# hku-mars/BALM

Measured on AMD Instinct MI355X. Metric: BA iterations/sec (W poses x F plane features), higher is better.
Workload: dtype f64

## Files before the change

### balm_amd/capi.py

```python
import ctypes as C
import os

import numpy as np

_HERE = os.path.dirname(os.path.abspath(__file__))
LIB_PATH = os.environ.get("BALM_HIP_LIB") or os.path.join(_HERE, "lib", "libbalm_hip.so")

FORM_LEFT, FORM_RIGHT = 0, 1
OK, ERR_ARG, ERR_HIP, ERR_STATE, ERR_TOO_FEW_PLANES, ERR_NUMERIC = range(6)
ABI_VERSION = 6
FLAG_TIMING = 1
FLAG_LOOPBACK_SHARDS = 2
FLAG_SYRK_INT8 = 4
T_MOMENTS, T_FACTORS, T_SYRK, T_ASSEMBLE, T_SOLVE, T_UPDATE, T_BUILD, T_VOXEL, T_COV, T_COMM, T_UPLOAD, T_COUNT = range(12)
TIMING_NAMES = ["moments", "factors", "syrk", "assemble", "solve", "update", "build", "voxel", "cov", "comm", "upload"]

EXPORTS = ["balm_create", "balm_prewarm", "balm_create_multi", "balm_destroy", "balm_set_features", "balm_set_features_cb", "balm_evaluate", "balm_only_residual",
           "balm_solve_damped", "balm_damping_iter", "balm_build_clusters", "balm_build_clusters_planes", "balm_voxel_defaults", "balm_associate", "balm_associate_scans", "balm_get_features", "balm_get_association", "balm_pose_covariance",
           "balm_window_open", "balm_window_add_scan", "balm_window_add_scan_strided", "balm_window_recut", "balm_window_get_points", "balm_window_features", "balm_window_marginalize", "balm_window_info", "balm_window_close",
           "balm_set_allreduce", "balm_comm_unique_id", "balm_comm_init_rank", "balm_comm_info",
           "balm_get_timing", "balm_get_shard_timing", "balm_get_solve_trace", "balm_chain_macro_plan", "balm_reset_timing", "balm_work_model", "balm_last_error", "balm_version", "balm_abi_version"]


class IterLog(C.Structure):
    _fields_ = [("r1", C.c_double), ("r2", C.c_double), ("u", C.c_double), ("v", C.c_double),
                ("q", C.c_double), ("q1", C.c_double), ("accepted", C.c_int), ("hess_evaluated", C.c_int)]


class LMOpts(C.Structure):
    _fields_ = [("form", C.c_int), ("u0", C.c_double), ("max_iter", C.c_int), ("rel_tol", C.c_double),
                ("min_planes_per_pose", C.c_int), ("force_hess", C.c_int), ("no_stop", C.c_int),
                ("verbose", C.c_int), ("reanchor", C.c_int), ("abs_tol", C.c_double)]


class VoxelOpts(C.Structure):
    _fields_ = [("voxel_size", C.c_double), ("eigen_thr", C.c_float * 3), ("min_ps", C.c_int), ("layer_limit", C.c_int),
                ("min_observers", C.c_int), ("fix_frames", C.c_int), ("max_plane_dist", C.c_double),
                ("max_lambda21", C.c_double), ("max_lambda0", C.c_double), ("want_point_features", C.c_int),
                ("fix_point_limit", C.c_int), ("defer_recut", C.c_int)]


ALLREDUCE_FN = C.CFUNCTYPE(C.c_int, C.c_void_p, C.c_long, C.c_void_p)
FILL_CLUSTERS_FN = C.CFUNCTYPE(None, C.c_void_p, C.c_int, C.c_int, C.POINTER(C.c_double))

_LIB = None


class BalmError(RuntimeError):
    def __init__(self, code, msg):
        super().__init__("balm_hip error %d: %s" % (code, msg))
        self.code = code


def lib():
    global _LIB
    if _LIB is None:
        if not os.path.exists(LIB_PATH):
            raise ImportError("libbalm_hip.so is not built (%s missing): run `python -m balm_amd.build`. "
                              "There is no CPU fallback for the HIP path." % LIB_PATH)
        L = C.CDLL(LIB_PATH)
        abi = getattr(L, "balm_abi_version", None)
        abi = abi() if abi is not None else 0
        if abi != ABI_VERSION:
            raise ImportError("libbalm_hip.so has ABI revision %d, this binding was written for %d: rebuild (python -m balm_amd.build)"
                              % (abi, ABI_VERSION))
        L.balm_create.restype = C.c_void_p
        L.balm_create.argtypes = [C.c_int, C.c_int, C.c_int]
        L.balm_create_multi.restype = C.c_void_p
        L.balm_create_multi.argtypes = [C.c_int, C.c_int, C.c_int, C.c_int]
        L.balm_prewarm.argtypes = [C.c_int]
        L.balm_destroy.restype = None
        L.balm_destroy.argtypes = [C.c_void_p]
        L.balm_set_features.argtypes = [C.c_void_p, C.c_int, C.c_void_p, C.c_void_p, C.c_void_p]
        L.balm_set_features_cb.argtypes = [C.c_void_p, C.c_int, FILL_CLUSTERS_FN, C.c_void_p, C.c_void_p, C.c_void_p]
        L.balm_evaluate.argtypes = [C.c_void_p, C.c_int, C.c_void_p, C.c_int, C.c_int, C.c_void_p, C.c_void_p,
                                    C.POINTER(C.c_double)]
        L.balm_only_residual.argtypes = [C.c_void_p, C.c_void_p, C.POINTER(C.c_double)]
        L.balm_solve_damped.argtypes = [C.c_void_p, C.c_void_p, C.c_void_p, C.c_double, C.c_void_p,
                                        C.POINTER(C.c_double)]
        L.balm_damping_iter.argtypes = [C.c_void_p, C.POINTER(LMOpts), C.c_void_p, C.POINTER(IterLog),
                                        C.POINTER(C.c_int)]
        L.balm_build_clusters.argtypes = [C.c_void_p, C.c_int, C.c_void_p, C.c_void_p, C.c_void_p, C.c_long,
                                          C.c_void_p, C.c_void_p, C.c_void_p]
        L.balm_build_clusters_planes.argtypes = [C.c_void_p, C.c_int, C.c_void_p, C.c_void_p, C.c_size_t, C.c_size_t, C.c_void_p,
                                                 C.c_void_p, C.c_void_p]
        L.balm_associate_scans.argtypes = [C.c_void_p, C.POINTER(VoxelOpts), C.c_int, C.c_void_p, C.c_void_p, C.c_size_t,
                                           C.c_void_p, C.POINTER(C.c_int), C.POINTER(C.c_long)]
        L.balm_window_add_scan_strided.argtypes = [C.c_void_p, C.c_void_p, C.c_long, C.c_size_t, C.c_void_p]
        L.balm_window_open.argtypes = [C.c_void_p, C.POINTER(VoxelOpts)]
        L.balm_window_add_scan.argtypes = [C.c_void_p, C.c_void_p, C.c_long, C.c_void_p]
        L.balm_window_recut.argtypes = [C.c_void_p]
        L.balm_window_get_points.argtypes = [C.c_void_p, C.c_void_p, C.c_void_p, C.c_void_p, C.c_long, C.c_void_p]
        L.balm_window_features.argtypes = [C.c_void_p, C.POINTER(C.c_int)]
        L.balm_window_marginalize.argtypes = [C.c_void_p, C.c_int, C.c_void_p]
        L.balm_window_info.argtypes = [C.c_void_p, C.POINTER(C.c_int), C.POINTER(C.c_long), C.POINTER(C.c_long)]
        L.balm_window_close.argtypes = [C.c_void_p]
        L.balm_associate.argtypes = [C.c_void_p, C.POINTER(VoxelOpts), C.c_void_p, C.c_void_p, C.c_long, C.c_void_p,
                                     C.POINTER(C.c_int), C.POINTER(C.c_long)]
        L.balm_get_features.argtypes = [C.c_void_p, C.c_void_p, C.c_void_p, C.c_void_p]
        L.balm_get_association.argtypes = [C.c_void_p, C.c_void_p, C.c_void_p]
        L.balm_voxel_defaults.restype = None
        L.balm_voxel_defaults.argtypes = [C.POINTER(VoxelOpts)]
        L.balm_pose_covariance.argtypes = [C.c_void_p, C.c_void_p, C.c_void_p, C.c_double, C.c_void_p, C.c_void_p]
        L.balm_set_allreduce.argtypes = [C.c_void_p, ALLREDUCE_FN, C.c_void_p]
        L.balm_comm_unique_id.argtypes = [C.c_void_p]
        L.balm_comm_init_rank.argtypes = [C.c_void_p, C.c_int, C.c_int, C.c_void_p]
        L.balm_comm_info.argtypes = [C.c_void_p, C.c_void_p]
        L.balm_get_timing.argtypes = [C.c_void_p, C.c_void_p, C.c_void_p]
        L.balm_get_shard_timing.argtypes = [C.c_void_p, C.c_int, C.c_void_p, C.c_void_p]
        L.balm_get_solve_trace.argtypes = [C.c_void_p, C.c_void_p, C.c_long, C.c_void_p]
        L.balm_chain_macro_plan.argtypes = [C.c_int, C.c_int, C.c_void_p, C.c_long]
        L.balm_reset_timing.argtypes = [C.c_void_p]
        L.balm_work_model.argtypes = [C.c_void_p, C.c_void_p]
        L.balm_last_error.restype = C.c_char_p
        L.balm_last_error.argtypes = [C.c_void_p]
        L.balm_version.restype = C.c_char_p
        _LIB = L
    return _LIB


def chain_macro_plan(panels, helpers):
    tab = np.empty(helpers * 64, np.int32)
    rc = lib().balm_chain_macro_plan(int(panels), int(helpers), tab.ctypes.data_as(C.c_void_p), tab.size)
    if rc != OK:
        raise BalmError(rc, "balm_chain_macro_plan(%d, %d)" % (panels, helpers))
    tab = tab.reshape(helpers, 64)
    return [[(int(e) & 0xffff, int(e) >> 16) for e in row if e >= 0] for row in tab]


def _p(a):
    return None if a is None else a.ctypes.data_as(C.c_void_p)


def _c(a, dtype=np.float64):
    return None if a is None else np.ascontiguousarray(a, dtype=dtype)


class Context:

    def __init__(self, win_size, device=0, flags=0, n_devices=None):
        self.L = lib()
        self.W = int(win_size)
        self.n = 6 * self.W
        if n_devices is None:
            self.h = self.L.balm_create(self.W, int(device), int(flags))
        else:
            self.h = self.L.balm_create_multi(self.W, int(device), int(n_devices), int(flags))
        if not self.h:
            raise BalmError(ERR_HIP, "balm_create(win_size=%d, device=%d, n_devices=%s) failed (no GPU, bad device, or "
                                     "win_size out of range)" % (win_size, device, n_devices))
        self.F = 0
        self._cb = None

    def close(self):
        if getattr(self, "h", None):
            self.L.balm_destroy(self.h)
            self.h = None

    def __del__(self):
        try:
            self.close()
        except Exception:
            pass

    def _check(self, rc):
        if rc != OK:
# ... 284 lines not shown
```

### balm_amd/csrc/balm_capi.hip

```cpp
#include <algorithm>
#include <array>
#include <atomic>
#include <chrono>
#include <cmath>
#include <cstdio>
#include <cstdlib>
#include <cstring>

#include "balm_internal.h"

using namespace balm;

#define HIP_TRY(expr)                                                                              \
  do {                                                                                             \
    hipError_t e_ = (expr);                                                                        \
    if (e_ != hipSuccess) {                                                                        \
      ctx->err = std::string(#expr) + ": " + hipGetErrorString(e_);                                \
      return BALM_ERR_HIP;                                                                         \
    }                                                                                              \
  } while (0)

namespace {

#ifdef BALM_COLD_TRACE
// ... 18 lines not shown
};
static DeviceWarm g_warm[64];

static void warm_body(int device) {
  DeviceWarm &w = g_warm[device];
  if (hipSetDevice(device) != hipSuccess) { hipGetLastError(); return; }
  std::thread ring_th([&w, device] {
    if (hipSetDevice(device) == hipSuccess && w.ring.init(device) == hipSuccess) w.ring_ready.store(true, std::memory_order_release);
    else hipGetLastError();
  });
  (void)preload_voxel(); (void)preload_build(); (void)prepare_device_accum(); (void)preload_solve(); (void)prepare_device_cov();
  hipGetLastError();
  ring_th.join();
}

static int warm_start(int device) {
  if (device < 0 || device >= 64) return BALM_ERR_ARG;
  DeviceWarm &w = g_warm[device];
  std::lock_guard<std::mutex> lk(w.mu);
  if (!w.started) { w.started = true; w.th = std::thread(warm_body, device); }
  return BALM_OK;
}

static void adopt_warm_ring(balm_ctx *ctx) {
  if (ctx->ring.buf[0] || ctx->device < 0 || ctx->device >= 64) return;
  DeviceWarm &w = g_warm[ctx->device];
  std::lock_guard<std::mutex> lk(w.mu);
  if (!w.started) return;
  if (w.th.joinable()) w.th.join();
  if (w.ring_ready.load(std::memory_order_acquire)) {
    const int key = ctx->ring.pool_key;
    ctx->ring = w.ring; ctx->ring.pool_key = key;
    w.ring = PinnedRing(); w.ring_ready.store(false);
  }
}

struct Span {
  balm_ctx *c; int slot; hipEvent_t a = nullptr, b = nullptr;
  Span(balm_ctx *ctx, int s) : c(ctx), slot(s) {
    if (!c->timer.on) return;
    a = take(); b = take();
    hipEventRecord(a, c->stream);
  }
  ~Span() {
    if (!c->timer.on) return;
    hipEventRecord(b, c->stream);
    c->timer.pending.push_back({a, b, slot});
  }
  hipEvent_t take() {
    if (!c->timer.pool.empty()) { hipEvent_t e = c->timer.pool.back(); c->timer.pool.pop_back(); return e; }
    hipEvent_t e; hipEventCreate(&e); return e;
  }
};

void collect_timing(balm_ctx *c) {
  for (auto &sp : c->timer.pending) {
    float ms = 0;
    if (hipEventElapsedTime(&ms, sp.a, sp.b) == hipSuccess) { c->timer.ms[sp.slot] += ms; c->timer.cnt[sp.slot]++; }
    c->timer.pool.push_back(sp.a); c->timer.pool.push_back(sp.b);
  }
  c->timer.pending.clear();
}

template <class T>
int dalloc(balm_ctx *ctx, T **p, size_t count) {
  if (*p) { hipFree(*p); *p = nullptr; }
  if (count == 0) count = 1;
  HIP_TRY(hipMalloc((void **)p, count * sizeof(T)));
  return BALM_OK;
}

template <class T>
int keep(balm_ctx *ctx, T **p, size_t *cap, size_t count) {
  if (*p && *cap >= count) return BALM_OK;
  for (int k = 0; k < balm_ctx::LM_GRAPHS; k++)
    if (ctx->lm_graph[k]) { hipGraphExecDestroy(ctx->lm_graph[k]); ctx->lm_graph[k] = nullptr; ctx->lm_graph_form[k] = -1; }
  int rc = dalloc(ctx, p, count + count / 4);
  *cap = rc ? 0 : count + count / 4;
  return rc;
}

template <class T>
int ensure(balm_ctx *ctx, T **p, size_t *cap, size_t count) {
  if (*p && *cap >= count) return BALM_OK;
  for (int k = 0; k < balm_ctx::LM_GRAPHS; k++)
    if (ctx->lm_graph[k]) { hipGraphExecDestroy(ctx->lm_graph[k]); ctx->lm_graph[k] = nullptr; ctx->lm_graph_form[k] = -1; }
  int rc = dalloc(ctx, p, count);
  if (rc) return rc;
  *cap = count;
  return BALM_OK;
}

int stage_begin(balm_ctx *ctx, size_t total_bytes) {
  total_bytes += 16 * 256;
  ctx->stage_off = 0;
  if (ctx->stage_cap >= total_bytes) return BALM_OK;
  if (ctx->d_stage) { hipStreamSynchronize(ctx->stream); hipFree(ctx->d_stage); ctx->d_stage = nullptr; ctx->stage_cap = 0; }
  const size_t want = total_bytes + total_bytes / 8;
  HIP_TRY(hipMalloc((void **)&ctx->d_stage, want));
  ctx->stage_cap = want;
  return BALM_OK;
}

template <class T>
T *stage_take(balm_ctx *ctx, size_t count) {
  const size_t off = (ctx->stage_off + 255) & ~(size_t)255;
  ctx->stage_off = off + count * sizeof(T);
  return reinterpret_cast<T *>(ctx->d_stage + off);
}

int sync_stream(balm_ctx *ctx) {
  HIP_TRY(hipStreamSynchronize(ctx->stream));
  HIP_TRY(hipGetLastError());
  collect_timing(ctx);
  return BALM_OK;
}

long red_dacc_off(const balm_ctx *c) { return (long)c->ntiles * TILE_ELEMS; }
long red_r_off(const balm_ctx *c) { return red_dacc_off(c) + (long)DACC_MAX * c->W; }

bool has_transport(const balm_ctx *ctx) { return ctx->comm || multi_is_loopback(ctx) || ctx->allreduce; }

int hook_allreduce(balm_ctx *ctx, double *buf, long n) {
  if (ctx->comm) { Span sp(ctx, BALM_T_COMM); return comm_allreduce(ctx, buf, n); }
  if (multi_is_loopback(ctx)) { Span sp(ctx, BALM_T_COMM); return loopback_allreduce(ctx, buf, n); }
  if (!ctx->allreduce) return BALM_OK;
  int rc = sync_stream(ctx);
  if (rc) return rc;
  if (ctx->allreduce((void *)buf, n, ctx->allreduce_user) != 0) {
    ctx->err = "all-reduce hook failed";
    return BALM_ERR_STATE;
  }
  return BALM_OK;
}

int set_damping(balm_ctx *ctx, double u) {
  ctx->u_value = u;
  ctx->u_on_device = false;
  return BALM_OK;
}
int push_damping(balm_ctx *ctx) {
  double *slot = ctx->h_scal + 16 + (ctx->u_ring++ & 63);
  *slot = ctx->u_value;
  HIP_TRY(hipMemcpyAsync(ctx->d_scal + SCAL_U, slot, sizeof(double), hipMemcpyHostToDevice, ctx->stream));
  ctx->u_on_device = true;
  return BALM_OK;
}

static void collect_timing_if_idle(balm_ctx *ctx) {
  if (!ctx->timer.on || ctx->timer.pending.empty()) return;
  if (hipStreamSynchronize(ctx->stream) == hipSuccess) collect_timing(ctx);
}

int wait_scalars(balm_ctx *ctx) {
  volatile double *stamp = ctx->h_scal + SCAL_STAMP;
  const double want = (double)ctx->mail_seq;
  const auto t0 = std::chrono::steady_clock::now();
  for (int spin = 0;; spin++) {
    if (*stamp == want) { std::atomic_thread_fence(std::memory_order_acquire); collect_timing_if_idle(ctx); return BALM_OK; }
    if ((spin & 255) == 255 && std::chrono::steady_clock::now() - t0 > std::chrono::microseconds(300)) break;
  }
  int rc = sync_stream(ctx);
  if (rc) return rc;
  if (*stamp != want) { ctx->err = "balm_damping_iter: the iteration's scalars did not arrive"; return BALM_ERR_HIP; }
  return BALM_OK;
}

void drop_lm_graphs(balm_ctx *ctx) {
  for (int k = 0; k < balm_ctx::LM_GRAPHS; k++) {
    if (ctx->lm_graph[k]) hipGraphExecDestroy(ctx->lm_graph[k]);
    ctx->lm_graph[k] = nullptr; ctx->lm_graph_form[k] = -1;
  }
}

int residual_device(balm_ctx *ctx, const double *d_poses, int f0, int f1, int slot, bool defer_sum = false, bool send_mail = false) {
  if (f1 <= f0) {
    HIP_TRY(hipMemsetAsync(ctx->d_scal + slot, 0, sizeof(double), ctx->stream));
    ctx->nr_tmp = 0;
  } else {
    Span sp(ctx, BALM_T_MOMENTS);
    launch_world_moments(ctx->stream, ctx->d_cl, d_poses, ctx->W, f0, f1, ctx->d_C);
    const EigenMail mail{ctx->d_scal, ctx->d_hscal, send_mail ? (double)++ctx->mail_seq : 0.0, slot};
    ctx->nr_tmp = launch_feature_eigen(ctx->stream, ctx->d_C, ctx->has_fix ? ctx->d_fix : nullptr, ctx->d_coe, f0, f1, ctx->d_feat_tmp,
                                       ctx->d_rpart_tmp, send_mail ? &mail : nullptr);
    if (!defer_sum) launch_sum_scalar(ctx->stream, ctx->d_rpart_tmp, ctx->nr_tmp, ctx->d_scal + slot);
  }
  HIP_TRY(hipGetLastError());
  if (defer_sum) return BALM_OK;
  return hook_allreduce(ctx, ctx->d_scal + slot, 1);
}

bool fuse_trial(const balm_ctx *ctx) {
  const char *e = getenv("BALM_FUSE_TRIAL");
  return ctx->W <= 256 && ctx->F > 0 && e && e[0] == '1';
}

static bool syrk_int8_mode(const balm_ctx *ctx) {
  if (ctx->flags & BALM_FLAG_SYRK_INT8) return true;
  const char *m = getenv("BALM_SYRK");
  return m && !strcmp(m, "int8");
}
static bool syrk_int8_for(const balm_ctx *ctx, long K) {
  if (!syrk_int8_mode(ctx)) return false;
  if (const char *m = getenv("BALM_SYRK_INT8_MIN_COLS")) return K >= atol(m);
  return K >= 12288L && ctx->W >= 96;
}

int prepare_evaluate(balm_ctx *ctx, int form, int nf) {
  if (nf <= 0) return BALM_OK;
  const SyrkPlan plan = plan_syrk(ctx->ntiles, 3L * nf);
  int rc;
  size_t gcols = (size_t)plan.Kpad + 64, parts = (size_t)plan.SG * ctx->ntiles;
  if (ctx->sparse && nf == ctx->F) {
    gcols = (size_t)ctx->sp_nchunks * ctx->sp_nsteps * 4 + 64;
    parts = (size_t)ctx->sp_nitems;
  }
  {
    const double *before = ctx->d_Gt;
    if ((rc = ensure(ctx, &ctx->d_Gt, &ctx->cap_Gt, gcols * ctx->npad))) return rc;
    if (ctx->d_Gt != before) ctx->gt_dirty_cols = ~(size_t)0;
  }
  if ((rc = ensure(ctx, &ctx->d_part, &ctx->cap_part, parts * TILE_ELEMS))) return rc;
  if (syrk_int8_for(ctx, 3L * nf) && !(ctx->sparse && nf == ctx->F)) {
    if ((rc = ensure(ctx, &ctx->d_i8, &ctx->cap_i8, syrk_i8_scratch_bytes(ctx->n, 3L * nf, nullptr)))) return rc;
    if (!ctx->d_rowmax) ctx->rowmax_cur_valid = false;
    if (!ctx->d_rowmax2) ctx->rowmax_trial_valid = false;
    if ((rc = ensure(ctx, &ctx->d_rowmax, &ctx->cap_rowmax, (size_t)ctx->npad + 128))) return rc;
    if ((rc = ensure(ctx, &ctx->d_rowmax2, &ctx->cap_rowmax2, (size_t)ctx->npad + 128))) return rc;
    if ((rc = ensure(ctx, &ctx->d_rowmax_part, &ctx->cap_rowmax_part, (size_t)factors_grid(ctx->W, nf, form) * 6 * ctx->W))) return rc;
    HIP_TRY(prepare_device_syrk_i8());
  }
  if ((rc = ensure(ctx, &ctx->d_dpart, &ctx->cap_dpart, (size_t)factors_grid(ctx->W, nf, form) * DACC_MAX * ctx->W))) return rc;
  if (nf == ctx->F && fuse_trial(ctx)) {
    if (ctx->cap_Gt2 < gcols * ctx->npad || ctx->cap_dpart2 < (size_t)factors_grid(ctx->W, nf, form) * DACC_MAX * ctx->W) ctx->gt_trial_valid = false;
    if ((rc = ensure(ctx, &ctx->d_Gt2, &ctx->cap_Gt2, gcols * ctx->npad))) return rc;
    if ((rc = ensure(ctx, &ctx->d_dpart2, &ctx->cap_dpart2, (size_t)factors_grid(ctx->W, nf, form) * DACC_MAX * ctx->W))) return rc;
  }
  return BALM_OK;
}

int evaluate_device(balm_ctx *ctx, int form, const double *d_poses, int f0, int f1, int slot) {
  const int W = ctx->W, nf = f1 - f0;
  const int dacc = form == 0 ? DACC_LEFT : DACC_RIGHT;
  int rc;
  if (nf <= 0) {
    HIP_TRY(hipMemsetAsync(ctx->d_red, 0, ctx->red_len * sizeof(double), ctx->stream));
    if ((rc = hook_allreduce(ctx, ctx->d_red, (long)ctx->red_len))) return rc;
    Span sp(ctx, BALM_T_ASSEMBLE);
    launch_assemble(ctx->stream, form, ctx->d_red, red_dacc_off(ctx), ctx->d_sub, ctx->ntiles, W, ctx->d_H, ctx->d_g,
                    ctx->d_red + red_r_off(ctx), ctx->d_scal + slot);
    return BALM_OK;
  }
  SyrkPlan plan = plan_syrk(ctx->ntiles, 3L * nf);
  if ((rc = prepare_evaluate(ctx, form, nf))) return rc;
  const int nblk = factors_grid(W, nf, form);
  hipStream_t s = ctx->stream;
  if (!(ctx->feat_cur_valid && f0 == 0 && f1 == ctx->F)) {
    Span sp(ctx, BALM_T_MOMENTS);
    launch_world_moments(s, ctx->d_cl, d_poses, W, f0, f1, ctx->d_C);
    ctx->nr_cur = launch_feature_eigen(s, ctx->d_C, ctx->has_fix ? ctx->d_fix : nullptr, ctx->d_coe, f0, f1, ctx->d_feat, ctx->d_rpart);
    ctx->feat_cur_valid = (f0 == 0 && f1 == ctx->F);
  }
  const int nr = ctx->nr_cur;
  const bool sparse = ctx->sparse && f0 == 0 && f1 == ctx->F;
  const size_t kpad = sparse ? (size_t)ctx->sp_nchunks * ctx->sp_nsteps * 4 : (size_t)plan.Kpad;
  if (!(ctx->gt_cur_valid && ctx->feat_cur_valid && f0 == 0 && f1 == ctx->F)) {
    Span sp(ctx, BALM_T_FACTORS);
    const size_t k0 = (size_t)3 * nf, k1 = kpad + 64;
    if (ctx->gt_dirty_cols == ~(size_t)0) {
      HIP_TRY(hipMemsetAsync(ctx->d_Gt, 0, ctx->cap_Gt * sizeof(double), s));
      ctx->gt_dirty_cols = 0;
    } else if (ctx->gt_dirty_cols > k0) {
      HIP_TRY(hipMemsetAsync(ctx->d_Gt + k0 * ctx->npad, 0, (std::max(ctx->gt_dirty_cols, k1) - k0) * ctx->npad * sizeof(double), s));
    }
    ctx->gt_dirty_cols = k0;
    ctx->rowmax_cur_valid = launch_factors(s, form, ctx->d_cl, d_poses, ctx->d_feat, W, ctx->npad, f0, f1, ctx->d_Gt, ctx->d_dpart, nblk,
                                           sparse ? ctx->d_slot : nullptr, (!sparse && syrk_int8_for(ctx, 3L * nf)) ? ctx->d_rowmax : nullptr, ctx->d_rowmax_part);
    ctx->gt_cur_valid = false;
  }
  HIP_TRY(hipGetLastError());
  const bool int8 = !sparse && syrk_int8_for(ctx, 3L * nf);
  {
    Span sp(ctx, BALM_T_SYRK);
    if (sparse) launch_syrk_sparse(s, ctx->d_Gt, ctx->npad, ctx->d_jobs, ctx->d_items, ctx->d_chunk_ids, ctx->sp_nsteps, ctx->sp_nitems, ctx->d_part);
    else if (int8) {
      if (launch_syrk_i8(s, ctx->d_Gt, ctx->npad, ctx->n, 3L * nf, ctx->d_sub, ctx->ntiles, ctx->d_i8, ctx->d_part,
                         ctx->rowmax_cur_valid ? ctx->d_rowmax : nullptr)) { ctx->err = "INT8 SYRK: unsupported size"; return BALM_ERR_ARG; }
      plan.SG = 1;
    }
    else launch_syrk(s, ctx->d_Gt, ctx->npad, ctx->ntiles, ctx->d_jobs, plan, ctx->d_part);
  }
  {
    Span sp(ctx, BALM_T_ASSEMBLE);
    launch_reduce(s, ctx->d_part, plan.SG, (long)ctx->ntiles * TILE_ELEMS, ctx->d_dpart, nblk, dacc * W,
                  ctx->d_rpart, nr, ctx->d_red, red_dacc_off(ctx), red_r_off(ctx), sparse ? ctx->d_csr : nullptr);
  }
  if ((rc = hook_allreduce(ctx, ctx->d_red, (long)ctx->red_len))) return rc;
  {
    Span sp(ctx, BALM_T_ASSEMBLE);
    launch_assemble(s, form, ctx->d_red, red_dacc_off(ctx), ctx->d_sub, ctx->ntiles, W, ctx->d_H, ctx->d_g, ctx->d_red + red_r_off(ctx),
                    ctx->d_scal + slot);
  }
  return BALM_OK;
}

int trial_device(balm_ctx *ctx, int form, const double *d_poses, int slot) {
  const int W = ctx->W, F = ctx->F;
  hipStream_t s = ctx->stream;
  const SyrkPlan plan = plan_syrk(ctx->ntiles, 3L * F);
  const bool sparse = ctx->sparse;
  const size_t kpad = sparse ? (size_t)ctx->sp_nchunks * ctx->sp_nsteps * 4 : (size_t)plan.Kpad;
  const int nblk = factors_grid(W, F, form);
  {
    Span sp(ctx, BALM_T_FACTORS);
    const size_t k0 = (size_t)3 * F, k1 = kpad + 64;
    HIP_TRY(hipMemsetAsync(ctx->d_Gt2 + k0 * ctx->npad, 0, (k1 - k0) * ctx->npad * sizeof(double), s));
    if (ctx->npad > ctx->n)
      HIP_TRY(hipMemset2DAsync(ctx->d_Gt2 + ctx->n, (size_t)ctx->npad * sizeof(double), 0,
                               (size_t)(ctx->npad - ctx->n) * sizeof(double), k0, s));
    ctx->nr_tmp = launch_moments_factors(s, form, ctx->d_cl, d_poses, ctx->has_fix ? ctx->d_fix : nullptr, ctx->d_coe, W, ctx->npad, F,
                                         ctx->d_Gt2, ctx->d_dpart2, nblk, sparse ? ctx->d_slot : nullptr, ctx->d_feat_tmp, ctx->d_rpart_tmp,
                                         (!sparse && syrk_int8_for(ctx, 3L * F) && ctx->d_rowmax2) ? ctx->d_rowmax2 : nullptr, ctx->d_rowmax_part);
    ctx->rowmax_trial_valid = !sparse && syrk_int8_for(ctx, 3L * F) && ctx->d_rowmax2;
  }
  HIP_TRY(hipGetLastError());
  {
    Span sp(ctx, BALM_T_MOMENTS);
    launch_sum_scalar(s, ctx->d_rpart_tmp, ctx->nr_tmp, ctx->d_scal + slot);
  }
  ctx->gt_trial_valid = true;
  return hook_allreduce(ctx, ctx->d_scal + slot, 1);
}

int read_scalars(balm_ctx *ctx) {
  HIP_TRY(hipMemcpyAsync(ctx->h_scal, ctx->d_scal, 16 * sizeof(double), hipMemcpyDeviceToHost, ctx->stream));
  return sync_stream(ctx);
}

std::vector<unsigned char> obs_of(const double *clusters, int F, int W) {
  std::vector<unsigned char> obs((size_t)F * W);
  parallel_ranges(obs.size(), (size_t)1 << 16, [&](size_t lo, size_t hi) {
    for (size_t t = lo; t < hi; t++) obs[t] = clusters[t * 10 + 9] != 0 ? 1 : 0;
  });
  return obs;
}

int feature_bookkeeping(balm_ctx *ctx, int F, const unsigned char *obs, const double *fix, const double *coeffs) {
  const int W = ctx->W;
  ctx->planes_per_pose.assign(W, 0);
  double S = 0, B = 0;
  int bad_a = F, bad_rc = BALM_OK;
  std::mutex mu;
  parallel_ranges((size_t)F, (size_t)(65536 / W + 1), [&](size_t lo, size_t hi) {
    std::vector<int> ppp((size_t)W, 0);
    double s = 0, b = 0;
    int my_bad = F, my_rc = BALM_OK;
    for (size_t a = lo; a < hi; a++) {
      int na = 0;
      const unsigned char *oa = obs + a * W;
      for (int i = 0; i < W; i++)
        if (oa[i]) { ppp[(size_t)i]++; na++; }
      if (my_rc == BALM_OK) {
        if (na == 0 && !(fix && fix[a * 10 + 9] != 0)) { my_bad = (int)a; my_rc = BALM_ERR_NUMERIC; }
        else if (!(coeffs[a] >= 0) || !std::isfinite(coeffs[a])) { my_bad = (int)a; my_rc = BALM_ERR_ARG; }
      }
      s += na; b += 0.5 * na * (na + 1.0);
    }
    std::lock_guard<std::mutex> lk(mu);
    for (int i = 0; i < W; i++) ctx->planes_per_pose[(size_t)i] += ppp[(size_t)i];
    S += s; B += b;
    if (my_rc != BALM_OK && my_bad < bad_a) { bad_a = my_bad; bad_rc = my_rc; }
  });
  if (bad_rc == BALM_ERR_NUMERIC) {
    ctx->err = "feature " + std::to_string(bad_a) + " has no observation and no fix cluster (zero point count)";
    return BALM_ERR_NUMERIC;
  }
  if (bad_rc == BALM_ERR_ARG) {
    ctx->err = "feature " + std::to_string(bad_a) + " has a negative or non-finite weight";
    return BALM_ERR_ARG;
  }
  ctx->work_S = S; ctx->work_B = B;
  return BALM_OK;
}

}

extern "C" {

const char *balm_version(void) { return "balm_hip 0.6.0 (gfx950)"; }
int balm_abi_version(void) { return BALM_ABI_VERSION; }

const char *balm_last_error(balm_ctx *ctx) { return ctx ? ctx->err.c_str() : "null context"; }

static void one_destroy(balm_ctx *ctx);

balm_ctx *balm_create(int win_size, int device, int flags) {
  if (win_size < 1 || win_size > MAX_W) return nullptr;
  cold_mark("balm_create: enter");
  int ndev = 0;
  if (hipGetDeviceCount(&ndev) != hipSuccess || ndev < 1 || device < 0 || device >= ndev) return nullptr;
  if (hipSetDevice(device) != hipSuccess) return nullptr;
  cold_mark("balm_create: hipGetDeviceCount + hipSetDevice");
  warm_start(device);
  if (prepare_device_accum() != hipSuccess || prepare_device_cov() != hipSuccess) return nullptr;
  cold_mark("balm_create: prepare_device (function attributes -> code objects)");
  balm_ctx *ctx = new balm_ctx();
  ctx->W = win_size;
  ctx->n = 6 * win_size;
  ctx->npad = (ctx->n + TILE - 1) / TILE * TILE;
  ctx->T = ctx->npad / TILE;
  ctx->nA = (ctx->n + NB - 1) / NB * NB;
  ctx->device = device;
  ctx->flags = flags;
  ctx->timer.on = (flags & BALM_FLAG_TIMING) != 0;
  auto fail = [&]() -> balm_ctx * { one_destroy(ctx); return nullptr; };
  std::vector<int> jobs, sub;
  {
    const int T = ctx->T, ngroups = T / 5;
    std::vector<std::array<int, 3>> mixed[4];
    std::vector<std::array<int, 2>> pairs;
    for (int r = 0; r < TM; r++) for (int c = r; c < TM; c++) pairs.push_back({r, c});
    for (int k = 0; k < 15; k++) mixed[1].push_back({0, pairs[k][0], pairs[k][1]});
    for (int k = 0; k < 10; k++) mixed[1].push_back({1, pairs[k][0], pairs[k][1]});
    for (int k = 10; k < 15; k++) mixed[2].push_back({1, pairs[k][0], pairs[k][1]});
    for (int k = 0; k < 15; k++) mixed[2].push_back({2, pairs[k][0], pairs[k][1]});
    for (int k = 0; k < 5; k++) mixed[2].push_back({3, pairs[k][0], pairs[k][1]});
    for (int k = 5; k < 15; k++) mixed[3].push_back({3, pairs[k][0], pairs[k][1]});
    for (int k = 0; k < 15; k++) mixed[3].push_back({4, pairs[k][0], pairs[k][1]});
    auto regular = [&](int I, int J) {
      jobs.insert(jobs.end(), {0, I, J, 0});
      for (int t = 0; t < 25; t++) sub.push_back(((TM * I + t / TM) << 16) | (TM * J + t % TM));
    };
    for (int m = 0; m < T; m++) {
      for (int i = 0; i < m; i++) regular(i, m);
      if (m >= TM * ngroups) regular(m, m);
      else if (m % TM == TM - 1) {
        const int b = m - (TM - 1);
        for (int v = 1; v <= 3; v++) {
          jobs.insert(jobs.end(), {v, b, b, 0});
          for (const auto &e : mixed[v]) sub.push_back(((TM * (b + e[0]) + e[1]) << 16) | (TM * (b + e[0]) + e[2]));
        }
      }
    }
  }
  ctx->ntiles = (int)(jobs.size() / 4);
  ctx->h_jobs = jobs;
  if (hipStreamCreateWithFlags(&ctx->stream, hipStreamNonBlocking) != hipSuccess) return fail();
  cold_mark("balm_create: job tables + stream");
  const int W = ctx->W, n = ctx->n, nA = ctx->nA;
  ctx->red_len = (size_t)ctx->ntiles * TILE_ELEMS + (size_t)DACC_MAX * W + 2;
  if (dalloc(ctx, &ctx->d_poses, (size_t)12 * W) || dalloc(ctx, &ctx->d_poses_tmp, (size_t)12 * W) ||
      dalloc(ctx, &ctx->d_red, ctx->red_len) || dalloc(ctx, &ctx->d_jobs, jobs.size()) || dalloc(ctx, &ctx->d_sub, sub.size()) ||
      dalloc(ctx, &ctx->d_H, (size_t)n * n) || dalloc(ctx, &ctx->d_g, (size_t)n) ||
      dalloc(ctx, &ctx->d_A, (size_t)(2 * nA + NB) * nA) || dalloc(ctx, &ctx->d_Wp, (size_t)2 * NB * (2 * nA + NB)) ||
      dalloc(ctx, &ctx->d_dvec, (size_t)nA) || dalloc(ctx, &ctx->d_z, (size_t)nA) || dalloc(ctx, &ctx->d_x, (size_t)16 * nA) ||
      dalloc(ctx, &ctx->d_perm, (size_t)nA) || dalloc(ctx, &ctx->d_flags, (size_t)2 * (2 * (nA / NB) + 1) * (nA / NB) + (nA / NB) + 8) || dalloc(ctx, &ctx->d_minv, (size_t)2 * (nA / NB) * NB * NB) || dalloc(ctx, &ctx->d_dx, (size_t)n) ||
      dalloc(ctx, &ctx->d_scal, (size_t)16) || dalloc(ctx, &ctx->d_pre, (size_t)W + 2))
    return fail();
  if (hipHostMalloc((void **)&ctx->h_scal, (16 + 64 + 8) * sizeof(double), hipHostMallocMapped | hipHostMallocCoherent) != hipSuccess) return fail();
  if (hipHostGetDevicePointer((void **)&ctx->d_hscal, ctx->h_scal, 0) != hipSuccess) return fail();
  ctx->h_scal[SCAL_STAMP] = 0.0;
  if (hipMemcpy(ctx->d_jobs, jobs.data(), jobs.size() * sizeof(int), hipMemcpyHostToDevice) != hipSuccess ||
      hipMemcpy(ctx->d_sub, sub.data(), sub.size() * sizeof(int), hipMemcpyHostToDevice) != hipSuccess)
    return fail();
  if (getenv("BALM_SOLVE_TRACE")) {
    const size_t cnt = (size_t)(2 * (nA / NB) + 1) * (nA / NB) * 6 + (size_t)(nA / NB) * 6;
    if (hipMalloc((void **)&ctx->d_trace, cnt * sizeof(long long)) != hipSuccess) return fail();
    hipMemset(ctx->d_trace, 0, cnt * sizeof(long long));
  }
  {
    std::vector<int> ident(nA);
    for (int i = 0; i < nA; i++) ident[i] = i;
    if (hipMemcpy(ctx->d_perm, ident.data(), (size_t)nA * sizeof(int), hipMemcpyHostToDevice) != hipSuccess) return fail();
  }
  if (hipMemset(ctx->d_scal, 0, 16 * sizeof(double)) != hipSuccess) return fail();
  if (hipMemset(ctx->d_red, 0, ctx->red_len * sizeof(double)) != hipSuccess) return fail();
  if (hipMemset(ctx->d_minv, 0, (size_t)2 * (nA / NB) * NB * NB * sizeof(double)) != hipSuccess) return fail();
  cold_mark("balm_create: device buffers + small copies");
  context_born(device); ctx->counted_live = true;
  return ctx;
}

static void one_destroy(balm_ctx *ctx) {
  if (!ctx) return;
  if (ctx->counted_live) { context_gone(ctx->device); ctx->counted_live = false; }
  comm_destroy(ctx);
  drop_lm_graphs(ctx);
  hipSetDevice(ctx->device);
  if (ctx->stream) hipStreamSynchronize(ctx->stream);
  if (ctx->window) { window_close(ctx->window); ctx->window = nullptr; }
  void *ptrs[] = {ctx->d_cl, ctx->d_fix, ctx->d_coe, ctx->d_poses, ctx->d_poses_tmp, ctx->d_C, ctx->d_feat,
                  ctx->d_Gt, ctx->d_Gt2, ctx->d_dpart2, ctx->d_part, ctx->d_dpart, ctx->d_rpart, ctx->d_feat_tmp, ctx->d_rpart_tmp, ctx->d_red, ctx->d_jobs, ctx->d_sub, ctx->d_H,
                  ctx->d_g, ctx->d_A, ctx->d_Wp, ctx->d_dvec, ctx->d_z, ctx->d_x, ctx->d_perm, ctx->d_dx, ctx->d_scal, ctx->d_arena, ctx->d_pre, ctx->d_flags, ctx->d_minv, ctx->d_macro_tab, ctx->d_trace, ctx->d_slot, ctx->d_items, ctx->d_csr, ctx->d_chunk_ids, ctx->d_stage, ctx->d_i8, ctx->d_rowmax, ctx->d_rowmax2, ctx->d_rowmax_part};
  for (void *p : ptrs) if (p) hipFree(p);
  if (ctx->h_scal) hipHostFree(ctx->h_scal);
  ctx->ring.release();
  if (ctx->amail.host) hipHostFree((void *)ctx->amail.host);
  if (ctx->amail.scan_state) hipFree(ctx->amail.scan_state);
  for (auto &sp : ctx->timer.pending) { hipEventDestroy(sp.a); hipEventDestroy(sp.b); }
  for (auto e : ctx->timer.pool) hipEventDestroy(e);
  if (ctx->stream) hipStreamDestroy(ctx->stream);
  delete ctx;
}

static int build_sparse_plan(balm_ctx *ctx, int F, const unsigned char *obs) {
  ctx->sparse = false;
  const char *mode = getenv("BALM_SYRK");
  if (mode && !strcmp(mode, "dense")) return BALM_OK;
  if (syrk_int8_for(ctx, 3L * F)) return BALM_OK;
  const int W = ctx->W, T = ctx->T, ntiles = ctx->ntiles;
  if (T > 128 || T <= 2 || F < 64) return BALM_OK;
  struct Key { uint64_t hi, lo; int a; };
  std::vector<Key> keys((size_t)F);
  parallel_ranges((size_t)F, (size_t)(65536 / W + 1), [&](size_t a0, size_t a1) {
    for (size_t a = a0; a < a1; a++) {
      uint64_t hi = 0, lo = 0;
      const unsigned char *oa = obs + a * W;
      for (int i = 0; i < W; i++)
        if (oa[i])
          for (int b = (6 * i) / TILE; b <= (6 * i + 5) / TILE; b++) {
            if (b < 64) hi |= 1ull << (63 - b); else lo |= 1ull << (127 - b);
          }
      keys[a] = {hi, lo, (int)a};
    }
  });
  auto first_of = [&](const Key &k) { for (int b = 0; b < T; b++) if (b < 64 ? (k.hi >> (63 - b)) & 1 : (k.lo >> (127 - b)) & 1) return b; return T; };
  auto last_of = [&](const Key &k) { for (int b = T - 1; b >= 0; b--) if (b < 64 ? (k.hi >> (63 - b)) & 1 : (k.lo >> (127 - b)) & 1) return b; return -1; };
  std::vector<int> fb((size_t)F), lb((size_t)F);
  for (int a = 0; a < F; a++) { fb[(size_t)a] = first_of(keys[(size_t)a]); lb[(size_t)a] = last_of(keys[(size_t)a]); }
  std::sort(keys.begin(), keys.end(), [&](const Key &x, const Key &y) {
    if (fb[(size_t)x.a] != fb[(size_t)y.a]) return fb[(size_t)x.a] < fb[(size_t)y.a];
    if (lb[(size_t)x.a] != lb[(size_t)y.a]) return lb[(size_t)x.a] < lb[(size_t)y.a];
    return x.hi != y.hi ? x.hi > y.hi : (x.lo != y.lo ? x.lo > y.lo : x.a < y.a);
  });
  const int C = 16, nsteps = 3 * C / 4, nchunks = (F + C - 1) / C;
  auto touched = [](const Key &k, int b) { return b < 64 ? (k.hi >> (63 - b)) & 1 : (k.lo >> (127 - b)) & 1; };
  std::vector<int> slot((size_t)F);
  std::vector<std::vector<int>> chunks_of((size_t)ntiles);
  long total = 0;
  for (int c = 0; c < nchunks; c++) {
    Key cm{0, 0, 0};
    for (int k = c * C; k < F && k < (c + 1) * C; k++) { cm.hi |= keys[(size_t)k].hi; cm.lo |= keys[(size_t)k].lo; slot[(size_t)keys[(size_t)k].a] = k; }
    for (int j = 0; j < ntiles; j++) {
      const int type = ctx->h_jobs[(size_t)4 * j], I = ctx->h_jobs[(size_t)4 * j + 1], J = ctx->h_jobs[(size_t)4 * j + 2];
      bool need;
      if (type == 0) need = touched(cm, I) && touched(cm, J);
      else if (type == 1) need = touched(cm, I) || touched(cm, I + 1);
      else if (type == 2) need = touched(cm, I + 1) || touched(cm, I + 2) || touched(cm, I + 3);
      else need = touched(cm, I + 3) || touched(cm, I + 4);
      if (need) { chunks_of[(size_t)j].push_back(c); total++; }
    }
  }
  const double dense_steps = (double)ntiles * ((3.0 * F + 3) / 4), sparse_steps = (double)total * nsteps;
  const bool forced = mode && !strcmp(mode, "sparse");
  if (total == 0 || (!forced && !(sparse_steps < 0.8 * dense_steps))) return BALM_OK;
  long per = total / 2048;
  if (per < 8) per = 8;
  std::vector<int> items, chunk_ids, csr((size_t)ntiles + 1, 0);
  struct Order { int first_chunk, item; };
  std::vector<Order> order;
  int run = 0;
  for (int j = 0; j < ntiles; j++) {
    csr[(size_t)j] = run;
    const std::vector<int> &L = chunks_of[(size_t)j];
    const long pieces = ((long)L.size() + per - 1) / per;
    for (long q = 0; q < pieces; q++) {
      const size_t b = (size_t)((long)L.size() * q / pieces), e = (size_t)((long)L.size() * (q + 1) / pieces);
      order.push_back({L[b], (int)(items.size() / 4)});
      items.insert(items.end(), {j, (int)chunk_ids.size(), (int)(e - b), run++});
      chunk_ids.insert(chunk_ids.end(), L.begin() + (long)b, L.begin() + (long)e);
    }
  }
  csr[(size_t)ntiles] = run;
  std::stable_sort(order.begin(), order.end(), [](const Order &x, const Order &y) { return x.first_chunk < y.first_chunk; });
  std::vector<int> sorted_items;
  sorted_items.reserve(items.size());
  for (const Order &o : order) sorted_items.insert(sorted_items.end(), items.begin() + 4L * o.item, items.begin() + 4L * o.item + 4);
  if (chunk_ids.empty()) chunk_ids.push_back(0);
  int rc;
  if ((rc = keep(ctx, &ctx->d_slot, &ctx->cap_slot, (size_t)F)) || (rc = keep(ctx, &ctx->d_items, &ctx->cap_items, sorted_items.size())) ||
      (rc = keep(ctx, &ctx->d_chunk_ids, &ctx->cap_chunk_ids, chunk_ids.size())) || (rc = keep(ctx, &ctx->d_csr, &ctx->cap_csr, csr.size())))
    return rc;
  HIP_TRY(hipMemcpy(ctx->d_slot, slot.data(), slot.size() * sizeof(int), hipMemcpyHostToDevice));
  HIP_TRY(hipMemcpy(ctx->d_items, sorted_items.data(), sorted_items.size() * sizeof(int), hipMemcpyHostToDevice));
  HIP_TRY(hipMemcpy(ctx->d_chunk_ids, chunk_ids.data(), chunk_ids.size() * sizeof(int), hipMemcpyHostToDevice));
  HIP_TRY(hipMemcpy(ctx->d_csr, csr.data(), csr.size() * sizeof(int), hipMemcpyHostToDevice));
  ctx->sparse = true; ctx->sp_nsteps = nsteps; ctx->sp_nchunks = nchunks; ctx->sp_nitems = run; ctx->sp_steps = sparse_steps;
  return BALM_OK;
}

static int install_feature_buffers(balm_ctx *ctx, int F, const double *fix, const double *coeffs,
                                   hipMemcpyKind kind = hipMemcpyHostToDevice) {
  int rc;
  drop_lm_graphs(ctx);
  ctx->has_fix = fix != nullptr;
  if (fix) {
    if ((rc = keep(ctx, &ctx->d_fix, &ctx->cap_fix, (size_t)F * 10))) return rc;
    HIP_TRY(hipMemcpyAsync(ctx->d_fix, fix, (size_t)F * 10 * sizeof(double), kind, ctx->stream));
  }
  if ((rc = keep(ctx, &ctx->d_coe, &ctx->cap_coe, (size_t)F))) return rc;
  HIP_TRY(hipMemcpyAsync(ctx->d_coe, coeffs, (size_t)F * sizeof(double), kind, ctx->stream));
  if ((rc = keep(ctx, &ctx->d_C, &ctx->cap_C, (size_t)F * 10))) return rc;
  if ((rc = keep(ctx, &ctx->d_feat, &ctx->cap_feat, (size_t)F * FEAT_STRIDE))) return rc;
  if ((rc = keep(ctx, &ctx->d_feat_tmp, &ctx->cap_feat_tmp, (size_t)F * FEAT_STRIDE))) return rc;
  if ((rc = keep(ctx, &ctx->d_rpart, &ctx->cap_rpart, (size_t)(F + 255) / 256 + 1024 + 1))) return rc;
  if ((rc = keep(ctx, &ctx->d_rpart_tmp, &ctx->cap_rpart_tmp, (size_t)(F + 255) / 256 + 1024 + 1))) return rc;
  ctx->feat_cur_valid = false; ctx->gt_cur_valid = false;
  ctx->F = F;
  return BALM_OK;
}

static int assoc_clusters_host(balm_ctx *ctx);

using FillClusters = std::function<void(int, int, double *, unsigned char *)>;

static int one_set_features_fn(balm_ctx *ctx, int F, const FillClusters &fill, const double *fix, const double *coeffs, bool shard_books = false) {
  if (!ctx) return BALM_ERR_ARG;
  if (ctx->multi && F == 0) { ctx->F = 0; ctx->feat_cur_valid = false; ctx->gt_cur_valid = false; ctx->planes_per_pose.clear(); ctx->work_S = ctx->work_B = 0; return BALM_OK; }
  if (F < 1 || !fill || !coeffs) { ctx->err = "balm_set_features: bad argument"; return BALM_ERR_ARG; }
  HIP_TRY(hipSetDevice(ctx->device));
  const int W = ctx->W;
  const size_t count = (size_t)F * W * 10;
  int rc;
  if ((rc = assoc_clusters_host(ctx))) return rc;
  ctx->F = 0;
  adopt_warm_ring(ctx);
  if ((rc = keep(ctx, &ctx->d_cl, &ctx->cap_cl, count))) return rc;
  if ((rc = stage_begin(ctx, count * sizeof(double)))) return rc;
  double *d_aos = stage_take<double>(ctx, count);
  std::vector<unsigned char> obs((size_t)F * W);
  const size_t unit = (size_t)W * 10 * sizeof(double);
  hipError_t e;
  {
    Span sp(ctx, BALM_T_UPLOAD);
    e = staged_upload(ctx->ring, ctx->device, ctx->stream, d_aos, count * sizeof(double), unit, [&](char *dst, size_t off, size_t len) {
      const int f0 = (int)(off / unit), f1 = f0 + (int)(len / unit);
      fill(f0, f1, reinterpret_cast<double *>(dst), obs.data() + (size_t)f0 * W);
    });
  }
  if (e == hipSuccess) launch_transpose_clusters(ctx->stream, d_aos, ctx->d_cl, F, W);
  HIP_TRY(e);
  if ((!ctx->multi || shard_books) && (rc = feature_bookkeeping(ctx, F, obs.data(), fix, coeffs))) { hipStreamSynchronize(ctx->stream); return rc; }
  if ((rc = build_sparse_plan(ctx, F, obs.data()))) { hipStreamSynchronize(ctx->stream); return rc; }
  if ((rc = install_feature_buffers(ctx, F, fix, coeffs))) { hipStreamSynchronize(ctx->stream); return rc; }
  return sync_stream(ctx);
}

static int one_set_features(balm_ctx *ctx, int F, const double *clusters, const double *fix, const double *coeffs) {
  if (ctx && !(ctx->multi && F == 0) && !clusters) { ctx->err = "balm_set_features: bad argument"; return BALM_ERR_ARG; }
  const size_t row = ctx ? (size_t)ctx->W * 10 : 0;
  return one_set_features_fn(ctx, F, [clusters, row](int f0, int f1, double *dst, unsigned char *o) {
    const double *src = clusters + (size_t)f0 * row;
    stream_copy(dst, src, (size_t)(f1 - f0) * row * sizeof(double));
// ... 415 lines not shown
  const int nblk = cov_factors_grid(W, F > 0 ? F : 1);
  if ((rc = ensure(ctx, &ctx->d_dpart, &ctx->cap_dpart, (size_t)nblk * DACC_MAX * W))) return rc;
  const bool int8 = F > 0 && syrk_int8_for(ctx, 3L * F);
  if (int8) {
    if ((rc = ensure(ctx, &ctx->d_i8, &ctx->cap_i8, syrk_i8_scratch_bytes(ctx->n, 3L * F, nullptr)))) return rc;
    HIP_TRY(prepare_device_syrk_i8());
  }
  const size_t pay = 2 * tiles + (size_t)21 * W, nn = (size_t)n * n;
  const size_t ncc = (cluster_cov && F > 0) ? (size_t)F * W * 81 : 0;
  if ((rc = stage_begin(ctx, (pay + 2 * nn + 2 * (size_t)nA * nA + ncc) * sizeof(double)))) return rc;
  double *buf = stage_take<double>(ctx, pay + 2 * nn + 2 * (size_t)nA * nA), *d_cc = nullptr;
  double *redx = buf, *redy = buf + tiles, *sdiag = buf + 2 * tiles, *Rraw = buf + pay, *Rc = Rraw + nn,
         *T0 = Rc + nn, *T1 = T0 + (size_t)nA * nA;
  hipError_t e = hipSuccess;
  if (ncc) {
    d_cc = stage_take<double>(ctx, ncc);
    adopt_warm_ring(ctx);
    if (e == hipSuccess) { Span sp(ctx, BALM_T_UPLOAD); e = staged_copy(ctx->ring, ctx->device, s, d_cc, cluster_cov, (size_t)F * W * 81 * sizeof(double)); }
  }
  double *Gx = ctx->d_Gt, *Gy = ctx->d_Gt + gcols * ctx->npad;
  if (e == hipSuccess && F == 0) e = hipMemsetAsync(buf, 0, pay * sizeof(double), s);
  if (e == hipSuccess && F > 0) {
    Span sp(ctx, BALM_T_COV);
    const size_t k0 = (size_t)3 * F;
    hipMemsetAsync(Gx + k0 * ctx->npad, 0, (gcols - k0) * ctx->npad * sizeof(double), s);
    hipMemsetAsync(Gy + k0 * ctx->npad, 0, (gcols - k0) * ctx->npad * sizeof(double), s);
    launch_cov_factors(s, ctx->d_cl, d_cc, point_sigma * point_sigma, ctx->d_poses, ctx->d_feat, W, ctx->npad, F, Gx, Gy,
                       ctx->d_dpart, nblk);
    e = hipGetLastError();
    if (int8) {
      if (launch_syrk_i8(s, Gx, ctx->npad, ctx->n, 3L * F, ctx->d_sub, ctx->ntiles, ctx->d_i8, ctx->d_part)) e = hipErrorInvalidValue;
      launch_cov_reduce_tiles(s, ctx->d_part, 1, (long)tiles, redx);
      if (launch_syrk_i8(s, Gy, ctx->npad, ctx->n, 3L * F, ctx->d_sub, ctx->ntiles, ctx->d_i8, ctx->d_part)) e = hipErrorInvalidValue;
      launch_cov_reduce_tiles(s, ctx->d_part, 1, (long)tiles, redy);
    } else {
      launch_syrk(s, Gx, ctx->npad, ctx->ntiles, ctx->d_jobs, plan, ctx->d_part);
      launch_cov_reduce_tiles(s, ctx->d_part, plan.SG, (long)tiles, redx);
      launch_syrk(s, Gy, ctx->npad, ctx->ntiles, ctx->d_jobs, plan, ctx->d_part);
      launch_cov_reduce_tiles(s, ctx->d_part, plan.SG, (long)tiles, redy);
    }
    launch_cov_reduce_dacc(s, ctx->d_dpart, nblk, W, sdiag);
  }
  if (e == hipSuccess) rc = hook_allreduce(ctx, buf, (long)pay);
  if (e == hipSuccess && !rc) {
    Span sp(ctx, BALM_T_COV);
    launch_cov_assemble(s, redx, redy, sdiag, ctx->d_sub, ctx->ntiles, W, Rraw);
    hipMemsetAsync(ctx->d_g, 0, (size_t)n * sizeof(double), s);
    set_damping(ctx, 0.0);
    ctx->need_minv = true;
    launch_solve(ctx, true);
    ctx->need_minv = false;
    launch_congruence_inverse(ctx, Rraw, T0, T1, Rc);
    if (Rcov) e = hipMemcpyAsync(Rcov, Rc, nn * sizeof(double), hipMemcpyDeviceToHost, s);
    if (e == hipSuccess && Rcov_raw) e = hipMemcpyAsync(Rcov_raw, Rraw, nn * sizeof(double), hipMemcpyDeviceToHost, s);
  }
  if (e == hipSuccess) e = hipStreamSynchronize(s);
  if (e == hipSuccess) e = hipGetLastError();
  if (rc) return rc;
  HIP_TRY(e);
  collect_timing(ctx);
  return BALM_OK;
}

int balm_comm_info(balm_ctx *ctx, long *out4) {
  if (!ctx || !out4) return BALM_ERR_ARG;
  out4[0] = 1; out4[1] = 0; out4[2] = (long)ctx->red_len; out4[3] = 0;
  if (ctx->comm) {
    int cnt = -1, rk = -1;
    comm_query(ctx, &cnt, &rk);
    out4[0] = cnt; out4[1] = rk; out4[3] = 1;
  } else if (multi_is_loopback(ctx)) {
    out4[0] = ctx->multi->n; out4[1] = ctx->rank; out4[3] = 2;
  } else if (ctx->allreduce) {
    out4[0] = -1; out4[3] = 3;
  }
  return BALM_OK;
}

int balm_set_allreduce(balm_ctx *ctx, balm_allreduce_fn fn, void *user) {
  if (!ctx) return BALM_ERR_ARG;
  if (fn && (ctx->multi || ctx->comm)) { ctx->err = "balm_set_allreduce: the context already has a collective transport"; return BALM_ERR_STATE; }
  ctx->allreduce = fn;
  ctx->allreduce_user = user;
  return BALM_OK;
}

static int one_evaluate(balm_ctx *ctx, int form, const double *poses, int head, int end, double *Hess, double *JacT,
                  double *residual) {
  if (!ctx) return BALM_ERR_ARG;
  if (!ctx->multi) {
    if (ctx->F < 1) { ctx->err = "balm_evaluate: no features installed"; return BALM_ERR_STATE; }
    if ((form != 0 && form != 1) || !poses || head < 0 || end > ctx->F || head >= end) {
      ctx->err = "balm_evaluate: bad argument"; return BALM_ERR_ARG;
    }
  }
  HIP_TRY(hipSetDevice(ctx->device));
  const int n = ctx->n;
  HIP_TRY(hipMemcpyAsync(ctx->d_poses, poses, (size_t)12 * ctx->W * sizeof(double), hipMemcpyHostToDevice, ctx->stream));
  ctx->feat_cur_valid = false; ctx->gt_cur_valid = false;
  int rc = evaluate_device(ctx, form, ctx->d_poses, head, end, 0);
  ctx->feat_cur_valid = false; ctx->gt_cur_valid = false;
  if (rc) return rc;
  if (Hess) HIP_TRY(hipMemcpyAsync(Hess, ctx->d_H, (size_t)n * n * sizeof(double), hipMemcpyDeviceToHost, ctx->stream));
  if (JacT) HIP_TRY(hipMemcpyAsync(JacT, ctx->d_g, (size_t)n * sizeof(double), hipMemcpyDeviceToHost, ctx->stream));
  if ((rc = read_scalars(ctx))) return rc;
  if (residual) *residual = ctx->h_scal[0];
  if (!std::isfinite(ctx->h_scal[0])) { ctx->err = "balm_evaluate: non-finite residual"; return BALM_ERR_NUMERIC; }
  return BALM_OK;
}

static int one_only_residual(balm_ctx *ctx, const double *poses, double *residual) {
  if (!ctx) return BALM_ERR_ARG;
  if (!ctx->multi && ctx->F < 1) { ctx->err = "balm_only_residual: no features installed"; return BALM_ERR_STATE; }
  if (!poses || !residual) { ctx->err = "balm_only_residual: bad argument"; return BALM_ERR_ARG; }
  HIP_TRY(hipSetDevice(ctx->device));
  HIP_TRY(hipMemcpyAsync(ctx->d_poses_tmp, poses, (size_t)12 * ctx->W * sizeof(double), hipMemcpyHostToDevice, ctx->stream));
  int rc = residual_device(ctx, ctx->d_poses_tmp, 0, ctx->F, 1);
  if (rc) return rc;
  if ((rc = read_scalars(ctx))) return rc;
  *residual = ctx->h_scal[1];
  if (!std::isfinite(ctx->h_scal[1])) { ctx->err = "balm_only_residual: non-finite residual"; return BALM_ERR_NUMERIC; }
  return BALM_OK;
}

int balm_solve_damped(balm_ctx *ctx, const double *Hess, const double *JacT, double u, double *dxi, double *q1) {
  if (!ctx) return BALM_ERR_ARG;
  if (!Hess || !JacT || !dxi) { ctx->err = "balm_solve_damped: bad argument"; return BALM_ERR_ARG; }
  HIP_TRY(hipSetDevice(ctx->device));
  const int n = ctx->n;
  HIP_TRY(hipMemcpyAsync(ctx->d_H, Hess, (size_t)n * n * sizeof(double), hipMemcpyHostToDevice, ctx->stream));
  HIP_TRY(hipMemcpyAsync(ctx->d_g, JacT, (size_t)n * sizeof(double), hipMemcpyHostToDevice, ctx->stream));
  {
    Span sp(ctx, BALM_T_SOLVE);
    int rcu = set_damping(ctx, u);
    if (rcu) return rcu;
    launch_solve(ctx, true);
  }
  HIP_TRY(hipMemcpyAsync(dxi, ctx->d_dx, (size_t)n * sizeof(double), hipMemcpyDeviceToHost, ctx->stream));
  int rc = read_scalars(ctx);
  if (rc) return rc;
  if (!std::isfinite(ctx->h_scal[2]) && !ctx->persistent_off && solve_timed_out(ctx)) {
    ctx->persistent_off = true;
    {
      Span sp(ctx, BALM_T_SOLVE);
      launch_solve(ctx, true);
    }
    HIP_TRY(hipMemcpyAsync(dxi, ctx->d_dx, (size_t)n * sizeof(double), hipMemcpyDeviceToHost, ctx->stream));
    if ((rc = read_scalars(ctx))) return rc;
  }
  if (q1) *q1 = ctx->h_scal[2];
  return BALM_OK;
}

static int lm_enqueue(balm_ctx *ctx, int form, bool evaluated, bool mail) {
  int rc;
  if (evaluated && (rc = evaluate_device(ctx, form, ctx->d_poses, 0, ctx->F, 0))) return rc;
  {
    Span sp(ctx, BALM_T_SOLVE);
    launch_solve(ctx, evaluated, form, ctx->d_poses, ctx->d_poses_tmp);
  }
  ctx->gt_trial_valid = false;
  bool sum_in_mail = false;
  if (fuse_trial(ctx) && ctx->d_Gt2 && ctx->d_dpart2) {
    if ((rc = trial_device(ctx, form, ctx->d_poses_tmp, 1))) return rc;
  } else {
    sum_in_mail = mail && !has_transport(ctx) && ctx->F > 0;
    const bool eigen_mails = sum_in_mail && ctx->F <= 256;
    if ((rc = residual_device(ctx, ctx->d_poses_tmp, 0, ctx->F, 1, sum_in_mail, eigen_mails))) return rc;
    if (eigen_mails) return BALM_OK;
  }
  if (mail) launch_scalars_mail(ctx->stream, ctx->d_scal, ctx->d_hscal, (double)++ctx->mail_seq, sum_in_mail ? ctx->d_rpart_tmp : nullptr,
                                ctx->nr_tmp, 1);
  else HIP_TRY(hipMemcpyAsync(ctx->h_scal, ctx->d_scal, 16 * sizeof(double), hipMemcpyDeviceToHost, ctx->stream));
  return BALM_OK;
}

static int lm_iteration(balm_ctx *ctx, int form, bool evaluated, int it) {
  const char *genv = getenv("BALM_GRAPH");
  const bool disabled = !(genv && (!strcmp(genv, "1") || !strcmp(genv, "debug")));
  const bool graphable = !disabled && ctx->graphs_ok && it >= 1 && !ctx->timer.on && !has_transport(ctx) && !ctx->multi &&
                         ctx->feat_cur_valid && ctx->F > 0 && !solve_is_persistent(ctx);
  if (graphable) {
    const bool fused = fuse_trial(ctx) && ctx->d_Gt2 && ctx->d_dpart2;
    const int slot = (ctx->gt_parity ? 16 : 0) | (fused ? 8 : 0) | (ctx->gt_cur_valid ? 4 : 0) | (evaluated ? 2 : 0) | ctx->parity;
    if (ctx->lm_graph[slot] && ctx->lm_graph_form[slot] != form) {
      hipGraphExecDestroy(ctx->lm_graph[slot]); ctx->lm_graph[slot] = nullptr;
    }
    if (!ctx->lm_graph[slot]) {
      hipGraph_t g = nullptr;
      ctx->u_on_device = true;
      bool ok = hipStreamBeginCapture(ctx->stream, hipStreamCaptureModeThreadLocal) == hipSuccess;
      if (ok) {
        const int rc = lm_enqueue(ctx, form, evaluated, false);
        const hipError_t e = hipStreamEndCapture(ctx->stream, &g);
        ok = rc == BALM_OK && e == hipSuccess && g != nullptr;
      }
      if (ok) ok = hipGraphInstantiate(&ctx->lm_graph[slot], g, nullptr, nullptr, 0) == hipSuccess;
      if (g) hipGraphDestroy(g);
      if (genv && !strcmp(genv, "debug")) fprintf(stderr, "balm_hip: LM graph slot %d capture %s\n", slot, ok ? "ok" : "FAILED");
      if (!ok) {
        hipGetLastError();
        ctx->lm_graph[slot] = nullptr;
        ctx->graphs_ok = false;
      } else {
        ctx->lm_graph_form[slot] = form;
      }
    }
    if (ctx->lm_graph[slot]) {
      int rcu = push_damping(ctx);
      if (rcu) return rcu;
      HIP_TRY(hipGraphLaunch(ctx->lm_graph[slot], ctx->stream));
      return sync_stream(ctx);
    }
    ctx->u_on_device = false;
  }
  int rc = lm_enqueue(ctx, form, evaluated, true);
  if (rc) return rc;
  return wait_scalars(ctx);
}

static int one_damping_iter(balm_ctx *ctx, const balm_lm_opts *o, double *poses, balm_iter_log *log, int *n_iters) {
  if (!ctx) return BALM_ERR_ARG;
  if (!ctx->multi && ctx->F < 1) { ctx->err = "balm_damping_iter: no features installed"; return BALM_ERR_STATE; }
  if (!o || !poses || (o->form != 0 && o->form != 1) || o->max_iter < 1) {
    ctx->err = "balm_damping_iter: bad argument"; return BALM_ERR_ARG;
  }
  if (n_iters) *n_iters = 0;
  HIP_TRY(hipSetDevice(ctx->device));
  const int W = ctx->W, F = ctx->F;
  hipStream_t s = ctx->stream;
  cold_mark("damping_iter: enter");
  int rc = prepare_evaluate(ctx, o->form, F);
  cold_mark("damping_iter: prepare_evaluate (scratch allocations)");
  std::vector<double> pre((size_t)W + 2, 0.0);
  for (size_t i = 0; i < ctx->planes_per_pose.size() && i < (size_t)W; i++) pre[i] = ctx->planes_per_pose[i];
  pre[(size_t)W] = rc ? 1.0 : 0.0;
  if (has_transport(ctx)) {
    int rc2;
    if (hipMemcpyAsync(ctx->d_pre, pre.data(), pre.size() * sizeof(double), hipMemcpyHostToDevice, s) != hipSuccess) return BALM_ERR_HIP;
    if ((rc2 = hook_allreduce(ctx, ctx->d_pre, (long)pre.size()))) return rc2;
    if (hipMemcpyAsync(pre.data(), ctx->d_pre, pre.size() * sizeof(double), hipMemcpyDeviceToHost, s) != hipSuccess) return BALM_ERR_HIP;
    if ((rc2 = sync_stream(ctx))) return rc2;
    if (pre[(size_t)W] != 0.0 && !rc) { ctx->err = "balm_damping_iter: another rank failed before the loop"; rc = BALM_ERR_STATE; }
  }
  if (rc) return rc;
  if (o->min_planes_per_pose > 0) {
    double mn = pre[0];
    for (int i = 1; i < W; i++) mn = pre[(size_t)i] < mn ? pre[(size_t)i] : mn;
    if (mn < o->min_planes_per_pose) {
      ctx->err = "Initial error too large. Please loose plane determination criteria for more planes. "
                 "The optimization is terminated.";
      return BALM_ERR_TOO_FEW_PLANES;
    }
  }
  HIP_TRY(hipMemcpyAsync(ctx->d_poses, poses, (size_t)12 * W * sizeof(double), hipMemcpyHostToDevice, s));
  ctx->feat_cur_valid = false; ctx->gt_cur_valid = false;
  double u = o->u0, v = 2, r1 = 0, r2 = 0;
  bool calc = true;
  int it = 0;
  int fault_rank = -1, fault_it = -1, timeout_it = -1;
  if (const char *fi = getenv("BALM_FAULT_INJECT")) {
    if (!strncmp(fi, "timeout,", 8)) timeout_it = atoi(fi + 8);
    else if (ctx->multi) sscanf(fi, "%d,%d", &fault_rank, &fault_it);
  }
  while (it < o->max_iter) {
    const bool evaluated = calc || o->force_hess;
    if (ctx->rank == fault_rank && it == fault_it) { ctx->err = "balm_damping_iter: injected fault"; return BALM_ERR_HIP; }
    if (it == timeout_it) { ctx->inject_solve_timeout = true; timeout_it = -1; }
    if ((rc = set_damping(ctx, u))) return rc;
    if ((rc = lm_iteration(ctx, o->form, evaluated, it))) return rc;
    double sc[3] = {ctx->h_scal[0], ctx->h_scal[1], ctx->h_scal[2]};
    if ((rc = multi_share_scalars(ctx, it, sc, 3))) return rc;
    r1 = sc[0]; r2 = sc[1];
    const double q1 = sc[2];
    double q = r1 - r2;
    if (!ctx->multi && !ctx->persistent_off && !(std::isfinite(r2) && std::isfinite(q1)) && std::isfinite(r1) && solve_timed_out(ctx)) {
      ctx->persistent_off = true;
      drop_lm_graphs(ctx);
      ctx->feat_cur_valid = false; ctx->gt_cur_valid = false;
      calc = true;
      continue;
    }
    if (!(std::isfinite(r1) && std::isfinite(r2))) {
      ctx->err = "balm_damping_iter: non-finite residual";
      return BALM_ERR_NUMERIC;
    }
    if (log) { log[it].r1 = r1; log[it].r2 = r2; log[it].u = u; log[it].v = v; log[it].q = q; log[it].q1 = q1;
               log[it].accepted = q > 0; log[it].hess_evaluated = evaluated; }
    if (o->verbose)
    {
      printf("iter%d: (%lf %lf) u: %lf v: %.1lf q: %.3lf %lf %lf\n", it, r1, r2, u, v, q / q1, q1, q);
      fflush(stdout);
    }
    if (q > 0) {
      double *t = ctx->d_poses; ctx->d_poses = ctx->d_poses_tmp; ctx->d_poses_tmp = t;
      t = ctx->d_feat; ctx->d_feat = ctx->d_feat_tmp; ctx->d_feat_tmp = t;
      t = ctx->d_rpart; ctx->d_rpart = ctx->d_rpart_tmp; ctx->d_rpart_tmp = t;
      ctx->nr_cur = ctx->nr_tmp;
      ctx->feat_cur_valid = true;
      ctx->gt_cur_valid = ctx->gt_trial_valid;
      if (ctx->gt_trial_valid) {
        std::swap(ctx->d_Gt, ctx->d_Gt2); std::swap(ctx->cap_Gt, ctx->cap_Gt2);
        std::swap(ctx->d_rowmax, ctx->d_rowmax2); std::swap(ctx->cap_rowmax, ctx->cap_rowmax2);
        ctx->rowmax_cur_valid = ctx->rowmax_trial_valid;
        ctx->gt_dirty_cols = ~(size_t)0;
        std::swap(ctx->d_dpart, ctx->d_dpart2); std::swap(ctx->cap_dpart, ctx->cap_dpart2);
        ctx->gt_parity ^= 1;
      }
      ctx->parity ^= 1;
      q = q / q1; v = 2; q = 1 - std::pow(2 * q - 1, 3);
      u *= (q < 1.0 / 3.0 ? 1.0 / 3.0 : q);
      calc = true;
    } else {
      u = u * v; v = 2 * v; calc = false;
    }
    it++;
    if (!o->no_stop && std::fabs(r1 - r2) / r1 < o->rel_tol) break;
    if (!o->no_stop && o->abs_tol > 0 && std::fabs(r1 - r2) < o->abs_tol) break;
  }
  ctx->feat_cur_valid = false; ctx->gt_cur_valid = false;
  if (o->reanchor) launch_reanchor(s, W, ctx->d_poses);
  HIP_TRY(hipMemcpyAsync(poses, ctx->d_poses, (size_t)12 * W * sizeof(double), hipMemcpyDeviceToHost, s));
  if ((rc = sync_stream(ctx))) return rc;
  if (n_iters) *n_iters = it;
  cold_mark("damping_iter: done");
  return BALM_OK;
}

static balm_multi *leader_of(balm_ctx *ctx) { return (ctx && ctx->multi && ctx->rank == 0) ? ctx->multi : nullptr; }

int balm_prewarm(int device) {
  int ndev = 0;
  if (hipGetDeviceCount(&ndev) != hipSuccess || device < 0 || device >= ndev) { hipGetLastError(); return BALM_ERR_ARG; }
  return warm_start(device);
}

balm_ctx *balm_create_multi(int win_size, int first_device, int n_devices, int flags) {
  if (n_devices < 1 || n_devices > MAX_SHARDS) return nullptr;
  const bool loopback = (flags & BALM_FLAG_LOOPBACK_SHARDS) != 0;
  HostPool::shard_pool_threads() = n_devices > 4 ? 8 : 0;
  std::vector<balm_ctx *> subs;
  for (int k = 0; k < n_devices; k++) {
    balm_ctx *c = balm_create(win_size, loopback ? first_device : first_device + k, flags);
    if (!c) { for (auto *q : subs) one_destroy(q); return nullptr; }
    c->ring.pool_key = k;
    subs.push_back(c);
  }
  std::string err;
  balm_multi *m = multi_new(subs, loopback, &err);
  if (!m) {
    fprintf(stderr, "balm_create_multi: %s\n", err.c_str());
    for (auto *q : subs) one_destroy(q);
    return nullptr;
  }
  return subs[0];
}

void balm_destroy(balm_ctx *ctx) {
  if (!ctx) return;
  if (balm_multi *m = ctx->multi) {
    std::vector<balm_ctx *> subs = m->sub;
    for (auto *q : subs) { hipSetDevice(q->device); if (q->stream) hipStreamSynchronize(q->stream); }
    multi_delete(m);
    for (auto *q : subs) { q->multi = nullptr; one_destroy(q); }
    return;
  }
  one_destroy(ctx);
}

int balm_comm_unique_id(void *id128) {
  if (!id128) return BALM_ERR_ARG;
  return comm_unique_id(id128);
}

int balm_comm_init_rank(balm_ctx *ctx, int n_ranks, int rank, const void *id128) {
  if (!ctx) return BALM_ERR_ARG;
  if (!id128 || n_ranks < 1 || rank < 0 || rank >= n_ranks) { ctx->err = "balm_comm_init_rank: bad argument"; return BALM_ERR_ARG; }
  if (ctx->multi || ctx->comm) { ctx->err = "balm_comm_init_rank: the context already has a collective transport"; return BALM_ERR_STATE; }
  HIP_TRY(hipSetDevice(ctx->device));
  return comm_init_rank(ctx, n_ranks, rank, id128);
}

static int multi_set_features(balm_ctx *ctx, balm_multi *m, int F, const double *clusters, const double *fix, const double *coeffs) {
  if (F < 1 || !clusters || !coeffs) { ctx->err = "balm_set_features: bad argument"; return BALM_ERR_ARG; }
  m->F = 0;
  m->books_per_shard = false;
  for (size_t k = 1; k < m->sub.size(); k++) { m->sub[k]->planes_per_pose.clear(); m->sub[k]->work_S = m->sub[k]->work_B = 0; }
  const std::vector<unsigned char> obs = obs_of(clusters, F, ctx->W);
  int rc = feature_bookkeeping(ctx, F, obs.data(), fix, coeffs);
  if (rc) return rc;
  {
    const int W = ctx->W;
    std::vector<double> cum((size_t)F + 1, 0.0);
    parallel_ranges((size_t)F, (size_t)(65536 / W + 1), [&](size_t lo, size_t hi) {
      for (size_t a = lo; a < hi; a++) {
        int na = 0;
        const unsigned char *oa = obs.data() + a * W;
        for (int i = 0; i < W; i++) na += oa[i];
        cum[a + 1] = 0.5 * na * (na + 1.0) + 4.0 * na + 1.0;
      }
    });
    for (int a = 0; a < F; a++) cum[(size_t)a + 1] += cum[(size_t)a];
    m->fbeg[0] = 0;
    for (int k = 1; k < m->n; k++) {
      const double target = cum[(size_t)F] * k / m->n;
      int f = (int)(std::lower_bound(cum.begin(), cum.end(), target) - cum.begin());
      if (f < m->fbeg[(size_t)k - 1]) f = m->fbeg[(size_t)k - 1];
      if (f > F) f = F;
      m->fbeg[(size_t)k] = f;
    }
    m->fbeg[(size_t)m->n] = F;
  }
  const size_t W = (size_t)ctx->W;
  rc = multi_run(m, [&](int k) {
    const int f0 = m->fbeg[(size_t)k], nf = m->fbeg[(size_t)k + 1] - f0;
    return one_set_features(m->sub[(size_t)k], nf, clusters + (size_t)f0 * W * 10, fix ? fix + (size_t)f0 * 10 : nullptr, coeffs + f0);
  });
  if (rc) { if (ctx->err.empty()) ctx->err = "balm_set_features: a device failed"; return rc; }
  m->F = F;
  return BALM_OK;
}

int balm_set_features(balm_ctx *ctx, int F, const double *clusters, const double *fix, const double *coeffs) {
  if (balm_multi *m = leader_of(ctx)) return multi_set_features(ctx, m, F, clusters, fix, coeffs);
  return one_set_features(ctx, F, clusters, fix, coeffs);
}

static void multi_cut(balm_multi *m, int F, const std::vector<double> &cum ) {
  m->fbeg[0] = 0;
  for (int k = 1; k < m->n; k++) {
    const double target = cum[(size_t)F] * k / m->n;
    int f = (int)(std::lower_bound(cum.begin(), cum.end(), target) - cum.begin());
    if (f < m->fbeg[(size_t)k - 1]) f = m->fbeg[(size_t)k - 1];
    if (f > F) f = F;
    m->fbeg[(size_t)k] = f;
  }
  m->fbeg[(size_t)m->n] = F;
}

static int multi_done(balm_ctx *ctx, balm_multi *m, int F, int rc, const char *who) {
  if (rc) { if (ctx->err.empty()) ctx->err = std::string(who) + ": a device failed"; for (auto *q : m->sub) if (!q->err.empty()) { ctx->err = q->err; break; } return rc; }
  m->F = F;
  m->books_per_shard = true;
  return BALM_OK;
}

int balm_set_features_cb(balm_ctx *ctx, int F, balm_fill_clusters_fn fill, void *user, const double *fix, const double *coeffs) {
  if (!ctx) return BALM_ERR_ARG;
  if (F < 1 || !fill || !coeffs) { ctx->err = "balm_set_features_cb: bad argument"; return BALM_ERR_ARG; }
  if (balm_multi *m = leader_of(ctx)) {
    const size_t Wc = (size_t)ctx->W, row = Wc * 10;
    m->F = 0;
    std::vector<double> cum((size_t)F + 1, 0.0);
    parallel_ranges((size_t)F, (size_t)(32768 / row + 1), [&](size_t lo, size_t hi) {
      const size_t blk = std::max<size_t>(1, (size_t)65536 / (row * sizeof(double)));
      std::vector<double> scratch(blk * row);
      for (size_t a0 = lo; a0 < hi; a0 += blk) {
        const size_t a1 = std::min(hi, a0 + blk);
        fill(user, (int)a0, (int)a1, scratch.data());
        for (size_t a = a0; a < a1; a++) {
          int na = 0;
          const double *r = scratch.data() + (a - a0) * row;
          for (size_t i = 0; i < Wc; i++) na += r[i * 10 + 9] != 0 ? 1 : 0;
          cum[a + 1] = 0.5 * na * (na + 1.0) + 4.0 * na + 1.0;
        }
      }
    });
    for (int a = 0; a < F; a++) cum[(size_t)a + 1] += cum[(size_t)a];
    multi_cut(m, F, cum);
    int rc = multi_run(m, [&](int k) {
      const int f0 = m->fbeg[(size_t)k], nf = m->fbeg[(size_t)k + 1] - f0;
      return one_set_features_fn(m->sub[(size_t)k], nf, [fill, user, Wc, f0](int a0, int a1, double *dst, unsigned char *o) {
        fill(user, f0 + a0, f0 + a1, dst);
        const size_t cnt = (size_t)(a1 - a0) * Wc;
        for (size_t t = 0; t < cnt; t++) o[t] = dst[t * 10 + 9] != 0 ? 1 : 0;
      }, fix ? fix + (size_t)f0 * 10 : nullptr, coeffs + f0, true);
    });
    return multi_done(ctx, m, F, rc, "balm_set_features_cb");
  }
// ... 286 lines not shown
```

### balm_amd/csrc/balm_internal.h

```cpp
#pragma once
#include <hip/hip_runtime.h>
#include <atomic>
#include <condition_variable>
#include <cstddef>
#include <cstdint>
#include <functional>
#include <mutex>
#include <string>
#include <thread>
#include <vector>

#include "../../include/balm_hip.h"
#include "host_stage.h"

namespace balm {

constexpr int TILE = 80;
constexpr int TM = 5;
constexpr int TILE_ELEMS = TILE * TILE;
constexpr int FEAT_STRIDE = 24;
constexpr int DACC_LEFT = 27;
constexpr int DACC_RIGHT = 30;
constexpr int DACC_MAX = 30;
constexpr int NB = 48;
constexpr int MAX_W_LDS = 480;
constexpr int MAX_W = 1024;
constexpr int MAX_SHARDS = 16;

enum { FT_NN = 0, FT_VBAR = 1, FT_LAM = 4, FT_U0 = 7, FT_U1 = 10, FT_U2 = 13, FT_C0 = 16, FT_C1 = 17,
       FT_C2 = 18, FT_COE = 19 };

struct Timer {
  bool on = false;
  struct Span { hipEvent_t a, b; int slot; };
  std::vector<Span> pending;
  std::vector<hipEvent_t> pool;
  double ms[BALM_T_COUNT] = {0};
  long cnt[BALM_T_COUNT] = {0};
};

}

namespace balm {
struct WindowSession;
struct AssocMail {
  volatile unsigned int *host = nullptr; unsigned int *dev = nullptr; unsigned int seq = 0;
  unsigned long long *scan_state = nullptr; unsigned int scan_gen = 0;
};
constexpr long SCAN_TILES_CAP = 8192;
}

struct balm_ctx {
  int W = 0, n = 0, npad = 0, T = 0, ntiles = 0, device = 0, flags = 0;
  int nA = 0;
  int F = 0;
  hipStream_t stream = nullptr;
  std::string err;

  double *d_cl = nullptr;
  double *d_fix = nullptr;
  double *d_coe = nullptr;
  double *d_poses = nullptr;
  double *d_poses_tmp = nullptr;
  double *d_C = nullptr;
  double *d_feat = nullptr;
  double *d_feat_tmp = nullptr;
  double *d_rpart_tmp = nullptr;
  int nr_cur = 0, nr_tmp = 0;
  bool feat_cur_valid = false;
  double *d_Gt = nullptr;
  double *d_Gt2 = nullptr, *d_dpart2 = nullptr;
  size_t cap_Gt2 = 0, cap_dpart2 = 0;
  size_t gt_dirty_cols = ~(size_t)0;
  bool gt_cur_valid = false;
  int gt_parity = 0;
  bool gt_trial_valid = false;
  size_t cap_cl = 0, cap_fix = 0, cap_coe = 0, cap_C = 0, cap_feat = 0, cap_feat_tmp = 0, cap_rpart = 0, cap_rpart_tmp = 0;
  size_t cap_slot = 0, cap_items = 0, cap_chunk_ids = 0, cap_csr = 0;
  bool has_fix = false;
  size_t cap_Gt = 0;
  double *d_part = nullptr;
  size_t cap_part = 0;
  double *d_dpart = nullptr;
  size_t cap_dpart = 0;
  double *d_rpart = nullptr;
  double *d_red = nullptr;
  size_t red_len = 0;
  std::vector<int> h_jobs;
  bool sparse = false;
  int sp_nsteps = 0, sp_nchunks = 0, sp_nitems = 0;
  int *d_slot = nullptr;
  int *d_items = nullptr;
  int *d_chunk_ids = nullptr;
  double sp_steps = 0;
  int *d_csr = nullptr;
  int *d_jobs = nullptr;
  int *d_sub = nullptr;
  double *d_H = nullptr;
  double *d_g = nullptr;
  double *d_A = nullptr;
  double *d_Wp = nullptr;
  double *d_dvec = nullptr;
  double *d_z = nullptr;
  double *d_x = nullptr;
  int *d_perm = nullptr;
  int *d_flags = nullptr;
  long long *d_trace = nullptr;
  int fused_cap = -1;
  int chain_cap = -1;
  double *d_minv = nullptr;
  int *d_macro_tab = nullptr;
  int macro_tab_P = 0, macro_tab_NH = 0;
  double *d_dx = nullptr;
  double *d_scal = nullptr;
  double *h_scal = nullptr;
  double *d_hscal = nullptr;
  unsigned long long mail_seq = 0;
  bool need_minv = false;
  bool solve_tiled = false;
  int chain_refused_P[2] = {-1, -1};
  bool solve_backsub = false;
  bool counted_live = false;
  bool persistent_off = false;
  bool inject_solve_timeout = false;
  bool small_ready = false, small_refused = false;
  double u_value = 0.0;
  bool u_on_device = false;
  int u_ring = 0;
  static constexpr int LM_GRAPHS = 32;
  hipGraphExec_t lm_graph[LM_GRAPHS] = {};
  int lm_graph_form[LM_GRAPHS] = {};
  bool graphs_ok = true;
  int parity = 0;
  std::vector<int> planes_per_pose;
  double work_S = 0, work_B = 0;
  std::vector<double> assoc_clusters, assoc_coeffs;
  bool assoc_cl_on_device = false;
  std::vector<int> assoc_layer, assoc_point_feat;
  std::vector<double> assoc_fix;
  balm::WindowSession *window = nullptr;
  bool window_dead = false;
  balm::AssocMail amail;
  void *d_arena = nullptr;
  size_t arena_cap = 0;
  char *d_stage = nullptr;
  size_t stage_cap = 0, stage_off = 0;
  balm::PinnedRing ring;
  balm_allreduce_fn allreduce = nullptr;
  void *allreduce_user = nullptr;
  balm::Timer timer;
  void *comm = nullptr;
  std::atomic<bool> comm_dead{false};
  bool comm_aborted = false;
  std::timed_mutex comm_mu;
  int rank = 0, nranks = 1;
  unsigned long long *d_rowmax = nullptr, *d_rowmax2 = nullptr; size_t cap_rowmax = 0, cap_rowmax2 = 0;
  double *d_rowmax_part = nullptr; size_t cap_rowmax_part = 0;
  bool rowmax_cur_valid = false, rowmax_trial_valid = false;
  unsigned char *d_i8 = nullptr; size_t cap_i8 = 0;
  struct balm_multi *multi = nullptr;
  double *d_pre = nullptr;
};

namespace balm {

hipError_t prepare_device_accum();
hipError_t prepare_device_cov();
hipError_t preload_solve();
hipError_t preload_build();
hipError_t preload_voxel();
void launch_transpose_clusters(hipStream_t s, const double *aos, double *soa, int F, int W);
void launch_world_moments(hipStream_t s, const double *cl, const double *poses, int W, int f0, int f1, double *C);
struct EigenMail { double *scal; double *host; double stamp; int slot; };
int launch_feature_eigen(hipStream_t s, const double *C, const double *fix, const double *coe, int f0, int f1,
                         double *feat, double *rpart, const EigenMail *mail = nullptr);
int factors_grid(int W, int nfeat, int form);
int factors_chunk(int W);
bool launch_factors(hipStream_t s, int form, const double *cl, const double *poses, const double *feat, int W,
                    int npad, int f0, int f1, double *Gt, double *dpart, int nblk, const int *slot = nullptr,
                    unsigned long long *rowmax = nullptr, double *rowmax_part = nullptr);
int launch_moments_factors(hipStream_t s, int form, const double *cl, const double *poses, const double *fix, const double *coe, int W,
                           int npad, int F, double *Gt, double *dpart, int nblk, const int *slot, double *feat, double *rpart,
                           unsigned long long *rowmax = nullptr, double *rowmax_part = nullptr);
struct SyrkPlan { int SG; int nsteps; int Kpad; long nblocks; };
SyrkPlan plan_syrk(int ntiles, long K);
void launch_syrk(hipStream_t s, const double *Gt, int npad, int ntiles, const int *tileIJ, const SyrkPlan &p,
                 double *part);
void launch_syrk_sparse(hipStream_t s, const double *Gt, int npad, const int *jobs, const int *items, const int *chunk_ids,
                        int nsteps, long nitems, double *part);
void launch_reduce(hipStream_t s, const double *part, int SG, long tile_elems_total, const double *dpart, int nblk,
                   int dacc_len, const double *rpart, int nr, double *red, long red_dacc_off, long red_r_off,
                   const int *csr_ptr = nullptr);
void launch_assemble(hipStream_t s, int form, const double *red, long red_dacc_off, const int *tileIJ, int ntiles,
                     int W, double *H, double *g, const double *r_in = nullptr, double *r_out = nullptr);
void launch_sum_scalar(hipStream_t s, const double *rpart, int nr, double *out);
struct I8Layout { int T, rows_p, NT, M; long Kp; size_t off_digits, off_rowmax, off_scale, off_part; };
size_t syrk_i8_scratch_bytes(int n, long K, I8Layout *lay);
hipError_t prepare_device_syrk_i8();
int launch_syrk_i8(hipStream_t s, const double *Gt, int npad, int n, long K, const int *tileIJ, int ntiles, unsigned char *scratch, double *part,
                   const unsigned long long *rowmax_known = nullptr);

struct Barrier;
}

struct balm_multi {
  int n = 0;
  bool loopback = false;
  std::vector<balm_ctx *> sub;
  std::vector<int> fbeg;
  int F = 0;
  bool books_per_shard = false;
  std::vector<std::thread> th;
  std::mutex mu;
  std::condition_variable cv_go, cv_done;
  uint64_t gen = 0;
  int pending = 0;
  bool quit = false;
  const std::function<int(int)> *job = nullptr;
  std::vector<int> rc;
  balm::Barrier *bar = nullptr;
  std::atomic<int> abort_rc{0};
  std::atomic<bool> dead{false};
  std::atomic<uint64_t> lm_seq{0};
  uint64_t lm_epoch = 0;
  double lm_vals[2][8] = {{0}};
  std::vector<hipEvent_t> ev1, ev2;
  std::vector<double *> lb_tmp, lb_buf;
  std::vector<size_t> lb_cap;
};

namespace balm {
balm_multi *multi_new(const std::vector<balm_ctx *> &subs, bool loopback, std::string *err);
void multi_delete(balm_multi *m);
int multi_run(balm_multi *m, const std::function<int(int)> &f);
int comm_unique_id(void *out128);
int comm_init_rank(balm_ctx *ctx, int nranks, int rank, const void *id128);
void comm_destroy(balm_ctx *ctx);
const char *rccl_load_error();
int comm_allreduce(balm_ctx *ctx, double *buf, long n);
void comm_query(const balm_ctx *ctx, int *count, int *rank);
int loopback_allreduce(balm_ctx *ctx, double *buf, long n);
bool multi_is_loopback(const balm_ctx *ctx);
int multi_share_scalars(balm_ctx *ctx, int it, double *vals, int count);
void multi_abort(balm_multi *m, int rc);
int multi_host_barrier_rc(balm_ctx *ctx, int rc);

constexpr int SCAL_U = 5;
constexpr int SCAL_STAMP = 16 + 64;
bool chain_macro_plan(int P, int NH, std::vector<int> &tab);
void context_born(int device);
void context_gone(int device);
bool solve_timed_out(balm_ctx *c);
bool solve_is_persistent(const balm_ctx *c);
void launch_solve(balm_ctx *c, bool new_hessian, int upd_form = 0, const double *upd_poses = nullptr, double *upd_out = nullptr);
void launch_update_poses(hipStream_t s, int form, int W, const double *poses, const double *dx, double *out);
void launch_scalars_mail(hipStream_t s, double *d_scal, double *d_hscal, double stamp, const double *rpart = nullptr, int nr = 0,
                         int slot = 0);
void launch_reanchor(hipStream_t s, int W, double *poses);

struct AssocOpts {
  int W;
  double voxel_size;
  float thr[3];
  int min_ps, layer_limit, min_observers, fix_frames;
  double max_dis, ratio21_max, lam0_max;
  int fix_limit = 50;
  int defer_recut = 0;
};
int associate_device(hipStream_t s, const float *d_xyz, const int *d_frame, const long *d_first, const double *d_poses, long n, const AssocOpts &o,
                     void *arena, size_t arena_cap, size_t *arena_need, int *F_out, double **d_out, double **d_coe,
                     double **d_fix, int **d_layer, int **d_point_feat, long *n_roots, AssocMail *mail, bool *outputs_owned);

WindowSession *window_open(hipStream_t s, const AssocOpts &o);
void window_close(WindowSession *w);
int window_add_scan(WindowSession *w, const float *xyz_new, long n_new, const double *pose12, bool xyz_on_host);
int window_recut(WindowSession *w);
int window_marginalize(WindowSession *w, int mg, const double *poses);
int window_features(WindowSession *w, int min_observers, int *F_out, double **d_out, double **d_coe, double **d_fix, int **d_layer);
long window_get_points(WindowSession *w, float *xyz, int *slot, int *feature, long cap);
int window_count(const WindowSession *w);
int window_min_observers(const WindowSession *w);
long window_points(const WindowSession *w);
long window_nodes(const WindowSession *w);

int cov_factors_grid(int W, int F);
void launch_cov_factors(hipStream_t s, const double *cl, const double *ccov, double sigma2, const double *poses,
                        const double *feat, int W, int npad, int F, double *Gx, double *Gy, double *dpart, int nblk);
void launch_cov_reduce_tiles(hipStream_t s, const double *part, int SG, long tile_total, double *red);
void launch_cov_reduce_dacc(hipStream_t s, const double *dpart, int nblk, int W, double *out);
void launch_cov_assemble(hipStream_t s, const double *redx, const double *redy, const double *sdiag, const int *tileIJ,
                         int ntiles, int W, double *Rout);
void launch_congruence_inverse(balm_ctx *c, const double *Rraw, double *T0, double *T1, double *Rcov);

void launch_build_clusters(hipStream_t s, const float *xyz, const int *feat_id, const int *pose_id, long n_pts,
                           int F, int W, double *soa, int *unsorted_flag);
void launch_build_clusters_any(hipStream_t s, const float *xyz, const int *feat_id, const int *pose_id, long n_pts,
                               int F, int W, double *soa);
void launch_soa_to_aos(hipStream_t s, const double *soa, double *aos, int F, int W);
void launch_rebase_ids(hipStream_t s, int *d_id, long n, int base);
void launch_expand_ids(hipStream_t s, const long *d_first, int m, long n, int *d_id);
void launch_unpack_xyzw(hipStream_t s, const float *d_rec, long n, float *d_xyz, int *d_aux);
void launch_obs_mask(hipStream_t s, const double *soa, int F, int W, unsigned char *mask);

}
```

### balm_amd/csrc/kernels_accum.hip

```cpp
#include "balm_internal.h"

namespace balm {

typedef double d4 __attribute__((ext_vector_type(4)));
typedef double d2 __attribute__((ext_vector_type(2)));

__device__ __forceinline__ double wave_sum(double v) {
#pragma unroll
  for (int off = 32; off > 0; off >>= 1) v += __shfl_xor(v, off, 64);
  return v;
}

struct Obs {
  double N;
  double Rv[3];
  double b[3];
  double Pw[6];
};

__device__ __forceinline__ void to_world(const double P[6], const double v[3], double N, const double R[9],
                                         const double p[3], Obs &o) {
  o.N = N;
#pragma unroll
  for (int r = 0; r < 3; r++) o.Rv[r] = R[r] * v[0] + R[3 + r] * v[1] + R[6 + r] * v[2];
// ... 57 lines not shown
  for (int t0 = 0; t0 < 12 * W; t0 += 10 * (int)blockDim.x) {
    double pv[10];
#pragma unroll
    for (int j = 0; j < 10; j++) {
      const int t = t0 + j * (int)blockDim.x + (int)threadIdx.x;
      pv[j] = t < 12 * W ? poses[t] : 0.0;
    }
#pragma unroll
    for (int j = 0; j < 10; j++) {
      const int t = t0 + j * (int)blockDim.x + (int)threadIdx.x;
      if (t < 12 * W) { const int i = t / 12, c = t - 12 * i; sp[c * W + i] = pv[j]; }
    }
  }
  __syncthreads();
  const int lane = threadIdx.x & 63, wv = threadIdx.x >> 6, nw = blockDim.x >> 6;
  for (int a = f0 + blockIdx.x * nw + wv; a < f1; a += gridDim.x * nw) {
    const double *ca = cl + (size_t)a * 10 * W;
    double acc[10];
#pragma unroll
    for (int c = 0; c < 10; c++) acc[c] = 0.0;
    for (int i = lane; i < W; i += 64) {
      double P[6], v[3];
      const double N = ca[(size_t)9 * W + i];
#pragma unroll
      for (int c = 0; c < 6; c++) P[c] = ca[(size_t)c * W + i];
#pragma unroll
      for (int c = 0; c < 3; c++) v[c] = ca[(size_t)(6 + c) * W + i];
      if ((int)N > 0) {
        double R[9], p[3];
#pragma unroll
        for (int c = 0; c < 9; c++) R[c] = sp[c * W + i];
#pragma unroll
        for (int c = 0; c < 3; c++) p[c] = sp[(9 + c) * W + i];
        Obs o;
        to_world(P, v, N, R, p, o);
#pragma unroll
        for (int c = 0; c < 6; c++) acc[c] += o.Pw[c];
#pragma unroll
        for (int c = 0; c < 3; c++) acc[6 + c] += o.b[c];
        acc[9] += N;
      }
    }
#pragma unroll
    for (int c = 0; c < 10; c++) acc[c] = wave_sum(acc[c]);
    if (lane == 0) {
#pragma unroll
      for (int c = 0; c < 10; c++) Cout[(size_t)a * 10 + c] = acc[c];
    }
  }
}

void launch_world_moments(hipStream_t s, const double *cl, const double *poses, int W, int f0, int f1, double *C) {
  int nf = f1 - f0;
  if (nf <= 0) return;
  int grid = (nf + 3) / 4;
  if (grid > 2048) grid = 2048;
  size_t lds = (size_t)12 * W * sizeof(double);
  hipLaunchKernelGGL(k_world_moments, dim3(grid), dim3(256), lds, s, cl, poses, W, f0, f1, C);
}

__device__ __forceinline__ void jrot(double &app, double &aqq, double &apq, double &arp, double &arq, double &v0p,
                                     double &v0q, double &v1p, double &v1q, double &v2p, double &v2q) {
  if (apq == 0.0) return;
  const double theta = (aqq - app) / (2.0 * apq);
  const double t = (theta >= 0.0 ? 1.0 : -1.0) / (fabs(theta) + sqrt(theta * theta + 1.0));
  const double c = 1.0 / sqrt(t * t + 1.0), s = t * c;
  app -= t * apq;
  aqq += t * apq;
  apq = 0.0;
  const double rp = c * arp - s * arq, rq = s * arp + c * arq;
  arp = rp; arq = rq;
  double x, y;
  x = c * v0p - s * v0q; y = s * v0p + c * v0q; v0p = x; v0q = y;
  x = c * v1p - s * v1q; y = s * v1p + c * v1q; v1p = x; v1q = y;
  x = c * v2p - s * v2q; y = s * v2p + c * v2q; v2p = x; v2q = y;
}

__device__ __forceinline__ void eig3_jacobi(double a00, double a01, double a02, double a11, double a12, double a22,
                                            double lam[3], double U[3][3]) {
  double v00 = 1, v01 = 0, v02 = 0, v10 = 0, v11 = 1, v12 = 0, v20 = 0, v21 = 0, v22 = 1;
  for (int sweep = 0; sweep < 30; sweep++) {
    const double off = a01 * a01 + a02 * a02 + a12 * a12;
    const double dia = a00 * a00 + a11 * a11 + a22 * a22;
    if (off <= 1e-300 || off <= 1e-34 * dia) break;
    jrot(a00, a11, a01, a02, a12, v00, v01, v10, v11, v20, v21);
    jrot(a00, a22, a02, a01, a12, v00, v02, v10, v12, v20, v22);
    jrot(a11, a22, a12, a01, a02, v01, v02, v11, v12, v21, v22);
  }
  double l0 = a00, l1 = a11, l2 = a22;
  double c0[3] = {v00, v10, v20}, c1[3] = {v01, v11, v21}, c2[3] = {v02, v12, v22};
#define BALM_CSWAP(la, lb, ca, cb)                                                         \
  if (la > lb) {                                                                            \
    double t_ = la; la = lb; lb = t_;                                                       \
    for (int k_ = 0; k_ < 3; k_++) { double s_ = ca[k_]; ca[k_] = cb[k_]; cb[k_] = s_; }    \
  }
  BALM_CSWAP(l0, l1, c0, c1)
  BALM_CSWAP(l1, l2, c1, c2)
  BALM_CSWAP(l0, l1, c0, c1)
#undef BALM_CSWAP
  lam[0] = l0; lam[1] = l1; lam[2] = l2;
  for (int k = 0; k < 3; k++) { U[k][0] = c0[k]; U[k][1] = c1[k]; U[k][2] = c2[k]; }
}

__global__ __launch_bounds__(256) void k_feature_eigen(const double *__restrict__ C, const double *__restrict__ fix,
                                                       const double *__restrict__ coe, int f0, int f1,
                                                       double *__restrict__ feat, double *__restrict__ rpart, EigenMail mail) {
  __shared__ double sred[256];
  const int a = f0 + blockIdx.x * blockDim.x + threadIdx.x;
  double res = 0.0;
  if (a < f1) {
    double c[10];
#pragma unroll
    for (int k = 0; k < 10; k++) c[k] = C[(size_t)a * 10 + k];
    if (fix) {
#pragma unroll
      for (int k = 0; k < 10; k++) c[k] += fix[(size_t)a * 10 + k];
    }
    const double NN = c[9];
    const double inv = 1.0 / NN;
    const double vb0 = c[6] * inv, vb1 = c[7] * inv, vb2 = c[8] * inv;
    double lam[3], U[3][3];
    eig3_jacobi(c[0] * inv - vb0 * vb0, c[1] * inv - vb0 * vb1, c[2] * inv - vb0 * vb2, c[3] * inv - vb1 * vb1,
                c[4] * inv - vb1 * vb2, c[5] * inv - vb2 * vb2, lam, U);
    const double w = coe[a];
    res = w * lam[0];
    double *f = feat + (size_t)a * FEAT_STRIDE;
    f[FT_NN] = NN;
    f[FT_VBAR] = vb0; f[FT_VBAR + 1] = vb1; f[FT_VBAR + 2] = vb2;
    f[FT_LAM] = lam[0]; f[FT_LAM + 1] = lam[1]; f[FT_LAM + 2] = lam[2];
#pragma unroll
    for (int k = 0; k < 3; k++) {
      f[FT_U0 + k] = U[k][0]; f[FT_U1 + k] = U[k][1]; f[FT_U2 + k] = U[k][2];
    }
    f[FT_C0] = sqrt(2.0 * w) * inv;
    f[FT_C1] = sqrt(2.0 * w / (lam[1] - lam[0])) * inv;
    f[FT_C2] = sqrt(2.0 * w / (lam[2] - lam[0])) * inv;
    f[FT_COE] = w;
  }
  sred[threadIdx.x] = res;
  __syncthreads();
  for (int s = 128; s > 0; s >>= 1) {
    if (threadIdx.x < s) sred[threadIdx.x] += sred[threadIdx.x + s];
    __syncthreads();
  }
  if (threadIdx.x == 0) rpart[blockIdx.x] = sred[0];
  if (!mail.host) return;
  if (threadIdx.x == 0) mail.scal[mail.slot] = sred[0];
  __syncthreads();
  volatile double *host = mail.host;
  if (threadIdx.x < 16) host[threadIdx.x] = ((int)threadIdx.x == mail.slot) ? sred[0] : mail.scal[threadIdx.x];
  __threadfence_system();
  __syncthreads();
  if (threadIdx.x == 0) { host[SCAL_STAMP] = mail.stamp; __threadfence_system(); }
}

int launch_feature_eigen(hipStream_t s, const double *C, const double *fix, const double *coe, int f0, int f1,
                         double *feat, double *rpart, const EigenMail *mail) {
  int nf = f1 - f0;
  if (nf <= 0) return 0;
  int grid = (nf + 255) / 256;
  const EigenMail none{nullptr, nullptr, 0.0, 0};
  hipLaunchKernelGGL(k_feature_eigen, dim3(grid), dim3(256), 0, s, C, fix, coe, f0, f1, feat, rpart, (mail && grid == 1) ? *mail : none);
  return grid;
}

__global__ __launch_bounds__(256) void k_sum_scalar(const double *__restrict__ part, int nr, double *__restrict__ out) {
  __shared__ double sred[256];
  double s = 0.0;
  for (int t = threadIdx.x; t < nr; t += 256) s += part[t];
  sred[threadIdx.x] = s;
  __syncthreads();
  for (int k = 128; k > 0; k >>= 1) {
    if (threadIdx.x < k) sred[threadIdx.x] += sred[threadIdx.x + k];
    __syncthreads();
  }
  if (threadIdx.x == 0) out[0] = sred[0];
}

void launch_sum_scalar(hipStream_t s, const double *rpart, int nr, double *out) {
  hipLaunchKernelGGL(k_sum_scalar, dim3(1), dim3(256), 0, s, rpart, nr, out);
}

__device__ __forceinline__ void cross3(const double a[3], const double b[3], double o[3]) {
  o[0] = a[1] * b[2] - a[2] * b[1];
  o[1] = a[2] * b[0] - a[0] * b[2];
  o[2] = a[0] * b[1] - a[1] * b[0];
}

__device__ __forceinline__ void store6(double *dst, const double x[6]) {
  d2 *q = reinterpret_cast<d2 *>(dst);
  d2 t0 = {x[0], x[1]}, t1 = {x[2], x[3]}, t2 = {x[4], x[5]};
  q[0] = t0; q[1] = t1; q[2] = t2;
}

struct FeatRec { double NN, iNN, vbar[3], u0[3], u1[3], u2[3], c0, c1, c2, coe; };

template <int FORM>
__device__ __forceinline__ void obs_factors(const FeatRec &fr, const double P[6], const double v[3], const double N,
                                            const double *__restrict__ sp, double *__restrict__ sacc, const int Wc, const int il,
                                            double col0[6], double col1[6], double col2[6]) {
  const double NN = fr.NN, iNN = fr.iNN, c0 = fr.c0, c1 = fr.c1, c2 = fr.c2, coe = fr.coe;
  const double *vbar = fr.vbar, *u0 = fr.u0, *u1 = fr.u1, *u2 = fr.u2;
  if ((int)N > 0) {
    double R[9], p[3];
#pragma unroll
    for (int c = 0; c < 9; c++) R[c] = sp[c * Wc + il];
#pragma unroll
    for (int c = 0; c < 3; c++) p[c] = sp[(9 + c) * Wc + il];

    if (FORM == 0) {
      Obs o;
      to_world(P, v, N, R, p, o);
      const double Pw[3][3] = {{o.Pw[0], o.Pw[1], o.Pw[2]}, {o.Pw[1], o.Pw[3], o.Pw[4]}, {o.Pw[2], o.Pw[4], o.Pw[5]}};
      double cvec[3];
#pragma unroll
      for (int r = 0; r < 3; r++) cvec[r] = o.b[r] - N * vbar[r];
      double m0[3], m1[3], m2[3];
      const double vu0 = vbar[0] * u0[0] + vbar[1] * u0[1] + vbar[2] * u0[2];
      const double vu1 = vbar[0] * u1[0] + vbar[1] * u1[1] + vbar[2] * u1[2];
      const double vu2 = vbar[0] * u2[0] + vbar[1] * u2[1] + vbar[2] * u2[2];
#pragma unroll
      for (int r = 0; r < 3; r++) {
        m0[r] = Pw[r][0] * u0[0] + Pw[r][1] * u0[1] + Pw[r][2] * u0[2] - o.b[r] * vu0;
        m1[r] = Pw[r][0] * u1[0] + Pw[r][1] * u1[1] + Pw[r][2] * u1[2] - o.b[r] * vu1;
        m2[r] = Pw[r][0] * u2[0] + Pw[r][1] * u2[1] + Pw[r][2] * u2[2] - o.b[r] * vu2;
      }
      const double s0 = cvec[0] * u0[0] + cvec[1] * u0[1] + cvec[2] * u0[2];
      const double s1 = cvec[0] * u1[0] + cvec[1] * u1[1] + cvec[2] * u1[2];
      const double s2 = cvec[0] * u2[0] + cvec[1] * u2[1] + cvec[2] * u2[2];
      double x00[3], x01[3], x10[3], x02[3], x20[3], bxu[3];
      cross3(m0, u0, x00);
      cross3(m0, u1, x01); cross3(m1, u0, x10);
      cross3(m0, u2, x02); cross3(m2, u0, x20);
      cross3(o.b, u0, bxu);
      double grad[6];
#pragma unroll
      for (int r = 0; r < 3; r++) {
        grad[r] = 2.0 * coe * iNN * x00[r];
        grad[3 + r] = 2.0 * coe * iNN * s0 * u0[r];
        col0[r] = c0 * bxu[r];
        col0[3 + r] = c0 * N * u0[r];
        col1[r] = c1 * (x01[r] + x10[r]);
        col1[3 + r] = c1 * (s0 * u1[r] + s1 * u0[r]);
        col2[r] = c2 * (x02[r] + x20[r]);
        col2[3 + r] = c2 * (s0 * u2[r] + s2 * u0[r]);
      }
      const double K[3][3] = {{0, -u0[2], u0[1]}, {u0[2], 0, -u0[0]}, {-u0[1], u0[0], 0}};
      double KP[3][3];
#pragma unroll
      for (int r = 0; r < 3; r++)
#pragma unroll
        for (int c = 0; c < 3; c++) KP[r][c] = K[r][0] * Pw[0][c] + K[r][1] * Pw[1][c] + K[r][2] * Pw[2][c];
      const double m0u0 = m0[0] * u0[0] + m0[1] * u0[1] + m0[2] * u0[2];
      const double k1 = coe * iNN, k2 = 2.0 * coe * iNN;
      double bd[21];
      int q = 0;
#pragma unroll
      for (int r = 0; r < 3; r++)
#pragma unroll
        for (int c = r; c < 3; c++) {
          double kpk = KP[r][0] * K[c][0] + KP[r][1] * K[c][1] + KP[r][2] * K[c][2];
          double ell = u0[r] * m0[c] + m0[r] * u0[c] - (r == c ? 2.0 * m0u0 : 0.0);
          bd[q++] = k1 * ell + k2 * kpk;
        }
#pragma unroll
      for (int r = 0; r < 3; r++)
#pragma unroll
        for (int c = 0; c < 3; c++) bd[q++] = k2 * bxu[r] * u0[c];
#pragma unroll
      for (int r = 0; r < 3; r++)
#pragma unroll
        for (int c = r; c < 3; c++) bd[q++] = k2 * N * u0[r] * u0[c];
#pragma unroll
      for (int k = 0; k < 6; k++) sacc[k * Wc + il] += grad[k];
#pragma unroll
      for (int k = 0; k < 21; k++) sacc[(6 + k) * Wc + il] += bd[k];
    } else {
      const double Pf[3][3] = {{P[0], P[1], P[2]}, {P[1], P[3], P[4]}, {P[2], P[4], P[5]}};
      const double NNi = (double)(int)NN;
      const double jNN = 1.0 / NNi;
      double r3[3];
#pragma unroll
      for (int c = 0; c < 3; c++) r3[c] = R[3 * c] * u0[0] + R[3 * c + 1] * u0[1] + R[3 * c + 2] * u0[2];
      double ai[3];
      cross3(v, r3, ai);
      double ti[3];
#pragma unroll
      for (int r = 0; r < 3; r++) ti[r] = p[r] - vbar[r];
      const double s = u0[0] * ti[0] + u0[1] * ti[1] + u0[2] * ti[2];
      double Pr[3];
#pragma unroll
      for (int r = 0; r < 3; r++) Pr[r] = Pf[r][0] * r3[0] + Pf[r][1] * r3[1] + Pf[r][2] * r3[2];
      const double h1[3] = {Pr[0] + v[0] * s, Pr[1] + v[1] * s, Pr[2] + v[2] * s};
      const double C1[3][3] = {{0, -h1[2], h1[1]}, {h1[2], 0, -h1[0]}, {-h1[1], h1[0], 0}};
      const double rh[3][3] = {{0, -r3[2], r3[1]}, {r3[2], 0, -r3[0]}, {-r3[1], r3[0], 0}};
      double Rv[3], combo2[3];
#pragma unroll
      for (int r = 0; r < 3; r++) {
        Rv[r] = R[r] * v[0] + R[3 + r] * v[1] + R[6 + r] * v[2];
        combo2[r] = Rv[r] + N * ti[r];
      }
      double E[3][3];
#pragma unroll
      for (int r = 0; r < 3; r++)
#pragma unroll
        for (int c = 0; c < 3; c++)
          E[r][c] = R[r] * Pf[0][c] + R[3 + r] * Pf[1][c] + R[6 + r] * Pf[2][c] + ti[r] * v[c];
      double Auk[3][6];
      const double c2u = combo2[0] * u0[0] + combo2[1] * u0[1] + combo2[2] * u0[2];
#pragma unroll
      for (int r = 0; r < 3; r++)
#pragma unroll
        for (int c = 0; c < 3; c++) {
          double erh = E[r][0] * rh[0][c] + E[r][1] * rh[1][c] + E[r][2] * rh[2][c];
          double rc1 = R[r] * C1[0][c] + R[3 + r] * C1[1][c] + R[6 + r] * C1[2][c];
          Auk[r][c] = (erh - rc1) * jNN;
          Auk[r][3 + c] = (combo2[r] * u0[c] + (r == c ? c2u : 0.0)) * jNN;
        }
      double jjt[6], a1[6], a2[6];
#pragma unroll
      for (int c = 0; c < 6; c++) {
        jjt[c] = Auk[0][c] * u0[0] + Auk[1][c] * u0[1] + Auk[2][c] * u0[2];
        a1[c] = Auk[0][c] * u1[0] + Auk[1][c] * u1[1] + Auk[2][c] * u1[2];
        a2[c] = Auk[0][c] * u2[0] + Auk[1][c] * u2[1] + Auk[2][c] * u2[2];
      }
      const double r0 = c0 * NN * jNN, r1 = c1 * NN, r2 = c2 * NN;
#pragma unroll
      for (int r = 0; r < 3; r++) {
        col0[r] = r0 * ai[r];
        col0[3 + r] = r0 * N * u0[r];
      }
#pragma unroll
      for (int c = 0; c < 6; c++) { col1[c] = r1 * a1[c]; col2[c] = r2 * a2[c]; }
      double D1[3][3];
#pragma unroll
      for (int r = 0; r < 3; r++)
#pragma unroll
        for (int c = 0; c < 3; c++)
          D1[r][c] = C1[r][c] - (rh[r][0] * Pf[0][c] + rh[r][1] * Pf[1][c] + rh[r][2] * Pf[2][c]);
      const double hj[3][3] = {{0, -jjt[2], jjt[1]}, {jjt[2], 0, -jjt[0]}, {-jjt[1], jjt[0], 0}};
      const double k2 = 2.0 * coe * jNN;
      double bd[24];
      int q = 0;
#pragma unroll
      for (int r = 0; r < 3; r++)
#pragma unroll
        for (int c = 0; c < 3; c++) {
          double d1rh = D1[r][0] * rh[0][c] + D1[r][1] * rh[1][c] + D1[r][2] * rh[2][c];
          bd[q++] = k2 * d1rh - 0.5 * coe * hj[r][c];
        }
#pragma unroll
      for (int r = 0; r < 3; r++)
#pragma unroll
        for (int c = 0; c < 3; c++) bd[q++] = k2 * ai[r] * u0[c];
#pragma unroll
      for (int r = 0; r < 3; r++)
#pragma unroll
        for (int c = r; c < 3; c++) bd[q++] = k2 * N * u0[r] * u0[c];
#pragma unroll
      for (int k = 0; k < 6; k++) sacc[k * Wc + il] += coe * jjt[k];
#pragma unroll
      for (int k = 0; k < 24; k++) sacc[(6 + k) * Wc + il] += bd[k];
    }
  } else {
#pragma unroll
    for (int k = 0; k < 6; k++) col0[k] = col1[k] = col2[k] = 0.0;
  }
}

__device__ __forceinline__ void track_rowmax(double rm[6], double &bad, const double col0[6], const double col1[6], const double col2[6]) {
#pragma unroll
  for (int k = 0; k < 6; k++) {
    rm[k] = fmax(rm[k], fmax(fabs(col0[k]), fmax(fabs(col1[k]), fabs(col2[k]))));
    bad = fma(col0[k] + col1[k] + col2[k], 0.0, bad);
  }
}
__device__ __forceinline__ void publish_rowmax(double *__restrict__ part, int W, int pose, const double rm[6], double bad) {
#pragma unroll
  for (int k = 0; k < 6; k++) part[(size_t)(blockIdx.x * 6 + k) * W + pose] = bad != bad ? bad : rm[k];
}
__device__ __forceinline__ double nanmax(double a, double b) { return (a != a || b != b) ? __longlong_as_double(0x7ff8000000000000ll) : fmax(a, b); }
__global__ __launch_bounds__(1024) void k_rowmax_reduce(const double *__restrict__ part, int nblk, int W, int npad, unsigned long long *__restrict__ rowmax) {
  __shared__ double sm[16][64];
  const int tx = threadIdx.x & 63, ty = threadIdx.x >> 6, t = blockIdx.x * 64 + tx;
  double m[4] = {0.0, 0.0, 0.0, 0.0};
  if (t < 6 * W) {
    int b = ty;
    for (; b + 48 < nblk; b += 64) {
#pragma unroll
      for (int u = 0; u < 4; u++) m[u] = nanmax(m[u], part[(size_t)(b + 16 * u) * 6 * W + t]);
    }
    for (; b < nblk; b += 16) m[0] = nanmax(m[0], part[(size_t)b * 6 * W + t]);
  }
  sm[ty][tx] = nanmax(nanmax(m[0], m[1]), nanmax(m[2], m[3]));
  __syncthreads();
  if (ty == 0) {
    double v = sm[0][tx];
#pragma unroll
    for (int k = 1; k < 16; k++) v = nanmax(v, sm[k][tx]);
    if (t < 6 * W) {
      const int r = t / W, pose = t - r * W;
      rowmax[6 * pose + r] = (unsigned long long)__double_as_longlong(v);
    } else if (t < npad) {
      rowmax[t] = 0ull;
    }
  }
}

template <int FORM, bool REGS, bool MAXR = false>
__global__ __launch_bounds__(256) void k_feature_factors(const double *__restrict__ cl,
                                                         const double *__restrict__ poses,
                                                         const double *__restrict__ feat, int W, int Wc, int npad, int f0,
                                                         int f1, double *__restrict__ Gt,
                                                         double *__restrict__ dpart, const int *__restrict__ slot, int staged,
                                                         double *__restrict__ rowmax_part = nullptr) {
  static_assert(!MAXR || REGS, "the row maxima live in the lane that owns the pose");
  double rm[6] = {0.0, 0.0, 0.0, 0.0, 0.0, 0.0}, bad = 0.0;
  constexpr int DACC = FORM == 0 ? DACC_LEFT : DACC_RIGHT;
  extern __shared__ __attribute__((aligned(16))) double sm[];
  const int p0 = blockIdx.y * Wc, wc = min(Wc, W - p0);
  double *sp = sm;
  double *sacc = sm + 12 * Wc;
  double preg[12], racc[DACC];
  if (REGS) {
    const double *q = poses + 12 * (p0 + (threadIdx.x < (unsigned)wc ? (int)threadIdx.x : 0));
#pragma unroll
    for (int c = 0; c < 12; c++) preg[c] = q[c];
#pragma unroll
    for (int k = 0; k < DACC; k++) racc[k] = 0.0;
  }
  if (!REGS)
  for (int t0 = 0; t0 < 12 * wc; t0 += 10 * (int)blockDim.x) {
    double pv[10];
#pragma unroll
    for (int j = 0; j < 10; j++) {
      const int t = t0 + j * (int)blockDim.x + (int)threadIdx.x;
      pv[j] = t < 12 * wc ? poses[12 * p0 + t] : 0.0;
    }
#pragma unroll
    for (int j = 0; j < 10; j++) {
      const int t = t0 + j * (int)blockDim.x + (int)threadIdx.x;
      if (t < 12 * wc) { const int il = t / 12, c = t - 12 * il; sp[c * Wc + il] = pv[j]; }
    }
  }
  if (!REGS) {
    for (int t = threadIdx.x; t < DACC * Wc; t += blockDim.x) sacc[t] = 0.0;
    __syncthreads();
  }

  double nxt[10];
  auto fetch = [&](int a, int i) {
    const double *ca = cl + (size_t)a * 10 * W + i;
#pragma unroll
    for (int c = 0; c < 10; c++) nxt[c] = ca[(size_t)c * W];
  };
  const int i_first = p0 + (threadIdx.x < (unsigned)wc ? (int)threadIdx.x : 0);
  const int a_begin = f0 + (int)blockIdx.x, a_end = f1, a_step = (int)gridDim.x;
  const int lane = threadIdx.x & 63;
  double *stg = sm + (12 + DACC) * Wc + (threadIdx.x >> 6) * 384;
  if (a_begin < a_end) fetch(a_begin, i_first);

  for (int a = a_begin; a < a_end; a += a_step) {
    const double *f = feat + (size_t)a * FEAT_STRIDE;
    const FeatRec fr = {f[FT_NN], 1.0 / f[FT_NN], {f[FT_VBAR], f[FT_VBAR + 1], f[FT_VBAR + 2]}, {f[FT_U0], f[FT_U0 + 1], f[FT_U0 + 2]},
                        {f[FT_U1], f[FT_U1 + 1], f[FT_U1 + 2]}, {f[FT_U2], f[FT_U2 + 1], f[FT_U2 + 2]}, f[FT_C0], f[FT_C1], f[FT_C2], f[FT_COE]};
    const double *ca = cl + (size_t)a * 10 * W;
    double *g0 = Gt + (size_t)(3 * (slot ? slot[a] : a - f0)) * npad;

    for (int ilb = 0; ilb < wc; ilb += blockDim.x) {
      const int il = ilb + (int)threadIdx.x;
      if (il - lane >= wc) break;
      const bool act = il < wc;
      const int i = p0 + (act ? il : wc - 1);
      double col0[6], col1[6], col2[6];
      double P[6], v[3];
      if (!act) {
#pragma unroll
        for (int c = 0; c < 6; c++) P[c] = 0.0;
        v[0] = v[1] = v[2] = 0.0;
      } else if (il == (int)threadIdx.x) {
#pragma unroll
        for (int c = 0; c < 6; c++) P[c] = nxt[c];
#pragma unroll
        for (int c = 0; c < 3; c++) v[c] = nxt[6 + c];
      } else {
#pragma unroll
        for (int c = 0; c < 6; c++) P[c] = ca[(size_t)c * W + i];
#pragma unroll
        for (int c = 0; c < 3; c++) v[c] = ca[(size_t)(6 + c) * W + i];
      }
      const double N = !act ? 0.0 : (il == (int)threadIdx.x ? nxt[9] : ca[(size_t)9 * W + i]);
      if (il == (int)threadIdx.x && a + a_step < a_end) fetch(a + a_step, i_first);
      if (REGS) obs_factors<FORM>(fr, P, v, N, preg, racc, 1, 0, col0, col1, col2);
      else obs_factors<FORM>(fr, P, v, N, sp, sacc, Wc, act ? il : wc - 1, col0, col1, col2);
      if (MAXR) track_rowmax(rm, bad, col0, col1, col2);
      if (!staged) {
        if (act) {
          store6(g0 + 6 * i, col0);
          store6(g0 + (size_t)npad + 6 * i, col1);
          store6(g0 + (size_t)2 * npad + 6 * i, col2);
        }
      } else {
        const int nval = 6 * min(64, wc - (il - lane));
        double *gw = g0 + 6 * (size_t)(p0 + il - lane);
        auto flush = [&](const double col[6], double *gcol) {
          d2 *q = reinterpret_cast<d2 *>(stg + 6 * lane);
          d2 t0 = {col[0], col[1]}, t1 = {col[2], col[3]}, t2 = {col[4], col[5]};
          q[0] = t0; q[1] = t1; q[2] = t2;
          asm volatile("" ::: "memory");
#pragma unroll
          for (int j = 0; j < 3; j++) {
            const int idx = 2 * (64 * j + lane);
            const d2 w = *reinterpret_cast<const d2 *>(stg + idx);
            if (idx < nval) *reinterpret_cast<d2 *>(gcol + idx) = w;
          }
          asm volatile("" ::: "memory");
        };
        flush(col0, gw);
        flush(col1, gw + (size_t)npad);
        flush(col2, gw + (size_t)2 * npad);
      }
    }
  }
  double *dp = dpart + (size_t)blockIdx.x * DACC * W + p0;
  if (REGS) {
    if (threadIdx.x < (unsigned)wc) {
#pragma unroll
      for (int k = 0; k < DACC; k++) dp[(size_t)k * W + threadIdx.x] = racc[k];
      if (MAXR) publish_rowmax(rowmax_part, W, p0 + (int)threadIdx.x, rm, bad);
    }
    return;
  }
  __syncthreads();
  for (int t = threadIdx.x; t < DACC * wc; t += blockDim.x) {
    const int k = t / wc, il = t - k * wc;
    dp[(size_t)k * W + il] = sacc[k * Wc + il];
  }
}

template <int FORM, bool MAXR = false>
__global__ __launch_bounds__(320, 3) void k_moments_factors(const double *__restrict__ cl, const double *__restrict__ poses,
                                                         const double *__restrict__ fix, const double *__restrict__ coe_in, int W, int npad,
                                                         int F, double *__restrict__ Gt, double *__restrict__ dpart,
                                                         const int *__restrict__ slot, double *__restrict__ feat_out,
                                                         double *__restrict__ rpart, double *__restrict__ rowmax_part = nullptr) {
  constexpr int DACC = FORM == 0 ? DACC_LEFT : DACC_RIGHT;
  double rm[6] = {0.0, 0.0, 0.0, 0.0, 0.0, 0.0}, bad = 0.0;
  extern __shared__ __attribute__((aligned(16))) double sm[];
  const int npl = (int)blockDim.x - 64, npw = npl >> 6;
  double *sp = sm;
  double *sacc = sm + 12 * W;
  double *mom = sacc + DACC * W;
  double *eig = mom + 80;
  const int tid = threadIdx.x, lane = tid & 63, wv = tid >> 6;
  const bool is_pose = tid < npl;
  for (int t = tid; t < 12 * W; t += blockDim.x) {
    const int i = t / 12, c = t - 12 * i;
    sp[c * W + i] = poses[t];
  }
  for (int t = tid; t < DACC * W; t += blockDim.x) sacc[t] = 0.0;
  __syncthreads();
  const int il = tid, G = gridDim.x, a0 = blockIdx.x;
  const bool has_pose = is_pose && il < W;
  double cur[10], nxt[10];
#pragma unroll
  for (int c = 0; c < 10; c++) cur[c] = nxt[c] = 0.0;
  auto fetch = [&](int a, double (&dst)[10]) {
    const double *ca = cl + (size_t)a * 10 * W + il;
#pragma unroll
// ... 11 lines not shown
      for (int c = 0; c < 3; c++) p[c] = sp[(9 + c) * W + il];
      Obs o;
      to_world(c10, c10 + 6, c10[9], R, p, o);
#pragma unroll
      for (int c = 0; c < 6; c++) m[c] = o.Pw[c];
#pragma unroll
      for (int c = 0; c < 3; c++) m[6 + c] = o.b[c];
      m[9] = c10[9];
    }
#pragma unroll
    for (int c = 0; c < 10; c++) m[c] = wave_sum(m[c]);
    if (lane == 0) {
#pragma unroll
      for (int c = 0; c < 10; c++) mom[(buf * 4 + wv) * 10 + c] = m[c];
    }
  };
  double res = 0.0;
  auto eigen_step = [&](int a, int buf) {
    double c[10];
#pragma unroll
    for (int k = 0; k < 10; k++) {
      double t = mom[(buf * 4) * 10 + k];
      for (int w = 1; w < npw; w++) t += mom[(buf * 4 + w) * 10 + k];
      c[k] = t;
    }
    if (fix) {
#pragma unroll
      for (int k = 0; k < 10; k++) c[k] += fix[(size_t)a * 10 + k];
    }
    const double NN = c[9], inv = 1.0 / NN;
    const double vb0 = c[6] * inv, vb1 = c[7] * inv, vb2 = c[8] * inv;
    double lam[3], U[3][3];
    eig3_jacobi(c[0] * inv - vb0 * vb0, c[1] * inv - vb0 * vb1, c[2] * inv - vb0 * vb2, c[3] * inv - vb1 * vb1,
                c[4] * inv - vb1 * vb2, c[5] * inv - vb2 * vb2, lam, U);
    const double w = coe_in[a];
    res += w * lam[0];
    double rec[FEAT_STRIDE];
#pragma unroll
    for (int k = 0; k < FEAT_STRIDE; k++) rec[k] = 0.0;
    rec[FT_NN] = NN;
    rec[FT_VBAR] = vb0; rec[FT_VBAR + 1] = vb1; rec[FT_VBAR + 2] = vb2;
    rec[FT_LAM] = lam[0]; rec[FT_LAM + 1] = lam[1]; rec[FT_LAM + 2] = lam[2];
#pragma unroll
    for (int k = 0; k < 3; k++) { rec[FT_U0 + k] = U[k][0]; rec[FT_U1 + k] = U[k][1]; rec[FT_U2 + k] = U[k][2]; }
    rec[FT_C0] = sqrt(2.0 * w) * inv;
    rec[FT_C1] = sqrt(2.0 * w / (lam[1] - lam[0])) * inv;
    rec[FT_C2] = sqrt(2.0 * w / (lam[2] - lam[0])) * inv;
    rec[FT_COE] = w;
    if (lane == 0) {
#pragma unroll
      for (int k = 0; k < FEAT_STRIDE; k++) { eig[buf * FEAT_STRIDE + k] = rec[k]; feat_out[(size_t)a * FEAT_STRIDE + k] = rec[k]; }
    }
  };

  if (a0 < F) {
    if (has_pose) fetch(a0, cur);
    if (is_pose) partial_moments(cur, 0);
    if (has_pose && a0 + G < F) fetch(a0 + G, nxt);
  }
  __syncthreads();
  if (!is_pose && a0 < F) eigen_step(a0, 0);
  __syncthreads();
  int b = 0;
  for (int a = a0; a < F; a += G, b ^= 1) {
    const bool has_next = a + G < F;
    if (is_pose && has_next) partial_moments(nxt, b ^ 1);
    __syncthreads();
    if (!is_pose) {
      if (has_next) eigen_step(a + G, b ^ 1);
    } else {
      const double *f = eig + b * FEAT_STRIDE;
      const FeatRec fr = {f[FT_NN], 1.0 / f[FT_NN], {f[FT_VBAR], f[FT_VBAR + 1], f[FT_VBAR + 2]}, {f[FT_U0], f[FT_U0 + 1], f[FT_U0 + 2]},
                          {f[FT_U1], f[FT_U1 + 1], f[FT_U1 + 2]}, {f[FT_U2], f[FT_U2 + 1], f[FT_U2 + 2]}, f[FT_C0], f[FT_C1], f[FT_C2], f[FT_COE]};
      if (has_pose) {
        double col0[6], col1[6], col2[6];
        obs_factors<FORM>(fr, cur, cur + 6, cur[9], sp, sacc, W, il, col0, col1, col2);
        if (MAXR) track_rowmax(rm, bad, col0, col1, col2);
        double *g0 = Gt + (size_t)(3 * (slot ? slot[a] : a)) * npad;
        store6(g0 + 6 * il, col0);
        store6(g0 + (size_t)npad + 6 * il, col1);
        store6(g0 + (size_t)2 * npad + 6 * il, col2);
#pragma unroll
        for (int c = 0; c < 10; c++) cur[c] = nxt[c];
        if (a + 2 * G < F) fetch(a + 2 * G, nxt);
      }
    }
    __syncthreads();
  }
  double *dp = dpart + (size_t)blockIdx.x * DACC * W;
  for (int t = tid; t < DACC * W; t += blockDim.x) dp[t] = sacc[t];
  if (MAXR && has_pose) publish_rowmax(rowmax_part, W, il, rm, bad);
  if (!is_pose && lane == 0) rpart[blockIdx.x] = res;
}

int factors_chunk(int W) { return W <= MAX_W_LDS ? W : 256; }

static size_t factors_lds(int W, int form) {
  const int dacc = form == 0 ? DACC_LEFT : DACC_RIGHT;
  return (size_t)(12 + dacc) * factors_chunk(W) * sizeof(double);
}
constexpr size_t FACTORS_STAGE_BYTES = 4 * 384 * sizeof(double);
static bool factors_staged(int W, int nfeat, int form) {
  if (factors_lds(W, form) + FACTORS_STAGE_BYTES > 160 * 1024) return false;
  if (const char *es = getenv("BALM_FACTORS_STAGE")) return es[0] != '0';
  return (long)nfeat * W >= 1000000;
}

int factors_grid(int W, int nfeat, int form) {
  size_t lds = factors_lds(W, form) + (factors_staged(W, nfeat, form) ? FACTORS_STAGE_BYTES : 0);
  int per_cu = (int)(160 * 1024 / lds);
  if (per_cu < 1) per_cu = 1;
  if (per_cu > 4) per_cu = 4;
  int grid = 256 * per_cu;
  if (grid > nfeat) grid = nfeat;
  if (grid < 1) grid = 1;
  return grid;
}

hipError_t prepare_device_accum() {
  hipError_t e = hipFuncSetAttribute((const void *)k_world_moments, hipFuncAttributeMaxDynamicSharedMemorySize, 160 * 1024);
  if (e == hipSuccess) e = hipFuncSetAttribute((const void *)k_feature_factors<0, false>, hipFuncAttributeMaxDynamicSharedMemorySize, 160 * 1024);
  if (e == hipSuccess) e = hipFuncSetAttribute((const void *)k_feature_factors<1, false>, hipFuncAttributeMaxDynamicSharedMemorySize, 160 * 1024);
  if (e == hipSuccess) e = hipFuncSetAttribute((const void *)k_feature_factors<0, true>, hipFuncAttributeMaxDynamicSharedMemorySize, 160 * 1024);
  if (e == hipSuccess) e = hipFuncSetAttribute((const void *)k_feature_factors<0, true, true>, hipFuncAttributeMaxDynamicSharedMemorySize, 160 * 1024);
  if (e == hipSuccess) e = hipFuncSetAttribute((const void *)k_moments_factors<0, false>, hipFuncAttributeMaxDynamicSharedMemorySize, 160 * 1024);
  if (e == hipSuccess) e = hipFuncSetAttribute((const void *)k_moments_factors<1, false>, hipFuncAttributeMaxDynamicSharedMemorySize, 160 * 1024);
  if (e == hipSuccess) e = hipFuncSetAttribute((const void *)k_moments_factors<0, true>, hipFuncAttributeMaxDynamicSharedMemorySize, 160 * 1024);
  if (e == hipSuccess) e = hipFuncSetAttribute((const void *)k_moments_factors<1, true>, hipFuncAttributeMaxDynamicSharedMemorySize, 160 * 1024);
  return e;
}

int launch_moments_factors(hipStream_t s, int form, const double *cl, const double *poses, const double *fix, const double *coe, int W,
                           int npad, int F, double *Gt, double *dpart, int nblk, const int *slot, double *feat, double *rpart,
                           unsigned long long *rowmax, double *rowmax_part) {
  const int dacc = form == 0 ? DACC_LEFT : DACC_RIGHT;
  const size_t lds = (size_t)((12 + dacc) * W + 80 + 2 * FEAT_STRIDE) * sizeof(double);
  const int bs = (W <= 64 ? 64 : (W <= 128 ? 128 : 256)) + 64;
  if (rowmax) {
    if (form == 0)
      hipLaunchKernelGGL((k_moments_factors<0, true>), dim3(nblk), dim3(bs), lds, s, cl, poses, fix, coe, W, npad, F, Gt, dpart, slot, feat, rpart, rowmax_part);
    else
      hipLaunchKernelGGL((k_moments_factors<1, true>), dim3(nblk), dim3(bs), lds, s, cl, poses, fix, coe, W, npad, F, Gt, dpart, slot, feat, rpart, rowmax_part);
    hipLaunchKernelGGL(k_rowmax_reduce, dim3((npad + 63) / 64), dim3(1024), 0, s, rowmax_part, nblk, W, npad, rowmax);
    return nblk;
  }
  if (form == 0)
    hipLaunchKernelGGL((k_moments_factors<0, false>), dim3(nblk), dim3(bs), lds, s, cl, poses, fix, coe, W, npad, F, Gt, dpart, slot, feat, rpart, nullptr);
  else
    hipLaunchKernelGGL((k_moments_factors<1, false>), dim3(nblk), dim3(bs), lds, s, cl, poses, fix, coe, W, npad, F, Gt, dpart, slot, feat, rpart, nullptr);
  return nblk;
}

bool launch_factors(hipStream_t s, int form, const double *cl, const double *poses, const double *feat, int W,
                    int npad, int f0, int f1, double *Gt, double *dpart, int nblk, const int *slot, unsigned long long *rowmax, double *rowmax_part) {
  const int Wc = factors_chunk(W), chunks = (W + Wc - 1) / Wc;
  size_t lds = factors_lds(W, form);
  int bs = W <= 64 ? 64 : (W <= 128 ? 128 : 256);
  const int staged = factors_staged(W, f1 - f0, form);
  if (staged) lds += FACTORS_STAGE_BYTES;
  const char *er = getenv("BALM_FACTORS_REGS");
  const bool regs = form == 0 && chunks == 1 && W <= bs && !(er && er[0] == '0');
  if (rowmax && regs) {
    hipLaunchKernelGGL((k_feature_factors<0, true, true>), dim3(nblk, chunks), dim3(bs), lds, s, cl, poses, feat, W, Wc, npad, f0, f1, Gt, dpart, slot, staged, rowmax_part);
    hipLaunchKernelGGL(k_rowmax_reduce, dim3((npad + 63) / 64), dim3(1024), 0, s, rowmax_part, nblk, W, npad, rowmax);
    return true;
  }
#define BALM_FACTORS(F, R) hipLaunchKernelGGL((k_feature_factors<F, R, false>), dim3(nblk, chunks), dim3(bs), lds, s, cl, poses, feat, W, Wc, npad, f0, f1, Gt, dpart, slot, staged, nullptr)
  if (form == 0) { if (regs) BALM_FACTORS(0, true); else BALM_FACTORS(0, false); }
  else BALM_FACTORS(1, false);
#undef BALM_FACTORS
  return false;
}

#include "syrk_mfma_asm.inc"

__device__ __forceinline__ void load5(const double *__restrict__ p, double (&x)[TM]) {
#pragma unroll
  for (int r = 0; r < TM; r++) x[r] = p[16 * r];
}

constexpr int SYRK_NBUF = 4;

__device__ __forceinline__ void syrk_sweep(const double *__restrict__ pa, const double *__restrict__ pb, size_t step,
                                           int nsteps) {
  double a[SYRK_NBUF][TM], b[SYRK_NBUF][TM];
#pragma unroll
  for (int i = 0; i < SYRK_NBUF - 1; i++) {
    load5(pa + i * step, a[i]);
    load5(pb + i * step, b[i]);
  }
  pa += (SYRK_NBUF - 1) * step;
  pb += (SYRK_NBUF - 1) * step;
  for (int s = 0; s < nsteps; s += SYRK_NBUF) {
#pragma unroll
    for (int j = 0; j < SYRK_NBUF; j++) {
      const int nb = (j + SYRK_NBUF - 1) % SYRK_NBUF;
      load5(pa, a[nb]);
      load5(pb, b[nb]);
      pa += step; pb += step;
      BALM_SYRK_MFMA_FULL(a[j], b[j])
    }
  }
}

#define BALM_DEFINE_MIXED_SWEEP(V)                                                                                  \
  __device__ __forceinline__ void syrk_sweep_mixed##V(const double *__restrict__ p, size_t step, int nsteps) {    \
    double x[SYRK_NBUF][BALM_SYRK_MIX##V##_NLOAD];                                                                  \
    _Pragma("unroll") for (int i = 0; i < SYRK_NBUF - 1; i++) {                                                    \
      const double *q = p + i * step;                                                                               \
      BALM_SYRK_MIX##V##_LOAD(q, x[i])                                                                              \
    }                                                                                                               \
    p += (SYRK_NBUF - 1) * step;                                                                                    \
    for (int s = 0; s < nsteps; s += SYRK_NBUF) {                                                                   \
      _Pragma("unroll") for (int j = 0; j < SYRK_NBUF; j++) {                                                      \
        const int nb = (j + SYRK_NBUF - 1) % SYRK_NBUF;                                                             \
        BALM_SYRK_MIX##V##_LOAD(p, x[nb])                                                                           \
        p += step;                                                                                                  \
        BALM_SYRK_MIX##V##_MFMA(x[j])                                                                               \
      }                                                                                                             \
    }                                                                                                               \
  }
BALM_DEFINE_MIXED_SWEEP(1)
BALM_DEFINE_MIXED_SWEEP(2)
BALM_DEFINE_MIXED_SWEEP(3)
#undef BALM_DEFINE_MIXED_SWEEP

__device__ __forceinline__ void syrk_accumulate(const double *__restrict__ Gt, int npad, int type, int I, int J,
                                                size_t k_begin, int nsteps) {
  const int lane = threadIdx.x;
  const double *base = Gt + (k_begin + (lane >> 4)) * (size_t)npad + (lane & 15);
  const double *pa = base + I * TILE;
  const double *pb = base + J * TILE;
  const size_t step = (size_t)4 * npad;
  if (type == 0) syrk_sweep(pa, pb, step, nsteps);
  else if (type == 1) syrk_sweep_mixed1(pa, step, nsteps);
  else if (type == 2) syrk_sweep_mixed2(pa, step, nsteps);
  else syrk_sweep_mixed3(pa, step, nsteps);
}

__device__ __forceinline__ void syrk_write_out(double *__restrict__ out) {
  asm volatile("s_nop 15\n\ts_nop 15\n\ts_nop 15" ::: "memory");
  out += threadIdx.x;
#define BALM_X(T)                                                                             \
  {                                                                                           \
    unsigned U[8];                                                                            \
    BALM_SYRK_READ_##T(U);                                                                    \
    _Pragma("unroll") for (int e = 0; e < 4; e++) out[(T * 4 + e) * 64] = __hiloint2double(U[2 * e + 1], U[2 * e]); \
  }
  BALM_SYRK_FOR_TILES(BALM_X)
#undef BALM_X
}

__device__ __forceinline__ long xcd_remap(long bid, long nblocks) {
  const long q = nblocks >> 3, r = nblocks & 7, x = bid & 7;
  return x * q + (x < r ? x : r) + (bid >> 3);
}

__global__ __launch_bounds__(64) void k_hessian_syrk(const double *__restrict__ Gt, int npad, int njobs,
                                                     const int *__restrict__ jobs, int nsteps, long nblocks,
                                                     double *__restrict__ part) {
  const long bid = xcd_remap(blockIdx.x, nblocks);
  const int tile = (int)(bid % njobs);
  const int sg = (int)(bid / njobs);
  BALM_SYRK_ZERO_ACC();
  syrk_accumulate(Gt, npad, jobs[4 * tile], jobs[4 * tile + 1], jobs[4 * tile + 2], (size_t)sg * nsteps * 4, nsteps);
  syrk_write_out(part + ((size_t)sg * njobs + tile) * TILE_ELEMS);
}

__global__ __launch_bounds__(64) void k_hessian_syrk_sparse(const double *__restrict__ Gt, int npad,
                                                            const int *__restrict__ jobs, const int *__restrict__ items,
                                                            const int *__restrict__ chunk_ids, int nsteps, long nitems,
                                                            double *__restrict__ part) {
  const long bid = xcd_remap(blockIdx.x, nitems);
  const int tile = items[4 * bid], first = items[4 * bid + 1], count = items[4 * bid + 2], slot = items[4 * bid + 3];
  const int type = jobs[4 * tile], I = jobs[4 * tile + 1], J = jobs[4 * tile + 2];
  BALM_SYRK_ZERO_ACC();
  for (int c = 0; c < count; c++)
    syrk_accumulate(Gt, npad, type, I, J, (size_t)chunk_ids[first + c] * nsteps * 4, nsteps);
  syrk_write_out(part + (size_t)slot * TILE_ELEMS);
}

SyrkPlan plan_syrk(int ntiles, long K) {
  SyrkPlan p;
  long steps = (K + 3) / 4;
  if (steps < 1) steps = 1;
  long max_sg = steps / 64;
  if (max_sg < 1) max_sg = 1;
  {
    const long one_round = 1024 / ntiles > 1 ? 1024 / ntiles : 1;
    if (max_sg < one_round) {
      long nst = SYRK_NBUF;
      while ((steps + nst - 1) / nst > one_round) nst += SYRK_NBUF;
      p.SG = (int)((steps + nst - 1) / nst);
      p.nsteps = (int)nst;
      p.Kpad = (int)(p.SG * nst * 4);
      p.nblocks = (long)p.SG * ntiles;
      return p;
    }
  }
  long base = (4096 + ntiles - 1) / ntiles, sg = base;
  double best = -1.0;
  for (long c = (base > 6 ? base - 6 : 1); c <= base + 6; c++) {
    const double per_xcd = (double)ntiles * c / 8.0;
    const double rounds = (double)(long)((per_xcd + 127.0) / 128.0);
    const double eff = per_xcd / (rounds * 128.0);
    if (eff > best + 1e-9) { best = eff; sg = c; }
  }
  if (sg > max_sg) sg = max_sg;
  if (steps / sg < 128 && sg > 1) {
    long one_round = 1024 / ntiles;
    if (one_round < 1) one_round = 1;
    if (one_round < sg) sg = one_round;
  }
  long nst = (steps + sg - 1) / sg;
  nst = (nst + SYRK_NBUF - 1) / SYRK_NBUF * SYRK_NBUF;
  p.SG = (int)sg;
  p.nsteps = (int)nst;
  p.Kpad = (int)(sg * nst * 4);
  p.nblocks = sg * ntiles;
  return p;
}

void launch_syrk_sparse(hipStream_t s, const double *Gt, int npad, const int *jobs, const int *items, const int *chunk_ids,
                        int nsteps, long nitems, double *part) {
  hipLaunchKernelGGL(k_hessian_syrk_sparse, dim3((unsigned)nitems), dim3(64), 0, s, Gt, npad, jobs, items, chunk_ids, nsteps,
                     nitems, part);
}

void launch_syrk(hipStream_t s, const double *Gt, int npad, int ntiles, const int *tileIJ, const SyrkPlan &p,
                 double *part) {
  hipLaunchKernelGGL(k_hessian_syrk, dim3((unsigned)p.nblocks), dim3(64), 0, s, Gt, npad, ntiles, tileIJ,
                     p.nsteps, p.nblocks, part);
}

template <class Sink>
__device__ __forceinline__ void reduce_tiles(const double *__restrict__ part, int SG, long tile_total, Sink sink,
                                             int bid, int nb) {
  for (long t = (long)bid * blockDim.x + threadIdx.x; t < tile_total; t += (long)nb * blockDim.x) {
    double s0 = 0.0, s1 = 0.0, s2 = 0.0, s3 = 0.0;
    const double *pp = part + t;
    int g = 0;
    for (; g + 3 < SG; g += 4) {
      s0 += pp[(size_t)g * tile_total];
      s1 += pp[(size_t)(g + 1) * tile_total];
      s2 += pp[(size_t)(g + 2) * tile_total];
      s3 += pp[(size_t)(g + 3) * tile_total];
    }
    for (; g < SG; g++) s0 += pp[(size_t)g * tile_total];
    sink(t, (s0 + s1) + (s2 + s3));
  }
}

template <class Sink>
__device__ __forceinline__ void reduce_tiles_quads(const double *__restrict__ part, int SG, long tile_total, Sink sink, int bid, int nb) {
  const int c = threadIdx.x & 3;
  const int full = SG / 4;
  for (long t = ((long)bid * blockDim.x + threadIdx.x) >> 2; t < tile_total; t += ((long)nb * blockDim.x) >> 2) {
    const double *pp = part + t + (size_t)c * tile_total;
    double s = 0.0;
    int m = 0;
    for (; m + 3 < full; m += 4) {
      const double v0 = pp[(size_t)(4 * m) * tile_total], v1 = pp[(size_t)(4 * m + 4) * tile_total],
                   v2 = pp[(size_t)(4 * m + 8) * tile_total], v3 = pp[(size_t)(4 * m + 12) * tile_total];
      s += v0;
      s += v1;
      s += v2;
      s += v3;
    }
    for (; m < full; m++) s += pp[(size_t)(4 * m) * tile_total];
    if (c == 0)
      for (int g = 4 * full; g < SG; g++) s += part[(size_t)g * tile_total + t];
    s += __shfl_xor(s, 1, 64);
    s += __shfl_xor(s, 2, 64);
    if (c == 0) sink(t, s);
  }
}

template <class Sink>
__device__ __forceinline__ void reduce_tiles_csr(const double *__restrict__ part, const int *__restrict__ ptr, long tile_total,
                                                 Sink sink, int bid, int nb) {
  for (long t = (long)bid * blockDim.x + threadIdx.x; t < tile_total; t += (long)nb * blockDim.x) {
    const int job = (int)(t / TILE_ELEMS);
    const long e = t - (long)job * TILE_ELEMS;
    const int s0 = ptr[job], s1 = ptr[job + 1];
    double a0 = 0.0, a1 = 0.0, a2 = 0.0, a3 = 0.0;
    int g = s0;
    for (; g + 3 < s1; g += 4) {
      a0 += part[(size_t)g * TILE_ELEMS + e];
      a1 += part[(size_t)(g + 1) * TILE_ELEMS + e];
      a2 += part[(size_t)(g + 2) * TILE_ELEMS + e];
      a3 += part[(size_t)(g + 3) * TILE_ELEMS + e];
    }
    for (; g < s1; g++) a0 += part[(size_t)g * TILE_ELEMS + e];
    sink(t, (a0 + a1) + (a2 + a3));
  }
}

__device__ __forceinline__ void reduce_dacc(const double *__restrict__ dpart, int nblk, int dacc_len, int dacc_cap,
                                            const double *__restrict__ rpart, int nr, double *__restrict__ red_dacc,
                                            double *__restrict__ red_r, int bid) {
  __shared__ double sq[256];
  const int jl = threadIdx.x & 63, q = threadIdx.x >> 6;
  const int j = bid * 64 + jl;
  double s = 0.0;
  if (j < dacc_len) {
    const int chunk = (nblk + 3) / 4;
    const int b0 = q * chunk, b1 = min(nblk, b0 + chunk);
    double a[8];
#pragma unroll
    for (int k = 0; k < 8; k++) a[k] = 0.0;
    int b = b0;
    for (; b + 7 < b1; b += 8) {
#pragma unroll
      for (int k = 0; k < 8; k++) a[k] += dpart[(size_t)(b + k) * dacc_len + j];
    }
    for (; b < b1; b++) a[0] += dpart[(size_t)b * dacc_len + j];
    s = ((a[0] + a[1]) + (a[2] + a[3])) + ((a[4] + a[5]) + (a[6] + a[7]));
  }
  sq[threadIdx.x] = s;
  __syncthreads();
  if (q == 0 && j < dacc_len) red_dacc[j] = (sq[jl] + sq[64 + jl]) + (sq[128 + jl] + sq[192 + jl]);
  if (q == 0 && j >= dacc_len && j < dacc_cap) red_dacc[j] = 0.0;
  if (bid == 0) {
    __syncthreads();
    double r = 0.0;
    for (int t = threadIdx.x; t < nr; t += 256) r += rpart[t];
    sq[threadIdx.x] = r;
    __syncthreads();
    for (int k = 128; k > 0; k >>= 1) {
      if (threadIdx.x < k) sq[threadIdx.x] += sq[threadIdx.x + k];
      __syncthreads();
    }
    if (threadIdx.x == 0) { red_r[0] = sq[0]; red_r[1] = 0.0; }
  }
}

__global__ __launch_bounds__(256) void k_reduce_all(const double *__restrict__ part, int SG, const int *__restrict__ csr_ptr, long tile_total,
                                                    int tile_blocks, const double *__restrict__ dpart, int nblk, int dacc_len, int dacc_cap,
                                                    const double *__restrict__ rpart, int nr, double *__restrict__ red, long dacc_off, long r_off, int quads) {
  if ((int)blockIdx.x < tile_blocks) {
    auto to_payload = [&](long t, double v) { red[t] = v; };
    if (csr_ptr) reduce_tiles_csr(part, csr_ptr, tile_total, to_payload, blockIdx.x, tile_blocks);
    else if (quads) reduce_tiles_quads(part, SG, tile_total, to_payload, blockIdx.x, tile_blocks);
    else reduce_tiles(part, SG, tile_total, to_payload, blockIdx.x, tile_blocks);
  } else {
    reduce_dacc(dpart, nblk, dacc_len, dacc_cap, rpart, nr, red + dacc_off, red + r_off, (int)blockIdx.x - tile_blocks);
  }
}

void launch_reduce(hipStream_t s, const double *part, int SG, long tile_total, const double *dpart, int nblk,
                   int dacc_len, const double *rpart, int nr, double *red, long dacc_off, long r_off, const int *csr_ptr) {
  const int dacc_cap = (int)(r_off - dacc_off);
  static const bool no_quads = getenv("BALM_REDUCE_QUADS") && getenv("BALM_REDUCE_QUADS")[0] == '0';
  const int quads = !csr_ptr && !no_quads && tile_total <= 32768 && SG >= 8;
  int grid = (int)(((quads ? 4 : 1) * tile_total + 255) / 256);
  if (grid > 8192) grid = 8192;
  hipLaunchKernelGGL(k_reduce_all, dim3(grid + (dacc_cap + 63) / 64), dim3(256), 0, s, part, SG, csr_ptr, tile_total, grid, dpart, nblk, dacc_len,
                     dacc_cap, rpart, nr, red, dacc_off, r_off, quads);
}

__device__ __forceinline__ int sym3(int r, int c) {
  if (r > c) { int t = r; r = c; c = t; }
  return r == 0 ? c : (r == 1 ? 2 + c : 5);
}

template <int FORM>
__device__ __forceinline__ double blockdiag_at(const double *__restrict__ dacc, int W, int i, int r, int c) {
  const double *d = dacc + i;
  if (FORM == 0) {
    if (r < 3 && c < 3) return d[(size_t)(6 + sym3(r, c)) * W];
    if (r < 3 && c >= 3) return d[(size_t)(12 + 3 * r + (c - 3)) * W];
    if (r >= 3 && c < 3) return d[(size_t)(12 + 3 * c + (r - 3)) * W];
    return d[(size_t)(21 + sym3(r - 3, c - 3)) * W];
  } else {
    if (r < 3 && c < 3) return d[(size_t)(6 + 3 * r + c) * W];
    if (r < 3 && c >= 3) return d[(size_t)(15 + 3 * r + (c - 3)) * W];
    if (r >= 3 && c < 3) return d[(size_t)(15 + 3 * c + (r - 3)) * W];
    return d[(size_t)(24 + sym3(r - 3, c - 3)) * W];
  }
}

template <int FORM>
__global__ __launch_bounds__(256) void k_assemble(const double *__restrict__ red, long dacc_off,
                                                  const int *__restrict__ tileIJ, int ntiles, int W,
                                                  double *__restrict__ H, double *__restrict__ g, const double *__restrict__ r_in,
                                                  double *__restrict__ r_out) {
  const int n = 6 * W;
  if (r_out && blockIdx.x == 0 && threadIdx.x == 0) *r_out = *r_in;
  const long total = (long)ntiles * TILE_ELEMS;
  const double *dacc = red + dacc_off;
  for (long t = (long)blockIdx.x * blockDim.x + threadIdx.x; t < total; t += (long)gridDim.x * blockDim.x) {
    const int tile = (int)(t / TILE_ELEMS);
    const int e = (int)(t - (long)tile * TILE_ELEMS);
    const int lane = e & 63, slot = e >> 6;
    const int reg = slot & 3, mt = slot >> 2;
    const int rc = tileIJ[tile * 25 + mt];
    const int row = (rc >> 16) * 16 + (lane >> 4) + 4 * reg;
    const int col = (rc & 0xffff) * 16 + (lane & 15);
    if (row >= n || col >= n || row > col) continue;
    double val = -red[t];
    const int pi = row / 6, pj = col / 6;
    if (pi == pj) {
      const int r = row - 6 * pi, c = col - 6 * pi;
      val += blockdiag_at<FORM>(dacc, W, pi, r, c);
      if (FORM == 1 && r != c) {
        H[(size_t)row * n + col] = -red[t] + blockdiag_at<FORM>(dacc, W, pi, c, r);
        H[(size_t)col * n + row] = val;
        continue;
      }
    }
    H[(size_t)col * n + row] = val;
    H[(size_t)row * n + col] = val;
  }
  for (long t = (long)blockIdx.x * blockDim.x + threadIdx.x; t < n; t += (long)gridDim.x * blockDim.x) {
    const int i = (int)(t / 6), k = (int)(t - 6 * (t / 6));
    g[t] = dacc[(size_t)k * W + i];
  }
}

void launch_assemble(hipStream_t s, int form, const double *red, long dacc_off, const int *tileIJ, int ntiles, int W,
                     double *H, double *g, const double *r_in, double *r_out) {
  long total = (long)ntiles * TILE_ELEMS;
  int grid = (int)((total + 255) / 256);
  if (grid > 4096) grid = 4096;
  if (form == 0)
    hipLaunchKernelGGL(k_assemble<0>, dim3(grid), dim3(256), 0, s, red, dacc_off, tileIJ, ntiles, W, H, g, r_in, r_out);
  else
    hipLaunchKernelGGL(k_assemble<1>, dim3(grid), dim3(256), 0, s, red, dacc_off, tileIJ, ntiles, W, H, g, r_in, r_out);
}


}
```

### balm_amd/csrc/kernels_solve.hip

```cpp
#include <algorithm>
#include <cfloat>
#include <cstdlib>
#include <cstring>

#include "balm_internal.h"

namespace balm {

typedef double d4 __attribute__((ext_vector_type(4)));

template <int MAXI>
__global__ __launch_bounds__(256) void k_rank_diag(const double *__restrict__ H, int n, int nA, int *__restrict__ perm) {
  extern __shared__ __attribute__((aligned(16))) double dabs[];
  int *part = reinterpret_cast<int *>(dabs + nA);
  double dv[MAXI];
#pragma unroll
  for (int it = 0; it < MAXI; it++) {
    const int i = threadIdx.x + 256 * it;
    dv[it] = i < n ? fabs(H[(size_t)i * n + i]) : -1.0;
  }
#pragma unroll
  for (int it = 0; it < MAXI; it++) {
    const int i = threadIdx.x + 256 * it;
    if (i < nA) dabs[i] = dv[it] == dv[it] ? dv[it] : -0.5;
// ... 707 lines not shown
}

static void launch_build_A(balm_ctx *c) {
  const int n = c->n, nA = c->nA, P = nA / NB;
  const double *pu = c->u_on_device ? c->d_scal + SCAL_U : nullptr;
  const int tiled = c->solve_tiled ? 1 : 0;
  const int nflags = 2 * (2 * P + 1) * P + P + 8;
  const size_t lds = (size_t)n * sizeof(double);
#define BALM_BUILD_A(M) hipLaunchKernelGGL(k_build_A<M>, dim3(nA), dim3(256), lds, c->stream, c->d_H, c->d_g, n, nA, c->d_perm, pu, c->u_value, \
                                           c->d_A, c->d_flags, nflags, c->d_x + nA, c->d_minv + (size_t)P * NB * NB, tiled)
  if (nA <= 256 * 5) BALM_BUILD_A(5);
  else if (nA <= 256 * 10) BALM_BUILD_A(10);
  else if (nA <= 256 * 16) BALM_BUILD_A(16);
  else BALM_BUILD_A(25);
#undef BALM_BUILD_A
}

static void launch_factor(balm_ctx *c) {
  hipStream_t s = c->stream;
  const int nA = c->nA, P = nA / NB;
  const bool backsub = c->solve_tiled;
  bool want_fused = backsub || solve_is_persistent(c);
  c->solve_backsub = false;
  static const bool dbg = getenv("BALM_SOLVE_DEBUG") != nullptr;
  if (dbg) fprintf(stderr, "balm_hip: solve P=%d persistent=%d backsub=%d chain_cap=%d fused_cap=%d multi=%d\n", P, (int)want_fused,
                   (int)backsub, c->chain_cap, c->fused_cap, c->multi ? c->multi->n : 0);
  if (backsub) {
    if (launch_factor_chain(c, false, c->solve_tiled)) { c->solve_backsub = true; return; }
    if (P > FUSED_MAX_P) want_fused = false;
    if (c->solve_tiled) { c->solve_tiled = false; launch_build_A(c); }
  } else {
    if (want_fused && solve_wants_chain(c, solve_mode()) && launch_factor_chain(c, true, false)) return;
  }
  if (want_fused) {
    const size_t lds = (size_t)(12 * FLR + 2 * NB * NB + NB) * sizeof(double);
    if (c->fused_cap < 0) c->fused_cap = fused_capacity(lds);
    const int RB = 2 * P + 1;
    int NH = persistent_slots(c, c->fused_cap) - RB;
    const int most = (P - 2) * P;
    if (NH > most) NH = most;
    if (P == 2) NH = 0;
    if (NH >= (P > 2 ? 1 : 0)) {
      FusedArgs fa{c->d_A, c->d_dvec, c->d_z, c->d_flags, c->d_flags + (size_t)RB * P, nA, P, RB, NH > 0 ? NH : 1, c->d_trace};
      if (persistent_launch(c, k_ldl_fused, dim3(RB + (P > 2 ? NH : 0)), dim3(FT), fa, lds, s) == hipSuccess)
        return;
      hipGetLastError();
      c->fused_cap = 0;
    }
  }
  const char *la = getenv("BALM_LOOKAHEAD");
  const bool lookahead = la ? !strcmp(la, "1") : true;
  const size_t wp_stride = (size_t)NB * (2 * nA + NB);
  for (int p = 0; p < P; p++) {
    const int c0 = p * NB;
    const int m = nA - c0 - NB;
    const int nR = nA + NB + NB * (p + 1);
    const int rows = nR - (c0 + NB);
    const int npb = (rows + PANEL_ROWS - 1) / PANEL_ROWS;
    const int mt = m / NB;
    double *Wp = c->d_Wp + (lookahead ? (size_t)(p & 1) * wp_stride : 0);
    const int mt_prev = mt + 1;
    if (lookahead && p > 0 && mt_prev > 1) {
      const int gx = (3 * (mt_prev - 1) + 3) / 4, gy = mt_prev + 1 + p;
      hipLaunchKernelGGL(k_ldl_panel_trail, dim3(npb + gx * gy), dim3(256), 0, s, c->d_A, nA, c0, nR, c->d_dvec, Wp, c->d_z, npb,
                         c0 - NB, c->d_Wp + (size_t)((p - 1) & 1) * wp_stride, mt_prev, gx);
    } else {
      hipLaunchKernelGGL(k_ldl_panel, dim3(npb), dim3(256), 0, s, c->d_A, nA, c0, nR, c->d_dvec, Wp, c->d_z);
    }
    if (m <= 0) continue;
    const int gy = mt + 1 + (p + 1);
    if (lookahead) hipLaunchKernelGGL(k_ldl_trail, dim3(1, gy), dim3(256), 0, s, c->d_A, nA, c0, Wp, mt, 0, 3);
    else hipLaunchKernelGGL(k_ldl_trail, dim3((3 * mt + 3) / 4, gy), dim3(256), 0, s, c->d_A, nA, c0, Wp, mt, 0, 3 * mt);
  }
}

#include "kernels_small.inc"

void launch_solve(balm_ctx *c, bool new_hessian, int upd_form, const double *upd_poses, double *upd_out) {
  hipStream_t s = c->stream;
  const int n = c->n, nA = c->nA;
  if (solve_wants_small(c)) {
    c->solve_backsub = false; c->solve_tiled = false;
    if (launch_solve_small(c, upd_form, upd_poses, upd_out)) return;
  }
  const double *pu = c->u_on_device ? c->d_scal + SCAL_U : nullptr;
  if (new_hessian) {
    const size_t lds = (size_t)nA * sizeof(double) + 256 * sizeof(int);
    const dim3 grid((nA + 15) / 16);
    if (nA <= 256 * 5) hipLaunchKernelGGL(k_rank_diag<5>, grid, dim3(256), lds, s, c->d_H, n, nA, c->d_perm);
    else if (nA <= 256 * 10) hipLaunchKernelGGL(k_rank_diag<10>, grid, dim3(256), lds, s, c->d_H, n, nA, c->d_perm);
    else if (nA <= 256 * 16) hipLaunchKernelGGL(k_rank_diag<16>, grid, dim3(256), lds, s, c->d_H, n, nA, c->d_perm);
    else hipLaunchKernelGGL(k_rank_diag<25>, grid, dim3(256), lds, s, c->d_H, n, nA, c->d_perm);
  }
  c->solve_tiled = solve_wants_backsub(c);
  launch_build_A(c);
  if (c->inject_solve_timeout) {
    const int P = nA / NB;
    hipMemsetAsync(c->d_flags + (size_t)2 * (2 * P + 1) * P + P, 1, sizeof(int), s);
    c->inject_solve_timeout = false;
  }
  launch_factor(c);
  if (c->solve_backsub) {
    const int P = nA / NB;
    hipLaunchKernelGGL(k_ldl_backsolve, dim3(P), dim3(256), 0, s, c->d_A, nA, P, c->solve_tiled ? 1 : 0, c->d_minv, c->d_dvec, c->d_z, c->d_x + nA, c->d_x,
                       c->d_flags + (size_t)2 * (2 * P + 1) * P + P);
  } else {
    hipLaunchKernelGGL(k_ldl_apply, dim3((nA + 63) / 64, APPLY_CHUNKS), dim3(256), 0, s, c->d_A, nA, c->d_dvec, c->d_z, c->d_x);
  }
  {
    const int P = nA / NB;
    int *abortf = c->d_flags + (size_t)2 * (2 * P + 1) * P + P;
    const int nch = c->solve_backsub ? 1 : APPLY_CHUNKS;
    hipLaunchKernelGGL(k_ldl_finish, dim3(1), dim3(1024), 0, s, c->d_x, nA, n, c->d_perm, c->d_H, c->d_g, pu, c->u_value, c->d_dx,
                       c->d_scal, abortf, upd_form, c->W, upd_poses, upd_out, nch);
  }
}

__global__ void k_update_poses(int form, int W, const double *__restrict__ poses, const double *__restrict__ dx,
                               double *__restrict__ out) {
  const int j = blockIdx.x * blockDim.x + threadIdx.x;
  if (j < W) update_pose(form, j, poses, dx, out);
}

void launch_update_poses(hipStream_t s, int form, int W, const double *poses, const double *dx, double *out) {
  hipLaunchKernelGGL(k_update_poses, dim3((W + 127) / 128), dim3(128), 0, s, form, W, poses, dx, out);
}

__global__ __launch_bounds__(256) void k_reanchor(int W, double *__restrict__ poses) {
  __shared__ double e0[12];
  if (threadIdx.x < 12) e0[threadIdx.x] = poses[threadIdx.x];
  __syncthreads();
  for (int j = threadIdx.x; j < W; j += blockDim.x) {
    double *q = poses + 12 * j;
    double R[3][3], p[3] = {q[9] - e0[9], q[10] - e0[10], q[11] - e0[11]};
#pragma unroll
    for (int c = 0; c < 3; c++)
#pragma unroll
      for (int r = 0; r < 3; r++) R[r][c] = q[3 * c + r];
#pragma unroll
    for (int r = 0; r < 3; r++) {
#pragma unroll
      for (int c = 0; c < 3; c++)
        q[3 * c + r] = e0[3 * r] * R[0][c] + e0[3 * r + 1] * R[1][c] + e0[3 * r + 2] * R[2][c];
      q[9 + r] = e0[3 * r] * p[0] + e0[3 * r + 1] * p[1] + e0[3 * r + 2] * p[2];
    }
  }
}

void launch_reanchor(hipStream_t s, int W, double *poses) {
  hipLaunchKernelGGL(k_reanchor, dim3(1), dim3(256), 0, s, W, poses);
}

__global__ __launch_bounds__(256) void k_scalars_mail(double *__restrict__ scal, volatile double *__restrict__ host, double stamp,
                                                      const double *__restrict__ rpart, int nr, int slot) {
  __shared__ double sred[256];
  if (rpart) {
    double s = 0.0;
    for (int t = threadIdx.x; t < nr; t += 256) s += rpart[t];
    sred[threadIdx.x] = s;
    __syncthreads();
    for (int k = 128; k > 0; k >>= 1) {
      if (threadIdx.x < k) sred[threadIdx.x] += sred[threadIdx.x + k];
      __syncthreads();
    }
    if (threadIdx.x == 0) scal[slot] = sred[0];
    __syncthreads();
  }
  if (threadIdx.x < 16) host[threadIdx.x] = (rpart && (int)threadIdx.x == slot) ? sred[0] : scal[threadIdx.x];
  __threadfence_system();
  __syncthreads();
  if (threadIdx.x == 0) { host[SCAL_STAMP] = stamp; __threadfence_system(); }
}

void launch_scalars_mail(hipStream_t s, double *d_scal, double *d_hscal, double stamp, const double *rpart, int nr, int slot) {
  hipLaunchKernelGGL(k_scalars_mail, dim3(1), dim3(256), 0, s, d_scal, d_hscal, stamp, rpart, nr, slot);
}

hipError_t preload_solve() {
  hipFuncAttributes a;
  return hipFuncGetAttributes(&a, (const void *)k_ldl_apply);
}

}
```

### include/balm_hip.h

```cpp
#ifndef BALM_HIP_H
#define BALM_HIP_H

#include <stddef.h>

#ifdef __cplusplus
extern "C" {
#endif

typedef struct balm_ctx balm_ctx;

enum { BALM_FORM_LEFT = 0, BALM_FORM_RIGHT = 1 };

enum {
  BALM_OK = 0,
  BALM_ERR_ARG = 1,
  BALM_ERR_HIP = 2,
  BALM_ERR_STATE = 3,
  BALM_ERR_TOO_FEW_PLANES = 4,
  BALM_ERR_NUMERIC = 5
};

enum {
  BALM_FLAG_TIMING = 1,
  BALM_FLAG_LOOPBACK_SHARDS = 2,
  BALM_FLAG_SYRK_INT8 = 4
};

typedef struct balm_iter_log {
  double r1, r2, u, v, q, q1;
  int accepted;
  int hess_evaluated;
} balm_iter_log;

typedef struct balm_lm_opts {
  int form;
  double u0;
  int max_iter;
  double rel_tol;
  int min_planes_per_pose;
  int force_hess;
  int no_stop;
  int verbose;
  int reanchor;
  double abs_tol;
} balm_lm_opts;

balm_ctx *balm_create(int win_size, int device, int flags);
void balm_destroy(balm_ctx *ctx);

int balm_prewarm(int device);

balm_ctx *balm_create_multi(int win_size, int first_device, int n_devices, int flags);

int balm_comm_unique_id(void *id128);
int balm_comm_init_rank(balm_ctx *ctx, int n_ranks, int rank, const void *id128);
int balm_comm_info(balm_ctx *ctx, long *out4);

int balm_set_features(balm_ctx *ctx, int F, const double *clusters, const double *fix,
                      const double *coeffs);

typedef void (*balm_fill_clusters_fn)(void *user, int f0, int f1, double *dst);
int balm_set_features_cb(balm_ctx *ctx, int F, balm_fill_clusters_fn fill, void *user, const double *fix,
                         const double *coeffs);

int balm_evaluate(balm_ctx *ctx, int form, const double *poses, int head, int end, double *Hess,
                  double *JacT, double *residual);

int balm_only_residual(balm_ctx *ctx, const double *poses, double *residual);

int balm_solve_damped(balm_ctx *ctx, const double *Hess, const double *JacT, double u, double *dxi,
                      double *q1);

int balm_damping_iter(balm_ctx *ctx, const balm_lm_opts *opts, double *poses_inout,
                      balm_iter_log *log, int *n_iters);

int balm_build_clusters(balm_ctx *ctx, int F, const float *xyz, const int *feat_id,
                        const int *pose_id, long n_pts, const double *fix, const double *coeffs,
                        double *clusters_out);

int balm_build_clusters_planes(balm_ctx *ctx, int F, const void *const *plane_points, const long *plane_count,
                               size_t stride_bytes, size_t pose_offset_bytes, const double *fix, const double *coeffs,
                               double *clusters_out);

typedef struct balm_voxel_opts {
  double voxel_size;
  float eigen_thr[3];
  int min_ps;
  int layer_limit;
  int min_observers;
  int fix_frames;
  double max_plane_dist;
  double max_lambda21;
  double max_lambda0;
  int want_point_features;
  int fix_point_limit;
  int defer_recut;
} balm_voxel_opts;
void balm_voxel_defaults(balm_voxel_opts *opts);
int balm_associate(balm_ctx *ctx, const balm_voxel_opts *opts, const float *xyz, const int *frame_id,
                   long n_pts, const double *poses, int *F_out, long *n_root_voxels);

int balm_associate_scans(balm_ctx *ctx, const balm_voxel_opts *opts, int n_scans, const void *const *scan_points,
                         const long *scan_count, size_t stride_bytes, const double *poses, int *F_out,
                         long *n_root_voxels);

int balm_window_open(balm_ctx *ctx, const balm_voxel_opts *opts);
int balm_window_recut(balm_ctx *ctx);
int balm_window_add_scan(balm_ctx *ctx, const float *xyz, long n_pts, const double *pose12);
int balm_window_add_scan_strided(balm_ctx *ctx, const void *points, long n_pts, size_t stride_bytes, const double *pose12);
int balm_window_features(balm_ctx *ctx, int *F_out);
int balm_window_marginalize(balm_ctx *ctx, int mg_size, const double *poses);
int balm_window_info(balm_ctx *ctx, int *scans_in_window, long *points, long *nodes);
int balm_window_get_points(balm_ctx *ctx, float *xyz, int *slot, int *feature, long capacity, long *n_out);
int balm_window_close(balm_ctx *ctx);

int balm_get_features(balm_ctx *ctx, double *clusters, double *coeffs, int *layer);

int balm_get_association(balm_ctx *ctx, double *fix, int *point_feature);

int balm_pose_covariance(balm_ctx *ctx, const double *poses, const double *cluster_cov, double point_sigma,
                         double *Rcov, double *Rcov_raw);

typedef int (*balm_allreduce_fn)(void *dev_buf, long n_doubles, void *user);
int balm_set_allreduce(balm_ctx *ctx, balm_allreduce_fn fn, void *user);

enum {
  BALM_T_MOMENTS = 0,
  BALM_T_FACTORS = 1,
  BALM_T_SYRK = 2,
  BALM_T_ASSEMBLE = 3,
  BALM_T_SOLVE = 4,
  BALM_T_UPDATE = 5,
  BALM_T_BUILD = 6,
  BALM_T_VOXEL = 7,
  BALM_T_COV = 8,
  BALM_T_COMM = 9,
  BALM_T_UPLOAD = 10,
  BALM_T_COUNT = 11
};
int balm_get_timing(balm_ctx *ctx, double *ms, long *count);
int balm_get_shard_timing(balm_ctx *ctx, int shard, double *ms, long *count);

int balm_get_solve_trace(balm_ctx *ctx, long long *ticks, long capacity, int *dims3);
int balm_reset_timing(balm_ctx *ctx);

int balm_chain_macro_plan(int panels, int helpers, int *table, long capacity);

int balm_work_model(balm_ctx *ctx, double *out4);

const char *balm_last_error(balm_ctx *ctx);
const char *balm_version(void);

#define BALM_ABI_VERSION 6
int balm_abi_version(void);

#ifdef __cplusplus
}
#endif
#endif
```

Measured before the change: 243.3.

## Speculatively queue next LM Hessian evaluation behind device-side accept/stop decision

After the trial residual is computed, a device kernel now decides whether the step is accepted and whether iteration continues, writing a go flag. The next iteration's Hessian evaluation (factors, SYRK, reduce, assemble) is enqueued immediately behind it and reads the flag to skip or pick the trial poses and features, so the GPU no longer idles during the host round-trip. The host waits on an event rather than syncing the whole stream. This adds gated kernels that may launch and exit early, plus state-tracking complexity, and is disabled for multi-device, int8 SYRK, fused-trial and graph modes.

```diff
diff --git a/balm_amd/capi.py b/balm_amd/capi.py
--- a/balm_amd/capi.py
+++ b/balm_amd/capi.py
@@ -12,6 +12,7 @@
 FLAG_TIMING = 1
 FLAG_LOOPBACK_SHARDS = 2
 FLAG_SYRK_INT8 = 4
+FLAG_LM_HOST_ORDER = 8
 T_MOMENTS, T_FACTORS, T_SYRK, T_ASSEMBLE, T_SOLVE, T_UPDATE, T_BUILD, T_VOXEL, T_COV, T_COMM, T_UPLOAD, T_COUNT = range(12)
 TIMING_NAMES = ["moments", "factors", "syrk", "assemble", "solve", "update", "build", "voxel", "cov", "comm", "upload"]
 
diff --git a/balm_amd/csrc/balm_capi.hip b/balm_amd/csrc/balm_capi.hip
--- a/balm_amd/csrc/balm_capi.hip
+++ b/balm_amd/csrc/balm_capi.hip
@@ -194,15 +194,20 @@
   if (hipStreamSynchronize(ctx->stream) == hipSuccess) collect_timing(ctx);
 }
 
-int wait_scalars(balm_ctx *ctx) {
+int wait_scalars(balm_ctx *ctx, bool work_behind = false) {
   volatile double *stamp = ctx->h_scal + SCAL_STAMP;
   const double want = (double)ctx->mail_seq;
   const auto t0 = std::chrono::steady_clock::now();
   for (int spin = 0;; spin++) {
-    if (*stamp == want) { std::atomic_thread_fence(std::memory_order_acquire); collect_timing_if_idle(ctx); return BALM_OK; }
+    if (*stamp == want) { std::atomic_thread_fence(std::memory_order_acquire); if (!work_behind) collect_timing_if_idle(ctx); return BALM_OK; }
     if ((spin & 255) == 255 && std::chrono::steady_clock::now() - t0 > std::chrono::microseconds(300)) break;
   }
-  int rc = sync_stream(ctx);
+  int rc = BALM_OK;
+  if (work_behind) {
+    HIP_TRY(hipEventSynchronize(ctx->mail_event));
+    HIP_TRY(hipGetLastError());
+    std::atomic_thread_fence(std::memory_order_acquire);
+  } else rc = sync_stream(ctx);
   if (rc) return rc;
   if (*stamp != want) { ctx->err = "balm_damping_iter: the iteration's scalars did not arrive"; return BALM_ERR_HIP; }
   return BALM_OK;
@@ -215,14 +220,16 @@
   }
 }
 
-int residual_device(balm_ctx *ctx, const double *d_poses, int f0, int f1, int slot, bool defer_sum = false, bool send_mail = false) {
+int residual_device(balm_ctx *ctx, const double *d_poses, int f0, int f1, int slot, bool defer_sum = false, bool send_mail = false,
+                    const LmDecide *dec = nullptr) {
   if (f1 <= f0) {
     HIP_TRY(hipMemsetAsync(ctx->d_scal + slot, 0, sizeof(double), ctx->stream));
     ctx->nr_tmp = 0;
   } else {
     Span sp(ctx, BALM_T_MOMENTS);
     launch_world_moments(ctx->stream, ctx->d_cl, d_poses, ctx->W, f0, f1, ctx->d_C);
-    const EigenMail mail{ctx->d_scal, ctx->d_hscal, send_mail ? (double)++ctx->mail_seq : 0.0, slot};
+    const EigenMail mail{ctx->d_scal, ctx->d_hscal, send_mail ? (double)++ctx->mail_seq : 0.0, slot,
+                         dec ? *dec : LmDecide{nullptr, 0.0, 0.0, 0, 0}};
     ctx->nr_tmp = launch_feature_eigen(ctx->stream, ctx->d_C, ctx->has_fix ? ctx->d_fix : nullptr, ctx->d_coe, f0, f1, ctx->d_feat_tmp,
                                        ctx->d_rpart_tmp, send_mail ? &mail : nullptr);
     if (!defer_sum) launch_sum_scalar(ctx->stream, ctx->d_rpart_tmp, ctx->nr_tmp, ctx->d_scal + slot);
@@ -281,7 +288,7 @@
   return BALM_OK;
 }
 
-int evaluate_device(balm_ctx *ctx, int form, const double *d_poses, int f0, int f1, int slot) {
+int evaluate_device(balm_ctx *ctx, int form, const double *d_poses, int f0, int f1, int slot, const LmGo *ahead = nullptr) {
   const int W = ctx->W, nf = f1 - f0;
   const int dacc = form == 0 ? DACC_LEFT : DACC_RIGHT;
   int rc;
@@ -297,6 +304,9 @@
   if ((rc = prepare_evaluate(ctx, form, nf))) return rc;
   const int nblk = factors_grid(W, nf, form);
   hipStream_t s = ctx->stream;
+  if (ahead && !(ctx->feat_cur_valid && !ctx->gt_cur_valid && f0 == 0 && f1 == ctx->F && !syrk_int8_for(ctx, 3L * nf))) {
+    ctx->err = "evaluate_device: this evaluation cannot be queued ahead"; return BALM_ERR_STATE;
+  }
   if (!(ctx->feat_cur_valid && f0 == 0 && f1 == ctx->F)) {
     Span sp(ctx, BALM_T_MOMENTS);
     launch_world_moments(s, ctx->d_cl, d_poses, W, f0, f1, ctx->d_C);
@@ -317,31 +327,33 @@
     }
     ctx->gt_dirty_cols = k0;
     ctx->rowmax_cur_valid = launch_factors(s, form, ctx->d_cl, d_poses, ctx->d_feat, W, ctx->npad, f0, f1, ctx->d_Gt, ctx->d_dpart, nblk,
-                                           sparse ? ctx->d_slot : nullptr, (!sparse && syrk_int8_for(ctx, 3L * nf)) ? ctx->d_rowmax : nullptr, ctx->d_rowmax_part);
+                                           sparse ? ctx->d_slot : nullptr, (!sparse && syrk_int8_for(ctx, 3L * nf)) ? ctx->d_rowmax : nullptr, ctx->d_rowmax_part,
+                                           ahead);
     ctx->gt_cur_valid = false;
   }
   HIP_TRY(hipGetLastError());
   const bool int8 = !sparse && syrk_int8_for(ctx, 3L * nf);
   {
     Span sp(ctx, BALM_T_SYRK);
-    if (sparse) launch_syrk_sparse(s, ctx->d_Gt, ctx->npad, ctx->d_jobs, ctx->d_items, ctx->d_chunk_ids, ctx->sp_nsteps, ctx->sp_nitems, ctx->d_part);
+    if (sparse) launch_syrk_sparse(s, ctx->d_Gt, ctx->npad, ctx->d_jobs, ctx->d_items, ctx->d_chunk_ids, ctx->sp_nsteps, ctx->sp_nitems, ctx->d_part,
+                                   ahead ? ahead->go : nullptr);
     else if (int8) {
       if (launch_syrk_i8(s, ctx->d_Gt, ctx->npad, ctx->n, 3L * nf, ctx->d_sub, ctx->ntiles, ctx->d_i8, ctx->d_part,
                          ctx->rowmax_cur_valid ? ctx->d_rowmax : nullptr)) { ctx->err = "INT8 SYRK: unsupported size"; return BALM_ERR_ARG; }
       plan.SG = 1;
     }
-    else launch_syrk(s, ctx->d_Gt, ctx->npad, ctx->ntiles, ctx->d_jobs, plan, ctx->d_part);
+    else launch_syrk(s, ctx->d_Gt, ctx->npad, ctx->ntiles, ctx->d_jobs, plan, ctx->d_part, ahead ? ahead->go : nullptr);
   }
   {
     Span sp(ctx, BALM_T_ASSEMBLE);
     launch_reduce(s, ctx->d_part, plan.SG, (long)ctx->ntiles * TILE_ELEMS, ctx->d_dpart, nblk, dacc * W,
-                  ctx->d_rpart, nr, ctx->d_red, red_dacc_off(ctx), red_r_off(ctx), sparse ? ctx->d_csr : nullptr);
+                  ctx->d_rpart, nr, ctx->d_red, red_dacc_off(ctx), red_r_off(ctx), sparse ? ctx->d_csr : nullptr, ahead);
   }
   if ((rc = hook_allreduce(ctx, ctx->d_red, (long)ctx->red_len))) return rc;
   {
     Span sp(ctx, BALM_T_ASSEMBLE);
     launch_assemble(s, form, ctx->d_red, red_dacc_off(ctx), ctx->d_sub, ctx->ntiles, W, ctx->d_H, ctx->d_g, ctx->d_red + red_r_off(ctx),
-                    ctx->d_scal + slot);
+                    ctx->d_scal + slot, ahead ? ahead->go : nullptr);
   }
   return BALM_OK;
 }
@@ -497,8 +509,10 @@
       dalloc(ctx, &ctx->d_A, (size_t)(2 * nA + NB) * nA) || dalloc(ctx, &ctx->d_Wp, (size_t)2 * NB * (2 * nA + NB)) ||
       dalloc(ctx, &ctx->d_dvec, (size_t)nA) || dalloc(ctx, &ctx->d_z, (size_t)nA) || dalloc(ctx, &ctx->d_x, (size_t)16 * nA) ||
       dalloc(ctx, &ctx->d_perm, (size_t)nA) || dalloc(ctx, &ctx->d_flags, (size_t)2 * (2 * (nA / NB) + 1) * (nA / NB) + (nA / NB) + 8) || dalloc(ctx, &ctx->d_minv, (size_t)2 * (nA / NB) * NB * NB) || dalloc(ctx, &ctx->d_dx, (size_t)n) ||
-      dalloc(ctx, &ctx->d_scal, (size_t)16) || dalloc(ctx, &ctx->d_pre, (size_t)W + 2))
+      dalloc(ctx, &ctx->d_scal, (size_t)16) || dalloc(ctx, &ctx->d_pre, (size_t)W + 2) || dalloc(ctx, &ctx->d_lm_go, (size_t)2))
     return fail();
+  if (hipEventCreateWithFlags(&ctx->mail_event, hipEventDisableTiming) != hipSuccess) { ctx->mail_event = nullptr; return fail(); }
+  ctx->lm_ahead = !(flags & BALM_FLAG_LM_HOST_ORDER);
   if (hipHostMalloc((void **)&ctx->h_scal, (16 + 64 + 8) * sizeof(double), hipHostMallocMapped | hipHostMallocCoherent) != hipSuccess) return fail();
   if (hipHostGetDevicePointer((void **)&ctx->d_hscal, ctx->h_scal, 0) != hipSuccess) return fail();
   ctx->h_scal[SCAL_STAMP] = 0.0;
@@ -516,6 +530,7 @@
     if (hipMemcpy(ctx->d_perm, ident.data(), (size_t)nA * sizeof(int), hipMemcpyHostToDevice) != hipSuccess) return fail();
   }
   if (hipMemset(ctx->d_scal, 0, 16 * sizeof(double)) != hipSuccess) return fail();
+  if (hipMemset(ctx->d_lm_go, 0, 2 * sizeof(int)) != hipSuccess) return fail();
   if (hipMemset(ctx->d_red, 0, ctx->red_len * sizeof(double)) != hipSuccess) return fail();
   if (hipMemset(ctx->d_minv, 0, (size_t)2 * (nA / NB) * NB * NB * sizeof(double)) != hipSuccess) return fail();
   cold_mark("balm_create: device buffers + small copies");
@@ -533,7 +548,7 @@
   if (ctx->window) { window_close(ctx->window); ctx->window = nullptr; }
   void *ptrs[] = {ctx->d_cl, ctx->d_fix, ctx->d_coe, ctx->d_poses, ctx->d_poses_tmp, ctx->d_C, ctx->d_feat,
                   ctx->d_Gt, ctx->d_Gt2, ctx->d_dpart2, ctx->d_part, ctx->d_dpart, ctx->d_rpart, ctx->d_feat_tmp, ctx->d_rpart_tmp, ctx->d_red, ctx->d_jobs, ctx->d_sub, ctx->d_H,
-                  ctx->d_g, ctx->d_A, ctx->d_Wp, ctx->d_dvec, ctx->d_z, ctx->d_x, ctx->d_perm, ctx->d_dx, ctx->d_scal, ctx->d_arena, ctx->d_pre, ctx->d_flags, ctx->d_minv, ctx->d_macro_tab, ctx->d_trace, ctx->d_slot, ctx->d_items, ctx->d_csr, ctx->d_chunk_ids, ctx->d_stage, ctx->d_i8, ctx->d_rowmax, ctx->d_rowmax2, ctx->d_rowmax_part};
+                  ctx->d_g, ctx->d_A, ctx->d_Wp, ctx->d_dvec, ctx->d_z, ctx->d_x, ctx->d_perm, ctx->d_dx, ctx->d_scal, ctx->d_arena, ctx->d_pre, ctx->d_flags, ctx->d_minv, ctx->d_macro_tab, ctx->d_trace, ctx->d_slot, ctx->d_items, ctx->d_csr, ctx->d_chunk_ids, ctx->d_stage, ctx->d_i8, ctx->d_rowmax, ctx->d_rowmax2, ctx->d_rowmax_part, ctx->d_lm_go};
   for (void *p : ptrs) if (p) hipFree(p);
   if (ctx->h_scal) hipHostFree(ctx->h_scal);
   ctx->ring.release();
@@ -541,6 +556,7 @@
   if (ctx->amail.scan_state) hipFree(ctx->amail.scan_state);
   for (auto &sp : ctx->timer.pending) { hipEventDestroy(sp.a); hipEventDestroy(sp.b); }
   for (auto e : ctx->timer.pool) hipEventDestroy(e);
+  if (ctx->mail_event) hipEventDestroy(ctx->mail_event);
   if (ctx->stream) hipStreamDestroy(ctx->stream);
   delete ctx;
 }
@@ -1262,27 +1278,47 @@
   return BALM_OK;
 }
 
-static int lm_enqueue(balm_ctx *ctx, int form, bool evaluated, bool mail) {
+struct LmAhead { LmDecide dec; bool queue_next, hess_queued; };
+static int lm_enqueue(balm_ctx *ctx, int form, bool evaluated, bool mail, LmAhead *ah = nullptr) {
   int rc;
-  if (evaluated && (rc = evaluate_device(ctx, form, ctx->d_poses, 0, ctx->F, 0))) return rc;
+  if (evaluated && !(ah && ah->hess_queued) && (rc = evaluate_device(ctx, form, ctx->d_poses, 0, ctx->F, 0))) return rc;
+  if (ah) {
+    ah->queue_next = ah->queue_next && ctx->feat_cur_valid && !ctx->gt_cur_valid;
+    ah->dec.go = ah->queue_next ? ctx->d_lm_go : nullptr;
+  }
+  const LmDecide *dec = (ah && ah->dec.go) ? &ah->dec : nullptr;
   {
     Span sp(ctx, BALM_T_SOLVE);
     launch_solve(ctx, evaluated, form, ctx->d_poses, ctx->d_poses_tmp);
   }
   ctx->gt_trial_valid = false;
-  bool sum_in_mail = false;
+  bool sum_in_mail = false, sent = false;
   if (fuse_trial(ctx) && ctx->d_Gt2 && ctx->d_dpart2) {
     if ((rc = trial_device(ctx, form, ctx->d_poses_tmp, 1))) return rc;
   } else {
     sum_in_mail = mail && !has_transport(ctx) && ctx->F > 0;
     const bool eigen_mails = sum_in_mail && ctx->F <= 256;
-    if ((rc = residual_device(ctx, ctx->d_poses_tmp, 0, ctx->F, 1, sum_in_mail, eigen_mails))) return rc;
-    if (eigen_mails) return BALM_OK;
-  }
-  if (mail) launch_scalars_mail(ctx->stream, ctx->d_scal, ctx->d_hscal, (double)++ctx->mail_seq, sum_in_mail ? ctx->d_rpart_tmp : nullptr,
-                                ctx->nr_tmp, 1);
+    if ((rc = residual_device(ctx, ctx->d_poses_tmp, 0, ctx->F, 1, sum_in_mail, eigen_mails, dec))) return rc;
+    sent = eigen_mails;
+  }
+  if (ah && !sum_in_mail) { ctx->err = "lm_enqueue: no mail to queue behind"; return BALM_ERR_STATE; }
+  if (sent) ;
+  else if (mail) launch_scalars_mail(ctx->stream, ctx->d_scal, ctx->d_hscal, (double)++ctx->mail_seq, sum_in_mail ? ctx->d_rpart_tmp : nullptr,
+                                     ctx->nr_tmp, 1, dec);
   else HIP_TRY(hipMemcpyAsync(ctx->h_scal, ctx->d_scal, 16 * sizeof(double), hipMemcpyDeviceToHost, ctx->stream));
-  return BALM_OK;
+  if (!ah) return BALM_OK;
+  HIP_TRY(hipEventRecord(ctx->mail_event, ctx->stream));
+  if (ah->queue_next) {
+    const LmGo go{ctx->d_lm_go, ctx->d_poses_tmp, ctx->d_feat_tmp, ctx->d_rpart_tmp};
+    if ((rc = evaluate_device(ctx, form, ctx->d_poses, 0, ctx->F, 0, &go))) return rc;
+  }
+  return BALM_OK;
+}
+
+static bool lm_ahead_ok(const balm_ctx *ctx) {
+  if (!ctx->lm_ahead || ctx->multi || has_transport(ctx) || ctx->F < 1 || fuse_trial(ctx) || syrk_int8_for(ctx, 3L * ctx->F)) return false;
+  const char *genv = getenv("BALM_GRAPH");
+  return !(genv && (!strcmp(genv, "1") || !strcmp(genv, "debug")));
 }
 
 static int lm_iteration(balm_ctx *ctx, int form, bool evaluated, int it) {
@@ -1329,7 +1365,7 @@
   return wait_scalars(ctx);
 }
 
-static int one_damping_iter(balm_ctx *ctx, const balm_lm_opts *o, double *poses, balm_iter_log *log, int *n_iters) {
+static int damping_iter_body(balm_ctx *ctx, const balm_lm_opts *o, double *poses, balm_iter_log *log, int *n_iters, bool *hess_queued_out) {
   if (!ctx) return BALM_ERR_ARG;
   if (!ctx->multi && ctx->F < 1) { ctx->err = "balm_damping_iter: no features installed"; return BALM_ERR_STATE; }
   if (!o || !poses || (o->form != 0 && o->form != 1) || o->max_iter < 1) {
@@ -1368,6 +1404,8 @@
   double u = o->u0, v = 2, r1 = 0, r2 = 0;
   bool calc = true;
   int it = 0;
+  const bool ahead = lm_ahead_ok(ctx);
+  bool &hess_queued = *hess_queued_out;
   int fault_rank = -1, fault_it = -1, timeout_it = -1;
   if (const char *fi = getenv("BALM_FAULT_INJECT")) {
     if (!strncmp(fi, "timeout,", 8)) timeout_it = atoi(fi + 8);
@@ -1378,7 +1416,13 @@
     if (ctx->rank == fault_rank && it == fault_it) { ctx->err = "balm_damping_iter: injected fault"; return BALM_ERR_HIP; }
     if (it == timeout_it) { ctx->inject_solve_timeout = true; timeout_it = -1; }
     if ((rc = set_damping(ctx, u))) return rc;
-    if ((rc = lm_iteration(ctx, o->form, evaluated, it))) return rc;
+    if (ahead) {
+      LmAhead ah{{nullptr, o->rel_tol, o->abs_tol, o->no_stop ? 1 : 0, o->force_hess ? 1 : 0}, it + 1 < o->max_iter, hess_queued};
+      rc = lm_enqueue(ctx, o->form, evaluated, true, &ah);
+      hess_queued = rc ? true : ah.queue_next;
+      if (!rc) rc = wait_scalars(ctx, true);
+      if (rc) return rc;
+    } else if ((rc = lm_iteration(ctx, o->form, evaluated, it))) return rc;
     double sc[3] = {ctx->h_scal[0], ctx->h_scal[1], ctx->h_scal[2]};
     if ((rc = multi_share_scalars(ctx, it, sc, 3))) return rc;
     r1 = sc[0]; r2 = sc[1];
@@ -1389,6 +1433,7 @@
       drop_lm_graphs(ctx);
       ctx->feat_cur_valid = false; ctx->gt_cur_valid = false;
       calc = true;
+      hess_queued = false;
       continue;
     }
     if (!(std::isfinite(r1) && std::isfinite(r2))) {
@@ -1432,9 +1477,17 @@
   if (o->reanchor) launch_reanchor(s, W, ctx->d_poses);
   HIP_TRY(hipMemcpyAsync(poses, ctx->d_poses, (size_t)12 * W * sizeof(double), hipMemcpyDeviceToHost, s));
   if ((rc = sync_stream(ctx))) return rc;
+  hess_queued = false;
   if (n_iters) *n_iters = it;
   cold_mark("damping_iter: done");
   return BALM_OK;
+}
+
+static int one_damping_iter(balm_ctx *ctx, const balm_lm_opts *o, double *poses, balm_iter_log *log, int *n_iters) {
+  bool hess_queued = false;
+  const int rc = damping_iter_body(ctx, o, poses, log, n_iters, &hess_queued);
+  if (rc && hess_queued && ctx && ctx->stream) { hipStreamSynchronize(ctx->stream); hipGetLastError(); }
+  return rc;
 }
 
 static balm_multi *leader_of(balm_ctx *ctx) { return (ctx && ctx->multi && ctx->rank == 0) ? ctx->multi : nullptr; }
diff --git a/balm_amd/csrc/balm_internal.h b/balm_amd/csrc/balm_internal.h
--- a/balm_amd/csrc/balm_internal.h
+++ b/balm_amd/csrc/balm_internal.h
@@ -132,6 +132,9 @@
   int lm_graph_form[LM_GRAPHS] = {};
   bool graphs_ok = true;
   int parity = 0;
+  bool lm_ahead = true;
+  int *d_lm_go = nullptr;
+  hipEvent_t mail_event = nullptr;
   std::vector<int> planes_per_pose;
   double work_S = 0, work_B = 0;
   std::vector<double> assoc_clusters, assoc_coeffs;
@@ -164,6 +167,17 @@
 
 namespace balm {
 
+constexpr int LM_GO_RUN = 1;
+constexpr int LM_GO_ACCEPTED = 2;
+struct LmDecide { int *go; double rel_tol, abs_tol; int no_stop, force_hess; };
+__device__ __forceinline__ void lm_decide(const LmDecide &d, double r1, double r2) {
+  const bool accepted = (r1 - r2) > 0;
+  const bool stop = !d.no_stop && (fabs(r1 - r2) / r1 < d.rel_tol || (d.abs_tol > 0 && fabs(r1 - r2) < d.abs_tol));
+  const bool run = !stop && (accepted || d.force_hess);
+  d.go[0] = (run ? LM_GO_RUN : 0) | (accepted ? LM_GO_ACCEPTED : 0);
+}
+struct LmGo { const int *go; const double *poses_alt, *feat_alt, *rpart_alt; };
+
 hipError_t prepare_device_accum();
 hipError_t prepare_device_cov();
 hipError_t preload_solve();
@@ -171,28 +185,29 @@
 hipError_t preload_voxel();
 void launch_transpose_clusters(hipStream_t s, const double *aos, double *soa, int F, int W);
 void launch_world_moments(hipStream_t s, const double *cl, const double *poses, int W, int f0, int f1, double *C);
-struct EigenMail { double *scal; double *host; double stamp; int slot; };
+struct EigenMail { double *scal; double *host; double stamp; int slot; LmDecide dec; };
 int launch_feature_eigen(hipStream_t s, const double *C, const double *fix, const double *coe, int f0, int f1,
                          double *feat, double *rpart, const EigenMail *mail = nullptr);
 int factors_grid(int W, int nfeat, int form);
 int factors_chunk(int W);
 bool launch_factors(hipStream_t s, int form, const double *cl, const double *poses, const double *feat, int W,
                     int npad, int f0, int f1, double *Gt, double *dpart, int nblk, const int *slot = nullptr,
-                    unsigned long long *rowmax = nullptr, double *rowmax_part = nullptr);
+                    unsigned long long *rowmax = nullptr, double *rowmax_part = nullptr,
+                    const LmGo *ahead = nullptr);
 int launch_moments_factors(hipStream_t s, int form, const double *cl, const double *poses, const double *fix, const double *coe, int W,
                            int npad, int F, double *Gt, double *dpart, int nblk, const int *slot, double *feat, double *rpart,
                            unsigned long long *rowmax = nullptr, double *rowmax_part = nullptr);
 struct SyrkPlan { int SG; int nsteps; int Kpad; long nblocks; };
 SyrkPlan plan_syrk(int ntiles, long K);
 void launch_syrk(hipStream_t s, const double *Gt, int npad, int ntiles, const int *tileIJ, const SyrkPlan &p,
-                 double *part);
+                 double *part, const int *go = nullptr);
 void launch_syrk_sparse(hipStream_t s, const double *Gt, int npad, const int *jobs, const int *items, const int *chunk_ids,
-                        int nsteps, long nitems, double *part);
+                        int nsteps, long nitems, double *part, const int *go = nullptr);
 void launch_reduce(hipStream_t s, const double *part, int SG, long tile_elems_total, const double *dpart, int nblk,
                    int dacc_len, const double *rpart, int nr, double *red, long red_dacc_off, long red_r_off,
-                   const int *csr_ptr = nullptr);
+                   const int *csr_ptr = nullptr, const LmGo *ahead = nullptr);
 void launch_assemble(hipStream_t s, int form, const double *red, long red_dacc_off, const int *tileIJ, int ntiles,
-                     int W, double *H, double *g, const double *r_in = nullptr, double *r_out = nullptr);
+                     int W, double *H, double *g, const double *r_in = nullptr, double *r_out = nullptr, const int *go = nullptr);
 void launch_sum_scalar(hipStream_t s, const double *rpart, int nr, double *out);
 struct I8Layout { int T, rows_p, NT, M; long Kp; size_t off_digits, off_rowmax, off_scale, off_part; };
 size_t syrk_i8_scratch_bytes(int n, long K, I8Layout *lay);
@@ -255,7 +270,7 @@
 void launch_solve(balm_ctx *c, bool new_hessian, int upd_form = 0, const double *upd_poses = nullptr, double *upd_out = nullptr);
 void launch_update_poses(hipStream_t s, int form, int W, const double *poses, const double *dx, double *out);
 void launch_scalars_mail(hipStream_t s, double *d_scal, double *d_hscal, double stamp, const double *rpart = nullptr, int nr = 0,
-                         int slot = 0);
+                         int slot = 0, const LmDecide *dec = nullptr);
 void launch_reanchor(hipStream_t s, int W, double *poses);
 
 struct AssocOpts {
diff --git a/balm_amd/csrc/kernels_accum.hip b/balm_amd/csrc/kernels_accum.hip
--- a/balm_amd/csrc/kernels_accum.hip
+++ b/balm_amd/csrc/kernels_accum.hip
@@ -233,6 +233,7 @@
   __threadfence_system();
   __syncthreads();
   if (threadIdx.x == 0) { host[SCAL_STAMP] = mail.stamp; __threadfence_system(); }
+  if (threadIdx.x == 0 && mail.dec.go) lm_decide(mail.dec, mail.scal[0], sred[0]);
 }
 
 int launch_feature_eigen(hipStream_t s, const double *C, const double *fix, const double *coe, int f0, int f1,
@@ -240,7 +241,7 @@
   int nf = f1 - f0;
   if (nf <= 0) return 0;
   int grid = (nf + 255) / 256;
-  const EigenMail none{nullptr, nullptr, 0.0, 0};
+  const EigenMail none{nullptr, nullptr, 0.0, 0, {nullptr, 0.0, 0.0, 0, 0}};
   hipLaunchKernelGGL(k_feature_eigen, dim3(grid), dim3(256), 0, s, C, fix, coe, f0, f1, feat, rpart, (mail && grid == 1) ? *mail : none);
   return grid;
 }
@@ -494,8 +495,12 @@
                                                          const double *__restrict__ feat, int W, int Wc, int npad, int f0,
                                                          int f1, double *__restrict__ Gt,
                                                          double *__restrict__ dpart, const int *__restrict__ slot, int staged,
-                                                         double *__restrict__ rowmax_part = nullptr) {
+                                                         double *__restrict__ rowmax_part, const int *__restrict__ go,
+                                                         const double *__restrict__ poses_alt, const double *__restrict__ feat_alt) {
   static_assert(!MAXR || REGS, "the row maxima live in the lane that owns the pose");
+  const int verdict = go ? *go : LM_GO_RUN;
+  if (!(verdict & LM_GO_RUN)) return;
+  if (verdict & LM_GO_ACCEPTED) { poses = poses_alt; feat = feat_alt; }
   double rm[6] = {0.0, 0.0, 0.0, 0.0, 0.0, 0.0}, bad = 0.0;
   constexpr int DACC = FORM == 0 ? DACC_LEFT : DACC_RIGHT;
   extern __shared__ __attribute__((aligned(16))) double sm[];
@@ -813,7 +818,9 @@
 }
 
 bool launch_factors(hipStream_t s, int form, const double *cl, const double *poses, const double *feat, int W,
-                    int npad, int f0, int f1, double *Gt, double *dpart, int nblk, const int *slot, unsigned long long *rowmax, double *rowmax_part) {
+                    int npad, int f0, int f1, double *Gt, double *dpart, int nblk, const int *slot, unsigned long long *rowmax, double *rowmax_part,
+                    const LmGo *ahead) {
+  const LmGo go = ahead ? *ahead : LmGo{nullptr, nullptr, nullptr, nullptr};
   const int Wc = factors_chunk(W), chunks = (W + Wc - 1) / Wc;
   size_t lds = factors_lds(W, form);
   int bs = W <= 64 ? 64 : (W <= 128 ? 128 : 256);
@@ -822,11 +829,11 @@
   const char *er = getenv("BALM_FACTORS_REGS");
   const bool regs = form == 0 && chunks == 1 && W <= bs && !(er && er[0] == '0');
   if (rowmax && regs) {
-    hipLaunchKernelGGL((k_feature_factors<0, true, true>), dim3(nblk, chunks), dim3(bs), lds, s, cl, poses, feat, W, Wc, npad, f0, f1, Gt, dpart, slot, staged, rowmax_part);
+    hipLaunchKernelGGL((k_feature_factors<0, true, true>), dim3(nblk, chunks), dim3(bs), lds, s, cl, poses, feat, W, Wc, npad, f0, f1, Gt, dpart, slot, staged, rowmax_part, go.go, go.poses_alt, go.feat_alt);
     hipLaunchKernelGGL(k_rowmax_reduce, dim3((npad + 63) / 64), dim3(1024), 0, s, rowmax_part, nblk, W, npad, rowmax);
     return true;
   }
-#define BALM_FACTORS(F, R) hipLaunchKernelGGL((k_feature_factors<F, R, false>), dim3(nblk, chunks), dim3(bs), lds, s, cl, poses, feat, W, Wc, npad, f0, f1, Gt, dpart, slot, staged, nullptr)
+#define BALM_FACTORS(F, R) hipLaunchKernelGGL((k_feature_factors<F, R, false>), dim3(nblk, chunks), dim3(bs), lds, s, cl, poses, feat, W, Wc, npad, f0, f1, Gt, dpart, slot, staged, nullptr, go.go, go.poses_alt, go.feat_alt)
   if (form == 0) { if (regs) BALM_FACTORS(0, true); else BALM_FACTORS(0, false); }
   else BALM_FACTORS(1, false);
 #undef BALM_FACTORS
@@ -919,7 +926,8 @@
 
 __global__ __launch_bounds__(64) void k_hessian_syrk(const double *__restrict__ Gt, int npad, int njobs,
                                                      const int *__restrict__ jobs, int nsteps, long nblocks,
-                                                     double *__restrict__ part) {
+                                                     double *__restrict__ part, const int *__restrict__ go) {
+  if (go && !(*go & LM_GO_RUN)) return;
   const long bid = xcd_remap(blockIdx.x, nblocks);
   const int tile = (int)(bid % njobs);
   const int sg = (int)(bid / njobs);
@@ -931,7 +939,8 @@
 __global__ __launch_bounds__(64) void k_hessian_syrk_sparse(const double *__restrict__ Gt, int npad,
                                                             const int *__restrict__ jobs, const int *__restrict__ items,
                                                             const int *__restrict__ chunk_ids, int nsteps, long nitems,
-                                                            double *__restrict__ part) {
+                                                            double *__restrict__ part, const int *__restrict__ go) {
+  if (go && !(*go & LM_GO_RUN)) return;
   const long bid = xcd_remap(blockIdx.x, nitems);
   const int tile = items[4 * bid], first = items[4 * bid + 1], count = items[4 * bid + 2], slot = items[4 * bid + 3];
   const int type = jobs[4 * tile], I = jobs[4 * tile + 1], J = jobs[4 * tile + 2];
@@ -983,15 +992,15 @@
 }
 
 void launch_syrk_sparse(hipStream_t s, const double *Gt, int npad, const int *jobs, const int *items, const int *chunk_ids,
-                        int nsteps, long nitems, double *part) {
+                        int nsteps, long nitems, double *part, const int *go) {
   hipLaunchKernelGGL(k_hessian_syrk_sparse, dim3((unsigned)nitems), dim3(64), 0, s, Gt, npad, jobs, items, chunk_ids, nsteps,
-                     nitems, part);
+                     nitems, part, go);
 }
 
 void launch_syrk(hipStream_t s, const double *Gt, int npad, int ntiles, const int *tileIJ, const SyrkPlan &p,
-                 double *part) {
+                 double *part, const int *go) {
   hipLaunchKernelGGL(k_hessian_syrk, dim3((unsigned)p.nblocks), dim3(64), 0, s, Gt, npad, ntiles, tileIJ,
-                     p.nsteps, p.nblocks, part);
+                     p.nsteps, p.nblocks, part, go);
 }
 
 template <class Sink>
@@ -1098,7 +1107,13 @@
 
 __global__ __launch_bounds__(256) void k_reduce_all(const double *__restrict__ part, int SG, const int *__restrict__ csr_ptr, long tile_total,
                                                     int tile_blocks, const double *__restrict__ dpart, int nblk, int dacc_len, int dacc_cap,
-                                                    const double *__restrict__ rpart, int nr, double *__restrict__ red, long dacc_off, long r_off, int quads) {
+                                                    const double *__restrict__ rpart, int nr, double *__restrict__ red, long dacc_off, long r_off, int quads,
+                                                    LmGo ahead) {
+  if (ahead.go) {
+    const int verdict = *ahead.go;
+    if (!(verdict & LM_GO_RUN)) return;
+    if (verdict & LM_GO_ACCEPTED) rpart = ahead.rpart_alt;
+  }
   if ((int)blockIdx.x < tile_blocks) {
     auto to_payload = [&](long t, double v) { red[t] = v; };
     if (csr_ptr) reduce_tiles_csr(part, csr_ptr, tile_total, to_payload, blockIdx.x, tile_blocks);
@@ -1110,14 +1125,14 @@
 }
 
 void launch_reduce(hipStream_t s, const double *part, int SG, long tile_total, const double *dpart, int nblk,
-                   int dacc_len, const double *rpart, int nr, double *red, long dacc_off, long r_off, const int *csr_ptr) {
+                   int dacc_len, const double *rpart, int nr, double *red, long dacc_off, long r_off, const int *csr_ptr, const LmGo *ahead) {
   const int dacc_cap = (int)(r_off - dacc_off);
   static const bool no_quads = getenv("BALM_REDUCE_QUADS") && getenv("BALM_REDUCE_QUADS")[0] == '0';
   const int quads = !csr_ptr && !no_quads && tile_total <= 32768 && SG >= 8;
   int grid = (int)(((quads ? 4 : 1) * tile_total + 255) / 256);
   if (grid > 8192) grid = 8192;
   hipLaunchKernelGGL(k_reduce_all, dim3(grid + (dacc_cap + 63) / 64), dim3(256), 0, s, part, SG, csr_ptr, tile_total, grid, dpart, nblk, dacc_len,
-                     dacc_cap, rpart, nr, red, dacc_off, r_off, quads);
+                     dacc_cap, rpart, nr, red, dacc_off, r_off, quads, ahead ? *ahead : LmGo{nullptr, nullptr, nullptr, nullptr});
 }
 
 __device__ __forceinline__ int sym3(int r, int c) {
@@ -1145,7 +1160,8 @@
 __global__ __launch_bounds__(256) void k_assemble(const double *__restrict__ red, long dacc_off,
                                                   const int *__restrict__ tileIJ, int ntiles, int W,
                                                   double *__restrict__ H, double *__restrict__ g, const double *__restrict__ r_in,
-                                                  double *__restrict__ r_out) {
+                                                  double *__restrict__ r_out, const int *__restrict__ go) {
+  if (go && !(*go & LM_GO_RUN)) return;
   const int n = 6 * W;
   if (r_out && blockIdx.x == 0 && threadIdx.x == 0) *r_out = *r_in;
   const long total = (long)ntiles * TILE_ELEMS;
@@ -1180,15 +1196,15 @@
 }
 
 void launch_assemble(hipStream_t s, int form, const double *red, long dacc_off, const int *tileIJ, int ntiles, int W,
-                     double *H, double *g, const double *r_in, double *r_out) {
+                     double *H, double *g, const double *r_in, double *r_out, const int *go) {
   long total = (long)ntiles * TILE_ELEMS;
   int grid = (int)((total + 255) / 256);
   if (grid > 4096) grid = 4096;
   if (form == 0)
-    hipLaunchKernelGGL(k_assemble<0>, dim3(grid), dim3(256), 0, s, red, dacc_off, tileIJ, ntiles, W, H, g, r_in, r_out);
+    hipLaunchKernelGGL(k_assemble<0>, dim3(grid), dim3(256), 0, s, red, dacc_off, tileIJ, ntiles, W, H, g, r_in, r_out, go);
   else
-    hipLaunchKernelGGL(k_assemble<1>, dim3(grid), dim3(256), 0, s, red, dacc_off, tileIJ, ntiles, W, H, g, r_in, r_out);
-}
-
-
-}
+    hipLaunchKernelGGL(k_assemble<1>, dim3(grid), dim3(256), 0, s, red, dacc_off, tileIJ, ntiles, W, H, g, r_in, r_out, go);
+}
+
+
+}
diff --git a/balm_amd/csrc/kernels_solve.hip b/balm_amd/csrc/kernels_solve.hip
--- a/balm_amd/csrc/kernels_solve.hip
+++ b/balm_amd/csrc/kernels_solve.hip
@@ -883,7 +883,7 @@
 }
 
 __global__ __launch_bounds__(256) void k_scalars_mail(double *__restrict__ scal, volatile double *__restrict__ host, double stamp,
-                                                      const double *__restrict__ rpart, int nr, int slot) {
+                                                      const double *__restrict__ rpart, int nr, int slot, LmDecide dec) {
   __shared__ double sred[256];
   if (rpart) {
     double s = 0.0;
@@ -901,10 +901,12 @@
   __threadfence_system();
   __syncthreads();
   if (threadIdx.x == 0) { host[SCAL_STAMP] = stamp; __threadfence_system(); }
-}
-
-void launch_scalars_mail(hipStream_t s, double *d_scal, double *d_hscal, double stamp, const double *rpart, int nr, int slot) {
-  hipLaunchKernelGGL(k_scalars_mail, dim3(1), dim3(256), 0, s, d_scal, d_hscal, stamp, rpart, nr, slot);
+  if (threadIdx.x == 0 && dec.go) lm_decide(dec, scal[0], (rpart && slot == 1) ? sred[0] : scal[1]);
+}
+
+void launch_scalars_mail(hipStream_t s, double *d_scal, double *d_hscal, double stamp, const double *rpart, int nr, int slot, const LmDecide *dec) {
+  hipLaunchKernelGGL(k_scalars_mail, dim3(1), dim3(256), 0, s, d_scal, d_hscal, stamp, rpart, nr, slot,
+                     dec ? *dec : LmDecide{nullptr, 0.0, 0.0, 0, 0});
 }
 
 hipError_t preload_solve() {
diff --git a/include/balm_hip.h b/include/balm_hip.h
--- a/include/balm_hip.h
+++ b/include/balm_hip.h
@@ -23,7 +23,8 @@
 enum {
   BALM_FLAG_TIMING = 1,
   BALM_FLAG_LOOPBACK_SHARDS = 2,
-  BALM_FLAG_SYRK_INT8 = 4
+  BALM_FLAG_SYRK_INT8 = 4,
+  BALM_FLAG_LM_HOST_ORDER = 8
 };
 
 typedef struct balm_iter_log {
```

Result: no change. 244.3, median of 4 (+0.4%).
